# PengjieRen/CaSE_RG

Measured on AMD Instinct MI355X. Metric: train tokens/sec (query+passage) CaSE model, higher is better.
Workload: dtype bf16; 1 GPU; CaSE train step fwd+bwd+allreduce+clip+Adam+EMA, d_model=512, 6 encoder layers, 10 passages x 384 tok, query 64, answer 40, vocab 30522, per-GPU batch 32, dropout on; global_batch=32, parallelism=dp1

## Files before the change

### case_rg_amd/_abi.py

```python
import ctypes as C
import os

import torch

_HERE = os.path.dirname(os.path.abspath(__file__))
LIB_PATH = os.environ.get("CASE_HIP_LIB") or os.path.join(_HERE, "csrc", "libcase_hip.so")

ABI_VERSION = 600
F32, BF16 = 0, 1
WS_ATTENTION_SPLITKV, WS_ATTENTION_BWD, WS_OPTIM_SUMSQ, WS_ENCODER_CHAIN_PACK, WS_GEMM_DW_SLABS = 1, 2, 3, 4, 5
(FEAT_GEMM_256, FEAT_GEMM_SMALL, FEAT_ENCODER_CHAIN, FEAT_ATTN_SCORES, FEAT_ATTN_DECODE, FEAT_OPTIM, FEAT_ATTN_RESIDENT, FEAT_RESERVED_CUS,
 FEAT_GEMM_DW_SLABS, FEAT_DECODER_CHAIN, FEAT_ATTN_DECODE_MQA, FEAT_POINTER_DECODE, FEAT_POINTER_HEAD, FEAT_GEMM_LN, FEAT_STEP_STATE,
 FEAT_INTERACTION, FEAT_ATTN_DECODE_APPEND, FEAT_LINEAR_SKINNY) = (1 << i for i in range(18))
EPI_BIAS_COL, EPI_BIAS_ROW, EPI_GELU, EPI_RELU = 1, 2, 4, 8
EPI_RESIDUAL, EPI_MUL_DGELU, EPI_MUL_DRELU, EPI_ATOMIC, EPI_DROPOUT = 16, 32, 64, 128, 256

i32, i64, u64, f32, f64, ptr = C.c_int32, C.c_int64, C.c_uint64, C.c_float, C.c_double, C.c_void_p


class GemmDesc(C.Structure):
    _fields_ = [(n, i64) for n in ("M", "N", "K", "lda", "ldb", "ldc", "ld_aux", "batch1", "batch2",
                                   "sa1", "sa2", "sb1", "sb2", "sc1", "sc2", "saux1", "saux2")] + \
               [(n, i32) for n in ("a_kmajor", "b_kmajor", "in_dtype", "out_dtype", "epilogue", "split_k", "tile")] + \
               [("alpha", f32), ("drop_p", f32), ("seed", u64), ("offset", u64), ("state", ptr)]


class StepState(C.Structure):
    _fields_ = [("rng_base", u64), ("step_size", f32), ("bc2_sqrt", f32), ("lr", f32), ("step", i32), ("reserved", u64 * 5)]


class EncoderChainDesc(C.Structure):
    _fields_ = [("rows", i64), ("width", i32), ("variant", i32), ("eps_ln2", f32), ("eps_ln1_next", f32)]


class SoftmaxDesc(C.Structure):
    _fields_ = [("outer", i64), ("inner", i64), ("R", i64), ("C", i64), ("causal", i32), ("in_dtype", i32),
                ("out_dtype", i32), ("drop_p", f32), ("seed", u64), ("offset", u64), ("state", ptr)]


class AttnDesc(C.Structure):
    _fields_ = [(n, i64) for n in ("N", "heads", "Lq", "Lk", "head_dim", "ldq", "ldk", "ldv", "sq", "sk", "sv", "ldo", "so")] + \
               [("causal", i32), ("scale", f32), ("drop_p", f32), ("seed", u64), ("offset", u64), ("state", ptr)]


class InteractionDesc(C.Structure):
    _fields_ = [(n, i64) for n in ("n", "Lp", "Lq", "H", "eq_div")] + [("dtype", i32)]


class AttnProductDesc(C.Structure):
    _fields_ = [(n, i64) for n in ("N", "heads", "M", "Kc", "head_dim", "lda", "sa_seq", "sa_head", "ldb", "sb_seq", "sb_head",
                                   "ldc", "sc_seq", "sc_head")] + [("a_transposed", i32), ("alpha", f32)]


SIGNATURES = {
    "case_gemm": [C.POINTER(GemmDesc), ptr, ptr, ptr, ptr, ptr, ptr, ptr, ptr],
    "case_gemm_dw_bias": [C.POINTER(GemmDesc), ptr, ptr, ptr, ptr, ptr],
    "case_gemm_dw_slabs": [C.POINTER(GemmDesc), ptr, ptr, ptr, ptr, ptr, i64, ptr],
    "case_embed_pos_fwd": [ptr, ptr, ptr, ptr, i64, i64, i64, i64, f32, f32, u64, u64, ptr, i32, ptr],
    "case_embed_pos_bwd": [ptr, ptr, ptr, i64, i64, i64, f32, f32, u64, u64, ptr, i32, ptr],
    "case_scale_add_rows": [ptr, ptr, ptr, i64, i64, i64, f32, i32, ptr],
    "case_layernorm_fwd": [ptr, ptr, ptr, ptr, ptr, ptr, ptr, i64, i64, f32, i32, ptr],
    "case_layernorm_bwd": [ptr, ptr, ptr, ptr, ptr, ptr, ptr, ptr, ptr, ptr, i64, i64, i32, ptr],
    "case_layernorm_bwd_dropout": [ptr, ptr, ptr, ptr, ptr, ptr, ptr, ptr, ptr, i64, i64, f32, u64, u64, ptr, i32, ptr],
    "case_layernorm_bwd_concat5": [ptr] * 15 + [i64, i64, i32, ptr],
    "case_softmax_fwd": [C.POINTER(SoftmaxDesc), ptr, ptr, ptr, ptr, ptr, ptr],
    "case_softmax_bwd": [C.POINTER(SoftmaxDesc), ptr, ptr, ptr, ptr],
    "case_attention_supported": [i64],
    "case_attention_fwd": [C.POINTER(AttnDesc), ptr, ptr, ptr, ptr, ptr, ptr, ptr],
    "case_attention_splitkv_workspace": [C.POINTER(AttnDesc), i32, C.POINTER(i64)],
    "case_attention_fwd_splitkv": [C.POINTER(AttnDesc), ptr, ptr, ptr, ptr, ptr, ptr, ptr, i64, i32, ptr],
    "case_attention_bwd_supported": [i64],
    "case_attention_decode_supported": [i64],
    "case_attention_decode": [C.POINTER(AttnDesc), ptr, ptr, ptr, ptr, ptr, ptr],
    "case_attention_decode_append": [C.POINTER(AttnDesc), ptr, ptr, ptr, ptr, ptr, i64, i64, ptr, ptr, ptr],
    "case_attention_bwd": [C.POINTER(AttnDesc), ptr, ptr, ptr, ptr, ptr, ptr, ptr, ptr, ptr, ptr, ptr, ptr],
    "case_attention_scores_supported": [C.POINTER(AttnDesc)],
    "case_attention_scores_fwd": [C.POINTER(AttnDesc), ptr, ptr, ptr, ptr, ptr, ptr],
    "case_attention_scores_bwd": [C.POINTER(AttnDesc), ptr, ptr, ptr, ptr, ptr],
    "case_attention_product_supported": [C.POINTER(AttnProductDesc)],
    "case_attention_product": [C.POINTER(AttnProductDesc), ptr, ptr, ptr, ptr],
    "case_add": [ptr, ptr, ptr, i64, i32, ptr],
    "case_add_n": [C.POINTER(ptr), i32, ptr, i64, i32, ptr],
    "case_dropout": [ptr, ptr, i64, f32, u64, u64, ptr, i32, ptr],
    "case_mask_rows": [ptr, ptr, ptr, i64, i64, i32, ptr],
    "case_colsum": [ptr, ptr, i64, i64, i32, ptr],
    "case_cast": [ptr, ptr, i64, i32, i32, ptr],
    "case_scale_cols": [ptr, ptr, ptr, i64, i64, i32, ptr],
    "case_scale_cols_bwd": [ptr, ptr, ptr, ptr, ptr, i64, i64, i32, ptr],
    "case_rowdot_fwd": [ptr, ptr, ptr, ptr, i64, i64, i32, ptr],
    "case_linear_skinny": [ptr, ptr, i32, ptr, ptr, ptr, i64, i32, i32, ptr],
    "case_rowdot_bwd": [ptr, ptr, ptr, ptr, ptr, ptr, i64, i64, i32, ptr],
    "case_masked_mean_fwd": [ptr, ptr, ptr, i64, i64, i64, i32, ptr],
    "case_masked_mean_bwd": [ptr, ptr, ptr, i64, i64, i64, i32, ptr],
    "case_highway_gate_fwd": [ptr, ptr, i64, i64, i32, ptr],
    "case_highway_gate_bwd": [ptr, ptr, ptr, i64, i64, i32, ptr],
    "case_concat5_fwd": [ptr, ptr, ptr, ptr, ptr, i64, i64, i32, ptr],
    "case_concat5_bwd": [ptr, ptr, ptr, ptr, ptr, ptr, ptr, ptr, i64, i64, i32, ptr],
    "case_max_over_p_fwd": [ptr, ptr, ptr, i64, i64, i64, i32, ptr],
    "case_max_over_p_bwd": [ptr, ptr, ptr, i64, i64, i64, i32, ptr],
    "case_additive_scores_fwd": [ptr, ptr, ptr, ptr, i64, i64, i64, i64, i32, ptr],
    "case_additive_scores_bwd": [ptr, ptr, ptr, ptr, ptr, ptr, ptr, i64, i64, i64, i64, i32, ptr],
    "case_copy_scatter_fwd": [ptr, ptr, ptr, i64, i64, i64, i64, ptr],
    "case_copy_scatter_bwd": [ptr, ptr, ptr, i64, i64, i64, i64, ptr],
    "case_source_sort": [ptr, ptr, i64, i64, i64, ptr],
    "case_copy_scatter_sorted_fwd": [ptr, ptr, ptr, i64, i64, i64, i64, ptr],
    "case_nll_gather_fwd": [ptr, ptr, ptr, i64, i64, ptr],
    "case_nll_gather_bwd": [ptr, ptr, ptr, ptr, i64, i64, ptr],
    "case_row_argmax": [ptr, ptr, ptr, i64, i64, i64, ptr],
    "case_sentence_compact": [ptr, ptr, ptr, i64, i64, i64, i64, i64, ptr],
    "case_encoder_chain_pack": [ptr, ptr, ptr, ptr, ptr, ptr],
    "case_encoder_chain": [C.POINTER(EncoderChainDesc)] + [ptr] * 14,
    "case_set_reserved_cus": [i32],
    "case_attention_decode_mqa": [ptr, ptr, ptr, ptr, i64, i64, i64, i32, ptr, i64, ptr],
    "case_additive_key_exp": [ptr, ptr, i64, ptr],
    "case_pointer_attend_decode": [ptr] * 11 + [i64, i64, i64, ptr],
    "case_pointer_head_decode": [ptr] * 5 + [i32] + [ptr] * 4 + [i64, i64, i64, ptr],
    "case_gemm_ln": [C.POINTER(GemmDesc), ptr, ptr, ptr, f32, ptr, ptr, ptr, ptr, ptr, ptr],
    "case_optim_sumsq": [ptr, ptr, i64, ptr, ptr, ptr],
    "case_optim_adam_ema": [ptr, ptr, i64, ptr, f32, f64, f64, f64, f64, ptr, ptr],
    "case_step_advance": [ptr, u64, f64, f64, ptr],
    "case_interaction_supported": [C.POINTER(InteractionDesc)],
    "case_interaction_fwd": [C.POINTER(InteractionDesc), ptr, ptr, ptr, ptr, ptr, ptr, ptr, ptr, ptr, ptr],
}


def _load():
    if not os.path.exists(LIB_PATH):
        raise ImportError(
            "case_rg_amd: %s is missing. Build it with `python -c 'import __graft_entry__ as g; g.build()'` "
            "(or `make -C case_rg_amd/csrc`). There is no CPU or eager fallback." % LIB_PATH)
    lib = C.CDLL(LIB_PATH)
    lib.case_version.restype = C.c_int
    if lib.case_version() != ABI_VERSION:
        raise ImportError("case_rg_amd: %s is ABI generation %d, this package binds %d -- rebuild it (make -C case_rg_amd/csrc)"
                          % (LIB_PATH, lib.case_version(), ABI_VERSION))
    for name, args in SIGNATURES.items():
        fn = getattr(lib, name)
        fn.argtypes = args
        fn.restype = C.c_int
    lib.case_optim_chunk_elems.restype = C.c_int
    lib.case_optim_chunk_elems.argtypes = []
    lib.case_encoder_chain_packed_bytes.restype = C.c_int64
    lib.case_encoder_chain_packed_bytes.argtypes = []
    lib.case_attention_bwd_scratch_floats.restype = C.c_int64
    lib.case_attention_bwd_scratch_floats.argtypes = [C.POINTER(AttnDesc)]
# ... 35 lines not shown
```

### case_rg_amd/common/TransformerBlock.py

```python
import torch
import torch.nn as nn
import torch.nn.functional as F

from .. import config, ops
from .attention import MultiheadAttention


class TransformerBlock(nn.Module):
    def __init__(self, num_heads, input_hidden_size, output_hidden_size, activation=None):
        super().__init__()
        self.output_hidden_size = output_hidden_size
        self.self_attn = MultiheadAttention(input_hidden_size, num_heads, dropout=0.1)
        self.norm1 = nn.LayerNorm(input_hidden_size)
        self.norm2 = nn.LayerNorm(input_hidden_size)
        self.linear1 = nn.Linear(input_hidden_size, output_hidden_size)
        self.linear2 = nn.Linear(output_hidden_size, output_hidden_size)
        if activation is None or activation is F.relu:
            self.activation = "relu"
        elif activation is F.gelu:
            self.activation = "gelu"
        else:
            raise NotImplementedError("TransformerBlock on the HIP path supports relu (reference default) or gelu")

    def forward(self, input, input_mask):
        B, N, L, E = input.shape
        x = input.reshape(B * N, L, E)
        valid = input_mask.reshape(B * N, L)
        p = config.drop_p(0.1, self.training)
        if torch.is_grad_enabled() and x.requires_grad:
            fused = ops.concat5_layer_norm_carry(input, self.norm1.weight, self.norm1.bias, self.norm1.eps)
            if fused is not None:
                n1, xres = fused[0].reshape(B * N, L, E), fused[1].reshape(B * N, L, E)
            else:
                n1, xres = ops.layer_norm_carry(x, self.norm1.weight, self.norm1.bias, self.norm1.eps)
        else:
            n1, xres = ops.layer_norm(x, self.norm1.weight, self.norm1.bias, self.norm1.eps), x
        n2 = self.self_attn.self_attention(n1, valid, residual=xres, p_res=0.1, ln=(self.norm2.weight, self.norm2.bias, self.norm2.eps))
        y = ops.ffn(n2, self.linear1.weight, self.linear1.bias, self.linear2.weight, self.linear2.bias,
                    self.activation, p_inner=p, p_out=0.0)
        y = ops.mask_rows(y, valid, in_place=True)
        return y.reshape(B, N, L, self.output_hidden_size)
```

### case_rg_amd/common/heads.py

```python
import os

import torch
import torch.distributed as dist
import torch.nn as nn
import torch.nn.functional as F

from .. import ops
from .TransformerBlock import TransformerBlock


def block_stack(num_heads, hidden_size, extra):
    return nn.ModuleList([TransformerBlock(num_heads, 5 * hidden_size, hidden_size)] +
                         [TransformerBlock(num_heads, hidden_size, hidden_size) for _ in range(extra)])


def run_blocks(blocks, reps, mask):
    for block in blocks:
        reps = block(reps, mask)
    return reps


SIDE_STREAM = os.environ.get("CASE_SIDE_STREAM", "1") != "0"
SIDE_STREAM_INFERENCE = os.environ.get("CASE_SIDE_STREAM_INFERENCE", "0") == "1"
SIDE_STREAM_NOT_UNDER_DP = os.environ.get("CASE_SIDE_STREAM_UNDER_DP", "0") != "1"
SIDE_STREAM_MIN_ELEMS = 100_000_000
_side = {}


def run_block_pair(query_blocks, g_pq, query_mask, passage_blocks, g_qp, passage_mask):
    if not (SIDE_STREAM and g_pq.is_cuda and g_qp.numel() >= SIDE_STREAM_MIN_ELEMS and (torch.is_grad_enabled() or SIDE_STREAM_INFERENCE)
            and not torch.cuda.is_current_stream_capturing() and not (SIDE_STREAM_NOT_UNDER_DP and dist.is_available() and dist.is_initialized())):
        return run_blocks(query_blocks, g_pq, query_mask), run_blocks(passage_blocks, g_qp, passage_mask)
    cur = torch.cuda.current_stream()
    side = _side.get(g_pq.device)
    if side is None:
        side = _side[g_pq.device] = torch.cuda.Stream(device=g_pq.device)
    ops.AUX_STREAMS[side.cuda_stream] = side
    ops.AUX_STREAMS[cur.cuda_stream] = cur
    side.wait_stream(cur)
    with torch.cuda.stream(side):
        g_pq.record_stream(side)
        if torch.is_tensor(query_mask):
            query_mask.record_stream(side)
        query_reps = run_blocks(query_blocks, g_pq, query_mask)
    passage_reps = run_blocks(passage_blocks, g_qp, passage_mask)
    cur.wait_stream(side)
    query_reps.record_stream(cur)
    return query_reps, passage_reps


def passage_bce(passage_score, passage_label):
    target = torch.zeros_like(passage_score).scatter_(1, passage_label.unsqueeze(-1), 1.0)
    return F.binary_cross_entropy_with_logits(passage_score.float(), target.float()).unsqueeze(0)


def generation_nll(dist, response):
    V = dist.size(-1)
    rows = ops.nll_rows(dist.reshape(-1, V), response.reshape(-1))
    count = response.ne(0).sum().clamp(min=1)
    return (rows.sum() / count).unsqueeze(0)
```

### case_rg_amd/csrc/gemm.hip

```cpp
#include "common.h"

typedef __attribute__((ext_vector_type(8))) short bf16x8;
typedef __attribute__((ext_vector_type(4))) short s16x4;
typedef __attribute__((ext_vector_type(16))) float f32x16;
typedef __attribute__((ext_vector_type(4))) float f32x4;
typedef __attribute__((ext_vector_type(4))) unsigned int u32x4;

struct Args {
  const void* A; const void* B; void* C;
  const float* bias_col; const float* bias_row; const void* aux; void* aux_out;
  int64_t M, N, K, lda, ldb, ldc, ld_aux;
  int64_t batch2, sa1, sa2, sb1, sb2, sc1, sc2, saux1, saux2;
  int tiles_m, tiles_n, split_k, k_tiles_per_split;
  int nwg;
  float alpha, drop_p;
  uint64_t seed, offset;
  const CaseStepState* state;
  int vec_a, vec_b;
  int vec_c;
  float* rowsum;
  float* slabs;
  int64_t slab_stride;
  const float* ln_gamma; const float* ln_beta; void* ln_out; float ln_eps;
};

#define GEMM_NS gemm_w4
#define GEMM_NTHREADS 256
#include "gemm_impl.inc"
#undef GEMM_NS
#undef GEMM_NTHREADS

#include "gemm8w.inc"
#include "gemm_small.inc"

namespace {
constexpr int BM = 128, BN = 128, ROWB = 128;

int device_cus() { return case_device_cus(); }
}

namespace {
int prepare(const CaseGemmDesc* d, const void* A, const void* B, void* C, const float* bias_col, const float* bias_row,
            const void* aux, void* aux_out, Args& a, int* tile) {
  CASE_REQUIRE(d && A && B && C, "case_gemm: null argument");
  CASE_REQUIRE(d->M > 0 && d->N > 0 && d->K > 0, "case_gemm: empty problem M=%lld N=%lld K=%lld", (long long)d->M,
               (long long)d->N, (long long)d->K);
  CASE_REQUIRE(d->batch1 > 0 && d->batch2 > 0, "case_gemm: batch must be positive");
  CASE_REQUIRE(d->tile == 0 || d->tile == 64 || d->tile == 128 || d->tile == 256, "case_gemm: tile must be 0, 64, 128 or 256");
  const int epi = d->epilogue;
  CASE_REQUIRE(!(epi & CASE_EPI_BIAS_COL) || bias_col, "case_gemm: BIAS_COL without bias_col");
  CASE_REQUIRE(!(epi & CASE_EPI_BIAS_ROW) || bias_row, "case_gemm: BIAS_ROW without bias_row");
  CASE_REQUIRE(!(epi & (CASE_EPI_RESIDUAL | CASE_EPI_MUL_DGELU | CASE_EPI_MUL_DRELU)) || aux,
               "case_gemm: epilogue needs aux");
  const int split = d->split_k < 1 ? 1 : d->split_k;
  CASE_REQUIRE(split == 1 || ((epi & CASE_EPI_ATOMIC) && d->out_dtype == CASE_F32),
               "case_gemm: split_k > 1 needs CASE_EPI_ATOMIC and f32 output");
  CASE_REQUIRE(!((epi & CASE_EPI_RESIDUAL) && (epi & (CASE_EPI_MUL_DGELU | CASE_EPI_MUL_DRELU))),
               "case_gemm: RESIDUAL and MUL_D* share the aux operand and cannot be combined");
  CASE_REQUIRE(!(epi & CASE_EPI_DROPOUT) || (d->drop_p > 0.f && d->drop_p < 1.f), "case_gemm: drop_p out of range");
  CASE_REQUIRE(!(epi & CASE_EPI_ATOMIC) ||
                   !(epi & (CASE_EPI_GELU | CASE_EPI_RELU | CASE_EPI_RESIDUAL | CASE_EPI_MUL_DGELU | CASE_EPI_MUL_DRELU |
                            CASE_EPI_DROPOUT)),
               "case_gemm: non-linear epilogue cannot be combined with split-K accumulation");
  CASE_REQUIRE((d->in_dtype == CASE_BF16 || d->in_dtype == CASE_F32) && (d->out_dtype == CASE_F32 || (d->out_dtype == CASE_BF16 && d->in_dtype == CASE_BF16)),
               "case_gemm: dtype combination in=%d out=%d", d->in_dtype, d->out_dtype);
  const int esz = d->in_dtype == CASE_BF16 ? 2 : 4;
  const int ept = 16 / esz;
  a.A = A; a.B = B; a.C = C; a.bias_col = bias_col; a.bias_row = bias_row; a.aux = aux; a.aux_out = aux_out;
  a.M = d->M; a.N = d->N; a.K = d->K; a.lda = d->lda; a.ldb = d->ldb; a.ldc = d->ldc; a.ld_aux = d->ld_aux;
  a.batch2 = d->batch2; a.sa1 = d->sa1; a.sa2 = d->sa2; a.sb1 = d->sb1; a.sb2 = d->sb2; a.sc1 = d->sc1;
  a.sc2 = d->sc2; a.saux1 = d->saux1; a.saux2 = d->saux2;
  a.tiles_m = (int)((d->M + BM - 1) / BM);
  a.tiles_n = (int)((d->N + BN - 1) / BN);
  const int bke = ROWB / esz;
  const int kt = (int)((d->K + bke - 1) / bke);
  a.split_k = split > kt ? kt : split;
  a.k_tiles_per_split = (kt + a.split_k - 1) / a.split_k;
  a.split_k = (kt + a.k_tiles_per_split - 1) / a.k_tiles_per_split;
  const int64_t nwg = (int64_t)a.tiles_m * a.tiles_n * a.split_k * d->batch1 * d->batch2;
  CASE_REQUIRE(nwg < (1ll << 31), "case_gemm: grid too large");
  a.nwg = (int)nwg;
  a.alpha = d->alpha;
  a.rowsum = nullptr;
  a.slabs = nullptr;
  a.slab_stride = 0;
  a.ln_gamma = a.ln_beta = nullptr;
  a.ln_out = nullptr;
  a.ln_eps = 0.f;
  a.drop_p = d->drop_p; a.seed = d->seed; a.offset = d->offset; a.state = d->state;
  auto aligned = [&](const void* p, int64_t ld, int64_t s1, int64_t s2, int64_t extent) {
    return ((uintptr_t)p % 16 == 0) && (ld % ept == 0) && (s1 % ept == 0) && (s2 % ept == 0) && (extent % ept == 0);
  };
  a.vec_a = aligned(A, d->lda, d->sa1, d->sa2, d->a_kmajor ? d->M : d->K);
  a.vec_b = aligned(B, d->ldb, d->sb1, d->sb2, d->b_kmajor ? d->N : d->K);
  {
    const int eo = d->out_dtype == CASE_BF16 ? 8 : 4;
    auto ok = [&](const void* p, int64_t ld, int64_t s1, int64_t s2, int e) {
      return p == nullptr || (((uintptr_t)p % 16 == 0) && ld % e == 0 && s1 % e == 0 && s2 % e == 0);
    };
    a.vec_c = ok(C, d->ldc, d->sc1, d->sc2, eo) && ok(aux, d->ld_aux, d->saux1, d->saux2, ept) &&
              ok(aux_out, d->ld_aux, d->saux1, d->saux2, ept) && ok(bias_col, 4, 0, 0, 4);
  }
  *tile = 128;
  if (d->tile != 128 && d->in_dtype == CASE_BF16 && d->batch1 * d->batch2 == 1 && d->M % 256 == 0 && d->N % 256 == 0 && d->K % 64 == 0 &&
      a.vec_a && a.vec_b && a.vec_c && d->lda < (1 << 22) && d->ldb < (1 << 22) && d->ldc < (1 << 22) && d->ld_aux < (1 << 22) &&
      (!(epi & CASE_EPI_ATOMIC) || (epi == CASE_EPI_ATOMIC && d->out_dtype == CASE_F32))) {
    const int64_t t256 = (d->M / 256) * (d->N / 256) * a.split_k;
    const bool span_ok = (!d->a_kmajor || (d->K / a.split_k + 64) * d->lda < (1ll << 30)) &&
                         (!d->b_kmajor || (d->K / a.split_k + 64) * d->ldb < (1ll << 30));
    if (span_ok && d->tile != 64 && (d->tile == 256 || gemm_t8w::prefer(nwg, t256, device_cus()))) *tile = 256;
  }
  if (*tile == 128 && d->tile != 128 && d->tile != 256 && d->in_dtype == CASE_BF16 && d->batch1 * d->batch2 == 1 && d->M % 64 == 0 &&
      d->N % 64 == 0 && d->K % 64 == 0 && a.k_tiles_per_split <= gemm_sm::MAXKT && a.vec_a && a.vec_b && d->lda < (1 << 22) &&
      d->ldb < (1 << 22) && (!(epi & CASE_EPI_ATOMIC) || d->out_dtype == CASE_F32)) {
    const int64_t t64 = (d->M / 64) * (d->N / 64) * a.split_k;
    const bool span_ok = (!d->a_kmajor || (int64_t)a.k_tiles_per_split * 64 * d->lda < (1ll << 30)) &&
                         (!d->b_kmajor || (int64_t)a.k_tiles_per_split * 64 * d->ldb < (1ll << 30));
    if (span_ok && (d->tile == 64 || (nwg < device_cus() && t64 <= 2 * device_cus()))) *tile = 64;
  }
  return 0;
}
}

#ifdef G8_CLOCK_STAMPS
extern "C" int case_debug_gemm_clock(unsigned long long* out2) {
  unsigned long long h[4];
  if (hipMemcpyFromSymbol(h, HIP_SYMBOL(gemm_t8w::g_clock_stamps), sizeof(h)) != hipSuccess) return 1;
  out2[0] = h[2] - h[0];
  out2[1] = h[3] - h[1];
  return 0;
}
#endif
extern "C" int case_gemm_tile_for(const CaseGemmDesc* d, const void* A, const void* B, const void* C, const float* bias_col,
                                  const void* aux, const void* aux_out) {
  Args a;
  int tile = 0;
  const float one = 0.f;
  const int rc = prepare(d, A, B, const_cast<void*>(C), bias_col, (d && (d->epilogue & CASE_EPI_BIAS_ROW)) ? &one : nullptr, aux,
                         const_cast<void*>(aux_out), a, &tile);
  return rc ? rc : tile;
}

extern "C" int case_gemm_dw_bias(const CaseGemmDesc* d, const void* A, const void* B, void* C, float* d_bias, case_stream_t stream) {
  Args a;
  int tile = 0;
  const int rc = prepare(d, A, B, C, nullptr, nullptr, nullptr, nullptr, a, &tile);
  if (rc) return rc;
  CASE_REQUIRE(d_bias, "case_gemm_dw_bias: null d_bias");
  if (!(tile == 256 && d->a_kmajor && d->epilogue == CASE_EPI_ATOMIC && d->out_dtype == CASE_F32))
    return case_set_error(CASE_E_UNSUPPORTED, "case_gemm_dw_bias: needs the 256x256 tiling (see case_gemm_tile_for), a k-major A, "
                                              "the bare ATOMIC epilogue and f32 output");
  a.rowsum = d_bias;
  return gemm_t8w::launch<float, 1>(a, d->epilogue, d->a_kmajor, d->b_kmajor, case_persistent_cus(), (hipStream_t)stream);
}

namespace {
__global__ __launch_bounds__(256) void splitk_reduce_kernel(const float* __restrict__ slabs, float* __restrict__ C, const int64_t quads,
                                                            const int splits, const int64_t stride, const int accumulate) {
  const int64_t q = (int64_t)blockIdx.x * 256 + threadIdx.x;
  if (q >= quads) return;
  const f32x4* src = reinterpret_cast<const f32x4*>(slabs) + q;
  const int64_t sq = stride / 4;
  f32x4 acc = accumulate ? reinterpret_cast<const f32x4*>(C)[q] : f32x4{0.f, 0.f, 0.f, 0.f};
  int s = 0;
  for (; s + 8 <= splits; s += 8) {
    f32x4 v[8];
#pragma unroll
    for (int u = 0; u < 8; ++u) v[u] = __builtin_nontemporal_load(src + (int64_t)(s + u) * sq);
#pragma unroll
    for (int u = 0; u < 8; ++u) acc += v[u];
  }
  for (; s < splits; ++s) acc += __builtin_nontemporal_load(src + (int64_t)s * sq);
  reinterpret_cast<f32x4*>(C)[q] = acc;
}
}

extern "C" int64_t case_gemm_dw_slab_bytes(const CaseGemmDesc* d) {
  if (!d || d->M <= 0 || d->N <= 0 || d->K <= 0) return 0;
  const int kt = (int)((d->K + 63) / 64);
  int split = d->split_k < 1 ? 1 : d->split_k;
  split = split > kt ? kt : split;
  const int per = (kt + split - 1) / split;
  split = (kt + per - 1) / per;
  return split < 2 ? 0 : (int64_t)split * d->M * d->N * 4;
}

extern "C" int case_gemm_dw_slabs(const CaseGemmDesc* d, const void* A, const void* B, void* C, float* d_bias, void* slabs,
                                  int64_t slab_bytes, case_stream_t stream) {
  Args a;
// ... 69 lines not shown
```

### case_rg_amd/csrc/gemm8w.inc

```
namespace gemm_t8w {

using gemm_w4::Epilogue;

constexpr int TM = 256, TN = 256, BKE = 64, NTHR = 512;
constexpr int OPB = 32768, STAGE = 2 * OPB, EXTRA = 32768, LDS_BYTES = 2 * STAGE + EXTRA;
constexpr int STRIP = 8192;

#pragma clang diagnostic push
#pragma clang diagnostic ignored "-Winline-asm"
typedef __attribute__((ext_vector_type(4))) int i32x4;
__device__ __forceinline__ void dma16(i32x4 rsrc, unsigned voff, unsigned soff, unsigned lds_addr) {
  asm volatile("s_mov_b32 m0, %0\n\ts_nop 0\n\tbuffer_load_dwordx4 %1, %2, %3 offen lds" ::"s"(lds_addr), "v"(voff), "s"(rsrc),
               "s"(soff)
               : "memory", "m0");
}
#pragma clang diagnostic pop
__device__ __forceinline__ i32x4 make_rsrc(const void* p) {
  i32x4 r;
  r[0] = __builtin_amdgcn_readfirstlane((int)(size_t)p);
  r[1] = __builtin_amdgcn_readfirstlane((int)(((size_t)p) >> 32) & 0xffff);
  r[2] = -1;
  r[3] = 0x00020000;
  return r;
}
// ... 21 lines not shown
struct Op {
  static __device__ __forceinline__ void dma_voff(int wave, int l, int64_t ld, unsigned& v0, unsigned& v1) {
    if constexpr (!KMAJOR) {
      const int r0 = wave * 16 + (l >> 3), r1 = r0 + 8;
      v0 = (unsigned)(r0 * ld * 2 + (((l & 7) ^ ((r0 >> 1) & 7)) * 16));
      v1 = (unsigned)(r1 * ld * 2 + (((l & 7) ^ ((r1 >> 1) & 7)) * 16));
    } else {
      const int j = l >> 3, f = ((j >> 1) & 1) + 2 * (wave & 1);
      v0 = (unsigned)((wave * 8 + j) * ld * 2 + (((l & 7) ^ (2 * f)) * 16));
      v1 = v0 + 128;
    }
  }
  static __device__ __forceinline__ unsigned half_goff(int64_t ld) { return KMAJOR ? 256u : (unsigned)(128 * ld * 2); }
  static __device__ __forceinline__ unsigned kt_goff(int64_t ld) { return KMAJOR ? (unsigned)(64 * ld * 2) : 128u; }
  static __device__ __forceinline__ unsigned piece0(unsigned wv) { return KMAJOR ? wv * 1024 : wv * 2048; }
  static __device__ __forceinline__ unsigned piece1(unsigned wv) { return KMAJOR ? 8192 + wv * 1024 : wv * 2048 + 1024; }
  static __device__ __forceinline__ const char* origin(const bf16_t* op, int64_t ld, int64_t mn0, int64_t k0) {
    return reinterpret_cast<const char*>(KMAJOR ? op + k0 * ld + mn0 : op + mn0 * ld + k0);
  }

  int base[KMAJOR ? 4 : 2];
  __device__ __forceinline__ void init(int l) {
    if constexpr (!KMAJOR) {
      const int r = l & 15, s = r >> 1;
      base[0] = r * 128 + ((((l >> 4) + 0) ^ s) * 16);
      base[1] = r * 128 + ((((l >> 4) + 4) ^ s) * 16);
    } else {
      const int g = l >> 4, q = (l & 15) >> 2, t = l & 3, f = (q >> 1) + 2 * (g & 1);
#pragma unroll
      for (int x = 0; x < 4; ++x) base[x] = g * 1024 + q * 128 + (((x ^ f) * 2 + (t >> 1)) * 16) + (t & 1) * 8;
    }
  }
  __device__ __forceinline__ bf16x8 frag_at(const char* img, int lane_base, int c, int kh) const {
    if constexpr (!KMAJOR) {
      return *reinterpret_cast<const bf16x8*>(img + c * 2048 + base[kh]);
    } else {
      typedef __attribute__((address_space(3))) s16x4 lds_s16x4;
      const char* p = img + kh * 4096 + lane_base;
      const s16x4 lo = __builtin_amdgcn_ds_read_tr16_b64_v4i16((lds_s16x4*)(p));
      const s16x4 hi = __builtin_amdgcn_ds_read_tr16_b64_v4i16((lds_s16x4*)(p + 512));
      bf16x8 r;
      r[0] = lo[0]; r[1] = lo[1]; r[2] = lo[2]; r[3] = lo[3];
      r[4] = hi[0]; r[5] = hi[1]; r[6] = hi[2]; r[7] = hi[3];
      return r;
    }
  }
  __device__ __forceinline__ int lane_base_of(bool upper, int i) const {
    if constexpr (!KMAJOR) return 0;
    else return upper ? base[2 + i] : base[i];
  }
  __device__ __forceinline__ bf16x8 frag(const char* img, int c, int kh) const {
    if constexpr (!KMAJOR) {
      return *reinterpret_cast<const bf16x8*>(img + c * 2048 + base[kh]);
    } else {
      typedef __attribute__((address_space(3))) s16x4 lds_s16x4;
      const char* p = img + ((c >> 2) & 1) * 8192 + kh * 4096 + base[c & 3];
      const s16x4 lo = __builtin_amdgcn_ds_read_tr16_b64_v4i16((lds_s16x4*)(p));
      const s16x4 hi = __builtin_amdgcn_ds_read_tr16_b64_v4i16((lds_s16x4*)(p + 512));
      bf16x8 r;
      r[0] = lo[0]; r[1] = lo[1]; r[2] = lo[2]; r[3] = lo[3];
      r[4] = hi[0]; r[5] = hi[1]; r[6] = hi[2]; r[7] = hi[3];
      return r;
    }
  }
};


struct Tile {
  int64_t m0, n0;
  int kt_begin, kt_end, split;
};

#define G8_FENCE() { asm volatile("" ::: "memory"); __builtin_amdgcn_sched_barrier(0); }
#define G8_BARRIER() { G8_FENCE() __builtin_amdgcn_s_barrier(); G8_FENCE() }

#ifndef CASE_STREAM_DEFAULT_POLICY
#define G8_AUX_POLICY 2
#else
#define G8_AUX_POLICY 0
#endif
template <int ECT, typename OutT>
__device__ __forceinline__ void drain_pass(const Args& g, const int epi_rt, const float* strip, const int le, const int p,
                                           const int64_t row_w, const int64_t col_w, const float (&bc)[8], const u32x4 (&ax)[4],
                                           const __amdgpu_buffer_rsrc_t rc, const __amdgpu_buffer_rsrc_t ro) {
  const int E = ECT >= 0 ? ECT : epi_rt;
  const int cc = (le & 7) * 8;
  const bool need_aux = E & (CASE_EPI_RESIDUAL | CASE_EPI_MUL_DGELU | CASE_EPI_MUL_DRELU);
  const float drop_scale = (E & CASE_EPI_DROPOUT) ? 1.f / (1.f - g.drop_p) : 1.f;
  const int vc = (int)(((le >> 3) * g.ldc + cc) * (int64_t)sizeof(OutT));
  const int va = (int)(((le >> 3) * g.ld_aux + cc) * 2);
  float v[4][8];
#pragma unroll
  for (int s = 0; s < 4; ++s) {
    const int rr = s * 8 + (le >> 3);
    const int s0 = ((le & 7) * 2) ^ (rr & 15), s1 = ((le & 7) * 2 + 1) ^ (rr & 15);
    const f32x4 lo = *reinterpret_cast<const f32x4*>(strip + rr * 64 + s0 * 4);
    const f32x4 hi = *reinterpret_cast<const f32x4*>(strip + rr * 64 + s1 * 4);
    v[s][0] = lo[0]; v[s][1] = lo[1]; v[s][2] = lo[2]; v[s][3] = lo[3];
    v[s][4] = hi[0]; v[s][5] = hi[1]; v[s][6] = hi[2]; v[s][7] = hi[3];
  }
#pragma unroll
  for (int s = 0; s < 4; ++s) {
    const int rb = p * 32 + s * 8;
    const int64_t row = row_w + rb + (le >> 3);
    float* x = v[s];
    float a8[8];
    if (need_aux) {
#pragma unroll
      for (int i = 0; i < 4; ++i) {
        a8[2 * i] = __uint_as_float(ax[s][i] << 16);
        a8[2 * i + 1] = __uint_as_float(ax[s][i] & 0xffff0000u);
      }
    }
    const float br = (E & CASE_EPI_BIAS_ROW) ? g.bias_row[row] : 0.f;
#pragma unroll
    for (int e = 0; e < 8; ++e) x[e] = g.alpha * x[e] + ((E & CASE_EPI_BIAS_COL) ? bc[e] : 0.f) + br;
    if (E & CASE_EPI_GELU) {
      if (g.aux_out) {
        u32x4 w;
#pragma unroll
        for (int i = 0; i < 4; ++i) w[i] = f32x2_to_bf16x2(x[2 * i], x[2 * i + 1]);
        __builtin_amdgcn_raw_buffer_store_b128(w, ro, va + (int)(rb * g.ld_aux * 2), 0, G8_AUX_POLICY);
      }
#pragma unroll
      for (int e = 0; e < 8; ++e) x[e] = gelu_f(x[e]);
    }
    if (E & CASE_EPI_RELU) {
#pragma unroll
      for (int e = 0; e < 8; ++e) x[e] = fmaxf(x[e], 0.f);
    }
    if (E & CASE_EPI_MUL_DGELU) {
#pragma unroll
      for (int e = 0; e < 8; ++e) x[e] *= dgelu_f(a8[e]);
    }
    if (E & CASE_EPI_MUL_DRELU) {
#pragma unroll
      for (int e = 0; e < 8; ++e) x[e] = a8[e] > 0.f ? x[e] : 0.f;
    }
    if (E & CASE_EPI_DROPOUT) {
      const uint64_t idx0 = g.offset + rng_base_of(g.state) + (uint64_t)(row * g.N + col_w + cc);
      dropout8(v[s], g.seed, idx0, g.drop_p, drop_scale);
    }
    if (E & CASE_EPI_RESIDUAL) {
#pragma unroll
      for (int e = 0; e < 8; ++e) x[e] += a8[e];
    }
    const int sc = (int)(rb * g.ldc * (int64_t)sizeof(OutT));
    if constexpr (sizeof(OutT) == 2) {
      u32x4 w;
#pragma unroll
      for (int i = 0; i < 4; ++i) w[i] = f32x2_to_bf16x2(x[2 * i], x[2 * i + 1]);
      __builtin_amdgcn_raw_buffer_store_b128(w, rc, vc + sc, 0, 0);
    } else {
      u32x4 w0, w1;
#pragma unroll
      for (int i = 0; i < 4; ++i) { w0[i] = __float_as_uint(x[i]); w1[i] = __float_as_uint(x[4 + i]); }
      __builtin_amdgcn_raw_buffer_store_b128(w0, rc, vc + sc, 0, 0);
      __builtin_amdgcn_raw_buffer_store_b128(w1, rc, vc + sc + 16, 0, 0);
    }
  }
}

template <int ECT, typename OutT>
__device__ __forceinline__ void epilogue_tile(const Args& g, const int epi_rt, float* strip, const int le, const int64_t row_w,
                                              const int64_t col_w, const f32x4 (&acc)[8][4], void* const cbase) {
  const int E = ECT >= 0 ? ECT : epi_rt;
  const bool need_aux = E & (CASE_EPI_RESIDUAL | CASE_EPI_MUL_DGELU | CASE_EPI_MUL_DRELU);
  float bc[8] = {0.f, 0.f, 0.f, 0.f, 0.f, 0.f, 0.f, 0.f};
  if (E & CASE_EPI_BIAS_COL) Epilogue<bf16_t, OutT>::load8(g.bias_col + col_w + (le & 7) * 8, bc);
  const __amdgpu_buffer_rsrc_t rc =
      __builtin_amdgcn_make_buffer_rsrc(uniform_ptr(reinterpret_cast<OutT*>(cbase) + row_w * g.ldc + col_w), 0, -1, 0x00020000);
  const bf16_t* auxp = g.aux ? (const bf16_t*)uniform_ptr(reinterpret_cast<const bf16_t*>(g.aux) + row_w * g.ld_aux + col_w) : nullptr;
  bf16_t* auxo = g.aux_out ? (bf16_t*)uniform_ptr(reinterpret_cast<bf16_t*>(g.aux_out) + row_w * g.ld_aux + col_w) : nullptr;
  const __amdgpu_buffer_rsrc_t ra = __builtin_amdgcn_make_buffer_rsrc((void*)auxp, 0, auxp ? -1 : 0, 0x00020000);
  const __amdgpu_buffer_rsrc_t ro = __builtin_amdgcn_make_buffer_rsrc((void*)auxo, 0, auxo ? -1 : 0, 0x00020000);
  const int va = (int)(((le >> 3) * g.ld_aux + (le & 7) * 8) * 2);
  const int lr = le & 15, lg = le >> 4;
#pragma unroll
  for (int p = 0; p < 4; ++p) {
    u32x4 ax[4];
    if (need_aux) {
#pragma unroll
      for (int s = 0; s < 4; ++s) ax[s] = __builtin_amdgcn_raw_buffer_load_b128(ra, va + (int)((p * 32 + s * 8) * g.ld_aux * 2), 0, G8_AUX_POLICY);
    }
#pragma unroll
    for (int ii = 0; ii < 2; ++ii)
#pragma unroll
      for (int j = 0; j < 4; ++j)
        *reinterpret_cast<f32x4*>(strip + (ii * 16 + lr) * 64 + (((j * 4 + lg) ^ lr) * 4)) = acc[2 * p + ii][j];
    asm volatile("" ::: "memory");
    __builtin_amdgcn_sched_barrier(0);
    drain_pass<ECT, OutT>(g, epi_rt, strip, le, p, row_w, col_w, bc, ax, rc, ro);
    asm volatile("" ::: "memory");
    __builtin_amdgcn_sched_barrier(0);
  }
}

template <int ECT, typename OutT>
__device__ __forceinline__ void epilogue_regs(const Args& g, const int epi_rt, const int le, const int64_t row_w, const int64_t col_w,
                                              const f32x4 (&acc)[8][4], void* const cbase) {
  const int E = ECT >= 0 ? ECT : epi_rt;
  const bool need_aux = E & (CASE_EPI_RESIDUAL | CASE_EPI_MUL_DGELU | CASE_EPI_MUL_DRELU);
  const float drop_scale = (E & CASE_EPI_DROPOUT) ? 1.f / (1.f - g.drop_p) : 1.f;
  const int lr = le & 15, lg = le >> 4;
  const int c0 = ((lg & 1) << 4) | ((lg >> 1) << 3);
  float bc[2][8];
#pragma unroll
  for (int p = 0; p < 2; ++p) {
    if (E & CASE_EPI_BIAS_COL) Epilogue<bf16_t, OutT>::load8(g.bias_col + col_w + c0 + 32 * p, bc[p]);
    else {
#pragma unroll
      for (int e = 0; e < 8; ++e) bc[p][e] = 0.f;
    }
  }
  const __amdgpu_buffer_rsrc_t rc =
      __builtin_amdgcn_make_buffer_rsrc(uniform_ptr(reinterpret_cast<OutT*>(cbase) + row_w * g.ldc + col_w), 0, -1, 0x00020000);
  const bf16_t* auxp = g.aux ? (const bf16_t*)uniform_ptr(reinterpret_cast<const bf16_t*>(g.aux) + row_w * g.ld_aux + col_w) : nullptr;
  bf16_t* auxo = g.aux_out ? (bf16_t*)uniform_ptr(reinterpret_cast<bf16_t*>(g.aux_out) + row_w * g.ld_aux + col_w) : nullptr;
  const __amdgpu_buffer_rsrc_t ra = __builtin_amdgcn_make_buffer_rsrc((void*)auxp, 0, auxp ? -1 : 0, 0x00020000);
  const __amdgpu_buffer_rsrc_t ro = __builtin_amdgcn_make_buffer_rsrc((void*)auxo, 0, auxo ? -1 : 0, 0x00020000);
  const int vc = (int)((lr * g.ldc + c0) * (int64_t)sizeof(OutT));
  const int va = (int)((lr * g.ld_aux + c0) * 2);
  u32x4 ax[4];
#define G8_AUX_LOAD(DST, IB)                                                                                          \
  _Pragma("unroll") for (int q = 0; q < 4; ++q)                                                                       \
    DST[q] = __builtin_amdgcn_raw_buffer_load_b128(ra, va + (int)((((IB) + (q >> 1)) * 16 * g.ld_aux + 32 * (q & 1)) * 2), 0, 0);
#pragma unroll
  for (int ib = 0; ib < 8; ib += 2) {
    if (need_aux) { G8_AUX_LOAD(ax, ib) }
#pragma unroll
    for (int q = 0; q < 4; ++q) {
      const int i = ib + (q >> 1), p = q & 1;
      float x[8];
#pragma unroll
      for (int e = 0; e < 4; ++e) {
        const auto sw = __builtin_amdgcn_permlane16_swap(__float_as_uint(acc[i][2 * p][e]), __float_as_uint(acc[i][2 * p + 1][e]), false, false);
        x[e] = __uint_as_float(sw[0]);
        x[4 + e] = __uint_as_float(sw[1]);
      }
      const int64_t row = row_w + 16 * i + lr;
      const int cc = c0 + 32 * p;
      float a8[8];
      if (need_aux) {
#pragma unroll
        for (int t = 0; t < 4; ++t) {
          a8[2 * t] = __uint_as_float(ax[q][t] << 16);
          a8[2 * t + 1] = __uint_as_float(ax[q][t] & 0xffff0000u);
        }
      }
      const float br = (E & CASE_EPI_BIAS_ROW) ? g.bias_row[row] : 0.f;
#pragma unroll
      for (int e = 0; e < 8; ++e) x[e] = g.alpha * x[e] + ((E & CASE_EPI_BIAS_COL) ? bc[p][e] : 0.f) + br;
      const int so = (int)((16 * i * g.ld_aux + 32 * p) * 2);
      if (E & CASE_EPI_GELU) {
        if (g.aux_out) {
          u32x4 w;
#pragma unroll
          for (int t = 0; t < 4; ++t) w[t] = f32x2_to_bf16x2(x[2 * t], x[2 * t + 1]);
          __builtin_amdgcn_raw_buffer_store_b128(w, ro, va + so, 0, 0);
        }
#pragma unroll
        for (int e = 0; e < 8; ++e) x[e] = gelu_f(x[e]);
      }
      if (E & CASE_EPI_RELU) {
#pragma unroll
        for (int e = 0; e < 8; ++e) x[e] = fmaxf(x[e], 0.f);
      }
      if (E & CASE_EPI_MUL_DGELU) {
#pragma unroll
        for (int e = 0; e < 8; ++e) x[e] *= dgelu_f(a8[e]);
      }
      if (E & CASE_EPI_MUL_DRELU) {
#pragma unroll
        for (int e = 0; e < 8; ++e) x[e] = a8[e] > 0.f ? x[e] : 0.f;
      }
      if (E & CASE_EPI_DROPOUT) {
        const uint64_t idx0 = g.offset + rng_base_of(g.state) + (uint64_t)(row * g.N + col_w + cc);
        dropout8(x, g.seed, idx0, g.drop_p, drop_scale);
      }
      if (E & CASE_EPI_RESIDUAL) {
#pragma unroll
        for (int e = 0; e < 8; ++e) x[e] += a8[e];
      }
      const int sc = (int)((16 * i * g.ldc + 32 * p) * (int64_t)sizeof(OutT));
      if constexpr (sizeof(OutT) == 2) {
        u32x4 w;
#pragma unroll
        for (int t = 0; t < 4; ++t) w[t] = f32x2_to_bf16x2(x[2 * t], x[2 * t + 1]);
        __builtin_amdgcn_raw_buffer_store_b128(w, rc, vc + sc, 0, 0);
      } else {
        u32x4 w0, w1;
#pragma unroll
        for (int t = 0; t < 4; ++t) { w0[t] = __float_as_uint(x[t]); w1[t] = __float_as_uint(x[4 + t]); }
        __builtin_amdgcn_raw_buffer_store_b128(w0, rc, vc + sc, 0, 0);
        __builtin_amdgcn_raw_buffer_store_b128(w1, rc, vc + sc + 16, 0, 0);
      }
    }
  }
#undef G8_AUX_LOAD
}

#ifdef G8_CLOCK_STAMPS
__device__ unsigned long long g_clock_stamps[4];
#endif
template <typename OutT, bool AK, bool BK_, int ATOMIC>
__global__ __launch_bounds__(NTHR, 2) void gemm8w_kernel(const Args g, const int epi, const int tiles_m, const int tiles_n,
                                                         const int ntiles) {
  extern __shared__ __attribute__((aligned(16))) char smem[];
  const int tid = threadIdx.x, l = tid & 63, wave = tid >> 6, wr = wave >> 2, wc = wave & 3;
  const unsigned lds0 = (unsigned)(size_t)(__attribute__((address_space(3))) char*)smem;
  const unsigned wv = __builtin_amdgcn_readfirstlane(wave);

  const int xcd = blockIdx.x & 7, idx = blockIdx.x >> 3;
  const int nwx = ((int)gridDim.x - xcd + 7) >> 3;
  const int q = ntiles >> 3, r = ntiles & 7;
  const int first = xcd < r ? xcd * (q + 1) : r * (q + 1) + (xcd - r) * q, count = q + (xcd < r ? 1 : 0);
  if (idx >= count) return;
#ifdef G8_CLOCK_STAMPS
  if (blockIdx.x == 0 && tid == 0) {
    g_clock_stamps[0] = __builtin_amdgcn_s_memtime();
    g_clock_stamps[1] = __builtin_amdgcn_s_memrealtime();
  }
#endif

  const int kt_total = (int)(g.K / BKE);
  auto decode = [&](int pid) {
    Tile t;
    const int per_slab = tiles_m * tiles_n;
    const int in_slab = pid % per_slab, split = pid / per_slab;
    constexpr int GM = 4;
    const int group = in_slab / (GM * tiles_n), first_m = group * GM, gm = min(GM, tiles_m - first_m);
    const int tm = first_m + (in_slab - group * GM * tiles_n) % gm, tn = (in_slab - group * GM * tiles_n) / gm;
    t.m0 = (int64_t)tm * TM;
    t.n0 = (int64_t)tn * TN;
    t.split = split;
    t.kt_begin = split * g.k_tiles_per_split;
    t.kt_end = min(t.kt_begin + g.k_tiles_per_split, kt_total);
    return t;
  };

  unsigned va0, va1, vb0, vb1;
  Op<AK>::dma_voff(wave, l, g.lda, va0, va1);
  Op<BK_>::dma_voff(wave, l, g.ldb, vb0, vb1);
  const unsigned hga = Op<AK>::half_goff(g.lda), hgb = Op<BK_>::half_goff(g.ldb);
  const unsigned kga = Op<AK>::kt_goff(g.lda), kgb = Op<BK_>::kt_goff(g.ldb);
  const unsigned pa0 = Op<AK>::piece0(wv), pa1 = Op<AK>::piece1(wv), pb0 = Op<BK_>::piece0(wv), pb1 = Op<BK_>::piece1(wv);
  const bf16_t* Ag = reinterpret_cast<const bf16_t*>(g.A);
  const bf16_t* Bg = reinterpret_cast<const bf16_t*>(g.B);
  Op<AK> fa;
  Op<BK_> fb;
  fa.init(l);
  fb.init(l);

#ifdef G8_TIMING_ONLY_L2_RESIDENT
#define G8_KT(KT) ((KT) & 7)
#else
#define G8_KT(KT) (KT)
#endif
#define ISSUE_A(S, H, KT)                                                       \
  {                                                                             \
    const unsigned sb = lds0 + (S) * STAGE + (H) * 16384;                       \
    const unsigned so = (unsigned)G8_KT(KT) * kga + (H) * hga;                  \
    dma16(rsa, va0, so, sb + pa0);                                              \
    dma16(rsa, va1, so, sb + pa1);                                              \
  }
// ... 140 lines not shown
      MMA(0, 1, HI)                                                                                                    \
      G8_BARRIER()                                                                                                     \
       \
       \
      READ_A(st, 1)                                                                                                    \
      if (n2) { ISSUE_B(s, 0, (kt) + 2) __builtin_amdgcn_s_waitcnt(0x0076); }                         \
      else if (n1) __builtin_amdgcn_s_waitcnt(0x0074);                                                \
      else LGKM0();                                                                                                    \
      G8_BARRIER()                                                                                                     \
      MMA(1, 1, HI)                                                                                                    \
      G8_BARRIER()                                                                                                     \
       \
       \
      if (n1) READ_B(sn, 0, HI)                                                                                        \
      if (n2) ISSUE_B(s, 1, (kt) + 2)                                                                                  \
      ROWSUM(1)                                                                                                        \
      if (n2) __builtin_amdgcn_s_waitcnt(0x0f74);                                                       \
      else __builtin_amdgcn_s_waitcnt(0x0f70);                                                          \
      G8_BARRIER()                                                                                                     \
      MMA(1, 0, LO)                                                                                                    \
      G8_BARRIER()                                                                                                     \
    }
    READ_B(smem, 0, 0)
    for (int kt2 = 0; kt2 < nk; kt2 += 2) {
      KTILE(kt2, 0, 1)
      if (kt2 + 1 < nk) KTILE(kt2 + 1, 1, 0)
    }
#undef KTILE
#endif
    if (wr == 0) G8_BARRIER()
#undef ROWSUM
#undef READ_A
#undef READ_B
#undef MMA
#undef LGKM0

    const int nit = it + nwx;
    const bool more = nit < count;
    Tile nxt = cur;
    if (more) {
      nxt = decode(first + nit);
      rsa = make_rsrc(Op<AK>::origin(Ag, g.lda, nxt.m0, (int64_t)nxt.kt_begin * BKE));
      rsb = make_rsrc(Op<BK_>::origin(Bg, g.ldb, nxt.n0, (int64_t)nxt.kt_begin * BKE));
      PROLOGUE(nxt.kt_end - nxt.kt_begin)
    }

    int le = l;
    asm volatile("" : "+v"(le));
    const int64_t row_w = cur.m0 + wr * 128, col_w = cur.n0 + wc * 64;
    if constexpr (ATOMIC != 0) {
      if constexpr (ATOMIC == 2) {
        epilogue_regs<0, float>(g, 0, le, row_w, col_w, acc, g.slabs + (int64_t)cur.split * g.slab_stride);
      } else {
        float* Cf = reinterpret_cast<float*>(g.C) + (row_w + 4 * (le >> 4)) * g.ldc + col_w + (le & 15);
#ifdef G8_TIMING_ONLY_NO_ATOMICS
#pragma unroll
        for (int i = 0; i < 8; ++i)
#pragma unroll
          for (int j = 0; j < 4; ++j) asm volatile("" ::"v"(acc[i][j]));
        if (g.alpha == 12345.f) Cf[0] = acc[0][0][0];
#else
#pragma unroll
        for (int i = 0; i < 8; ++i)
#pragma unroll
          for (int j = 0; j < 4; ++j)
#pragma unroll
            for (int e = 0; e < 4; ++e) atomicAdd(Cf + (i * 16 + e) * g.ldc + j * 16, g.alpha * acc[i][j][e]);
#endif
      }
      if constexpr (AK) {
        if (do_rs) {
#pragma unroll
          for (int u = 0; u < 2; ++u) {
            float v = rs[u];
            v += __shfl_xor(v, 16);
            v += __shfl_xor(v, 32);
            if (le < 16) atomicAdd(g.rowsum + row_w + (2 * wc + u) * 16 + le, g.alpha * v);
          }
        }
      }
    } else {
      float* strip = reinterpret_cast<float*>(smem + (wave < 4 ? STAGE + wave * STRIP : 2 * STAGE + (wave - 4) * STRIP));
      constexpr int B = CASE_EPI_BIAS_COL, R = CASE_EPI_RESIDUAL, D = CASE_EPI_DROPOUT, G = CASE_EPI_GELU;
      constexpr int RL = CASE_EPI_RELU, DG = CASE_EPI_MUL_DGELU, DR = CASE_EPI_MUL_DRELU;
#define EPI(E)                                                                                  \
  {                                                                                             \
    if constexpr (sizeof(OutT) == 4) epilogue_regs<E, OutT>(g, epi, le, row_w, col_w, acc, g.C); \
    else epilogue_tile<E, OutT>(g, epi, strip, le, row_w, col_w, acc, g.C);                     \
  }
      switch (epi) {
        case 0: EPI(0); break;
        case B: EPI(B); break;
        case B | R: EPI(B | R); break;
        case B | R | D: EPI(B | R | D); break;
        case B | G: EPI(B | G); break;
        case B | G | D: EPI(B | G | D); break;
        case B | RL | D: EPI(B | RL | D); break;
        case DG | D: EPI(DG | D); break;
        case DR | D: EPI(DR | D); break;
        default: EPI(-1); break;
      }
#undef EPI
    }
    if (!more) break;
    younger = younger_per_tile;
    cur = nxt;
    it = nit;
  }
#ifdef G8_CLOCK_STAMPS
  if (blockIdx.x == 0 && tid == 0) {
    g_clock_stamps[2] = __builtin_amdgcn_s_memtime();
    g_clock_stamps[3] = __builtin_amdgcn_s_memrealtime();
  }
#endif
#undef ISSUE_A
#undef ISSUE_B
#undef PROLOGUE
}
#undef G8_FENCE
#undef G8_BARRIER

static inline bool prefer(int64_t tiles128, int64_t tiles256, int cus) {
  const double t128 = (double)((tiles128 + 2 * cus - 1) / (2 * cus)) * 2.0 / 830.0;
  const double t256 = (double)((tiles256 + cus - 1) / cus) * 4.0 / 1300.0;
  return t256 < t128;
}

template <typename OutT, int ATOMIC>
int launch(const Args& a, int epi, bool ak, bool bk, int cus, hipStream_t s) {
  const int tiles_m = (int)(a.M / TM), tiles_n = (int)(a.N / TN);
  const int ntiles = tiles_m * tiles_n * a.split_k;
  const dim3 grid(ntiles < cus ? ntiles : cus), block(NTHR);
#define GO(AKV, BKV)                                                                                       \
  do {                                                                                                     \
    if (hipFuncSetAttribute(reinterpret_cast<const void*>(&gemm8w_kernel<OutT, AKV, BKV, ATOMIC>),         \
                            hipFuncAttributeMaxDynamicSharedMemorySize, LDS_BYTES) != hipSuccess)          \
      return case_set_error(CASE_E_LAUNCH, "case_gemm: cannot reserve %d bytes of LDS", LDS_BYTES);        \
    hipLaunchKernelGGL((gemm8w_kernel<OutT, AKV, BKV, ATOMIC>), grid, block, LDS_BYTES, s, a, epi, tiles_m, tiles_n, ntiles); \
  } while (0)
  if (!ak && !bk) GO(false, false);
  else if (!ak && bk) GO(false, true);
  else if (ak && !bk) GO(true, false);
  else GO(true, true);
#undef GO
  return case_check_launch("case_gemm");
}

}
```

### case_rg_amd/csrc/gemm_impl.inc

```
namespace GEMM_NS {

constexpr int BM = 128, BN = 128, NTHREADS = GEMM_NTHREADS;
constexpr int CHUNKS = 1024 / NTHREADS;
constexpr int MI = 512 / NTHREADS;
constexpr int MIN_WAVES = NTHREADS / 128;
constexpr int ROWB = 128;
constexpr int RM_STRIDE = ROWB + 16;
constexpr int OP_BYTES = 20480;
constexpr int STAGE_BYTES = 2 * OP_BYTES;

template <typename T> struct KM;
template <> struct KM<bf16_t> { static constexpr int row_stride = 256 + 64; };
template <> struct KM<float> { static constexpr int row_stride = 512 + 16; };


template <typename T, bool VEC>
__device__ __forceinline__ u32x4 load_chunk(const T* __restrict__ base, int64_t ld, int64_t lead, int64_t lead_max,
                                            int64_t c0, int64_t c_max, bool& ok) {
  constexpr int EPT = 16 / sizeof(T);
  ok = lead < lead_max && c0 < c_max;
  if constexpr (VEC) {
    return *reinterpret_cast<const u32x4*>(base + (ok ? lead * ld + c0 : 0));
  } else {
    T tmp[EPT];
// ... 165 lines not shown
      for (int e = 0; e < 4; ++e)
#pragma unroll
        for (int i = 0; i < MI; ++i)
#pragma unroll
          for (int j = 0; j < 2; ++j)
            acc[i][j] = __builtin_amdgcn_mfma_f32_32x32x2f32(a[i][e], b[j][e], acc[i][j], 0, 0, 0);
    }
  }
}

template <typename T, bool AK, bool BK_, bool VEC, bool FULL>
__device__ __forceinline__ void k_loop(f32x16 (&acc)[MI][2], char* smem, const T* __restrict__ A, const T* __restrict__ B,
                                       const Args& g, int64_t m0, int64_t n0, int kt_begin, int kt_end, int wr, int wc) {
  constexpr int BKE = ROWB / sizeof(T);
  u32x4 ra0[CHUNKS], rb0[CHUNKS], ra1[CHUNKS], rb1[CHUNKS];
  unsigned oka0, okb0, oka1 = 0, okb1 = 0;
  Loader<T, AK> lda_;
  Loader<T, BK_> ldb_;
  if constexpr (VEC) {
    lda_.init(A, g.lda, m0, g.M, (int64_t)kt_begin * BKE);
    ldb_.init(B, g.ldb, n0, g.N, (int64_t)kt_begin * BKE);
  }
#define LOAD_A(R, KT) (VEC ? lda_.template load<FULL>(R, (int64_t)(KT) * BKE, g.K) : stage_load<T, AK, false>(R, A, g.lda, m0, g.M, (int64_t)(KT) * BKE, g.K))
#define LOAD_B(R, KT) (VEC ? ldb_.template load<FULL>(R, (int64_t)(KT) * BKE, g.K) : stage_load<T, BK_, false>(R, B, g.ldb, n0, g.N, (int64_t)(KT) * BKE, g.K))
  oka0 = LOAD_A(ra0, kt_begin);
  okb0 = LOAD_B(rb0, kt_begin);
  stage_store<T, AK, FULL>(ra0, oka0, smem);
  stage_store<T, BK_, FULL>(rb0, okb0, smem + OP_BYTES);
  if (kt_begin + 1 < kt_end) {
    oka0 = LOAD_A(ra0, kt_begin + 1);
    okb0 = LOAD_B(rb0, kt_begin + 1);
  }
  __syncthreads();
  int cur = 0;
#define GEMM_STEP(KT, FARC, NEXTC, WAITN, RA_NEXT, RB_NEXT, OKA_NEXT, OKB_NEXT, RA_FAR, RB_FAR, OKA_FAR, OKB_FAR)  \
  {                                                                                                                \
    if (FARC) {                                                                                                    \
      OKA_FAR = LOAD_A(RA_FAR, (KT) + 2);                                                                          \
      OKB_FAR = LOAD_B(RB_FAR, (KT) + 2);                                                                          \
    }                                                                                                              \
    const char* la = smem + cur * STAGE_BYTES;                                                                     \
    mma_tile<T, AK, BK_>(acc, la, la + OP_BYTES, wr, wc);                                                          \
    if (NEXTC) {                                                                                                   \
      char* nx = smem + (cur ^ 1) * STAGE_BYTES;                                                                   \
      stage_store<T, AK, FULL>(RA_NEXT, OKA_NEXT, nx);                                                             \
      stage_store<T, BK_, FULL>(RB_NEXT, OKB_NEXT, nx + OP_BYTES);                                                 \
    }                                                                                                              \
    __syncthreads();                                                                                               \
    cur ^= 1;                                                                                                      \
  }
  int kt = kt_begin;
  for (; kt + 3 < kt_end; kt += 2) {
    GEMM_STEP(kt, true, true, 8, ra0, rb0, oka0, okb0, ra1, rb1, oka1, okb1)
    GEMM_STEP(kt + 1, true, true, 8, ra1, rb1, oka1, okb1, ra0, rb0, oka0, okb0)
  }
  const int left = kt_end - kt;
  if (left == 3) {
    GEMM_STEP(kt, true, true, 8, ra0, rb0, oka0, okb0, ra1, rb1, oka1, okb1)
    GEMM_STEP(kt + 1, false, true, 0, ra1, rb1, oka1, okb1, ra0, rb0, oka0, okb0)
    GEMM_STEP(kt + 2, false, false, 0, ra0, rb0, oka0, okb0, ra1, rb1, oka1, okb1)
  } else if (left == 2) {
    GEMM_STEP(kt, false, true, 0, ra0, rb0, oka0, okb0, ra1, rb1, oka1, okb1)
    GEMM_STEP(kt + 1, false, false, 0, ra1, rb1, oka1, okb1, ra0, rb0, oka0, okb0)
  } else if (left == 1) {
    GEMM_STEP(kt, false, false, 0, ra0, rb0, oka0, okb0, ra1, rb1, oka1, okb1)
  }
#undef GEMM_STEP
#undef LOAD_A
#undef LOAD_B
}

constexpr int CT_STRIDE = 132;
static_assert(BM * CT_STRIDE * 4 <= 2 * STAGE_BYTES, "staged C tile must fit in the K-loop buffers");

__device__ __forceinline__ void stage_acc(float* ctile, const f32x16& a, int r0, int c0) {
  float* base = ctile + r0 * CT_STRIDE + c0;
#pragma unroll
  for (int e = 0; e < 16; ++e) base[((e & 3) + 8 * (e >> 2)) * CT_STRIDE] = a[e];
}

template <typename T, typename OutT>
struct Epilogue {
  OutT* C; const T* aux; T* aux_out; const float* bias_row; const float* bias_col;
  int64_t ldc, ld_aux, M, N;
  float alpha, drop_p, drop_scale;
  uint64_t seed, rng_base;
  int epi;
  __device__ __forceinline__ void emit(float accv, int64_t row, int64_t col, float bias_c) const {
    if (row >= M || col >= N) return;
    float v = alpha * accv + bias_c;
    if (epi & CASE_EPI_BIAS_ROW) v += bias_row[row];
    if (epi & CASE_EPI_GELU) {
      if (aux_out) Elem<T>::st(aux_out + row * ld_aux + col, v);
      v = gelu_f(v);
    }
    if (epi & CASE_EPI_RELU) v = fmaxf(v, 0.f);
    if (epi & CASE_EPI_MUL_DGELU) v *= dgelu_f(Elem<T>::ld(aux + row * ld_aux + col));
    if (epi & CASE_EPI_MUL_DRELU) v = Elem<T>::ld(aux + row * ld_aux + col) > 0.f ? v : 0.f;
    if (epi & CASE_EPI_DROPOUT) v = rng_uniform(seed, rng_base + (uint64_t)(row * N + col)) >= drop_p ? v * drop_scale : 0.f;
    if (epi & CASE_EPI_RESIDUAL) v += Elem<T>::ld(aux + row * ld_aux + col);
    OutT* dst = C + row * ldc + col;
    if constexpr (sizeof(OutT) == 4) {
      if (epi & CASE_EPI_ATOMIC) atomicAdd(reinterpret_cast<float*>(dst), v);
      else *reinterpret_cast<float*>(dst) = v;
    } else {
      Elem<OutT>::st(dst, v);
    }
  }
  __device__ __forceinline__ void tile(const f32x16& a, int64_t row0, int64_t col) const {
    const float bc = ((epi & CASE_EPI_BIAS_COL) && col < N) ? bias_col[col] : 0.f;
    emit(a[0], row0 + 0, col, bc);   emit(a[1], row0 + 1, col, bc);   emit(a[2], row0 + 2, col, bc);   emit(a[3], row0 + 3, col, bc);
    emit(a[4], row0 + 8, col, bc);   emit(a[5], row0 + 9, col, bc);   emit(a[6], row0 + 10, col, bc);  emit(a[7], row0 + 11, col, bc);
    emit(a[8], row0 + 16, col, bc);  emit(a[9], row0 + 17, col, bc);  emit(a[10], row0 + 18, col, bc); emit(a[11], row0 + 19, col, bc);
    emit(a[12], row0 + 24, col, bc); emit(a[13], row0 + 25, col, bc); emit(a[14], row0 + 26, col, bc); emit(a[15], row0 + 27, col, bc);
  }
  __device__ __forceinline__ void chunk8(float (&v)[8], int64_t row, int64_t col, bool vec) const {
    const bool full = vec && col + 8 <= N;
    if (full) {
      float ax[8];
      const bool need_aux = epi & (CASE_EPI_RESIDUAL | CASE_EPI_MUL_DGELU | CASE_EPI_MUL_DRELU);
      if (need_aux) load8(aux + row * ld_aux + col, ax);
      float bc[8];
      if (epi & CASE_EPI_BIAS_COL) {
        const f32x4 b0 = *reinterpret_cast<const f32x4*>(bias_col + col), b1 = *reinterpret_cast<const f32x4*>(bias_col + col + 4);
        bc[0] = b0[0]; bc[1] = b0[1]; bc[2] = b0[2]; bc[3] = b0[3]; bc[4] = b1[0]; bc[5] = b1[1]; bc[6] = b1[2]; bc[7] = b1[3];
      }
      const float br = (epi & CASE_EPI_BIAS_ROW) ? bias_row[row] : 0.f;
#pragma unroll
      for (int e = 0; e < 8; ++e) v[e] = alpha * v[e] + ((epi & CASE_EPI_BIAS_COL) ? bc[e] : 0.f) + br;
      if (epi & CASE_EPI_GELU) {
        if (aux_out) store8(aux_out + row * ld_aux + col, v);
#pragma unroll
        for (int e = 0; e < 8; ++e) v[e] = gelu_f(v[e]);
      }
      if (epi & CASE_EPI_RELU) {
#pragma unroll
        for (int e = 0; e < 8; ++e) v[e] = fmaxf(v[e], 0.f);
      }
      if (epi & CASE_EPI_MUL_DGELU) {
#pragma unroll
        for (int e = 0; e < 8; ++e) v[e] *= dgelu_f(ax[e]);
      }
      if (epi & CASE_EPI_MUL_DRELU) {
#pragma unroll
        for (int e = 0; e < 8; ++e) v[e] = ax[e] > 0.f ? v[e] : 0.f;
      }
      if (epi & CASE_EPI_DROPOUT) {
        dropout8(v, seed, rng_base + (uint64_t)(row * N + col), drop_p, drop_scale);
      }
      if (epi & CASE_EPI_RESIDUAL) {
#pragma unroll
        for (int e = 0; e < 8; ++e) v[e] += ax[e];
      }
      store8(C + row * ldc + col, v);
    } else {
#pragma unroll
      for (int e = 0; e < 8; ++e)
        emit(v[e], row, col + e, ((epi & CASE_EPI_BIAS_COL) && col + e < N) ? bias_col[col + e] : 0.f);
    }
  }
  __device__ __forceinline__ void store_tile(const float* ctile, int64_t m0, int64_t n0, bool vec) const {
#pragma unroll 2
    for (int i = 0; i < 2048 / NTHREADS; ++i) {
      const int c = threadIdx.x + i * NTHREADS;
      const int r = c >> 4, cc = (c & 15) * 8;
      const int64_t row = m0 + r, col = n0 + cc;
      if (row >= M || col >= N) continue;
      const f32x4 lo = *reinterpret_cast<const f32x4*>(ctile + r * CT_STRIDE + cc);
      const f32x4 hi = *reinterpret_cast<const f32x4*>(ctile + r * CT_STRIDE + cc + 4);
      float v[8] = {lo[0], lo[1], lo[2], lo[3], hi[0], hi[1], hi[2], hi[3]};
      chunk8(v, row, col, vec);
    }
  }
  static __device__ __forceinline__ void load8(const float* p, float (&o)[8]) {
    const f32x4 a = *reinterpret_cast<const f32x4*>(p), b = *reinterpret_cast<const f32x4*>(p + 4);
    o[0] = a[0]; o[1] = a[1]; o[2] = a[2]; o[3] = a[3]; o[4] = b[0]; o[5] = b[1]; o[6] = b[2]; o[7] = b[3];
  }
  static __device__ __forceinline__ void load8(const bf16_t* p, float (&o)[8]) {
    const u32x4 w = *reinterpret_cast<const u32x4*>(p);
#pragma unroll
    for (int i = 0; i < 4; ++i) {
      o[2 * i] = __uint_as_float(w[i] << 16);
      o[2 * i + 1] = __uint_as_float(w[i] & 0xffff0000u);
    }
  }
  static __device__ __forceinline__ void store8(float* p, const float (&v)[8]) {
    f32x4 a = {v[0], v[1], v[2], v[3]}, b = {v[4], v[5], v[6], v[7]};
    *reinterpret_cast<f32x4*>(p) = a;
    *reinterpret_cast<f32x4*>(p + 4) = b;
  }
  static __device__ __forceinline__ void store8(bf16_t* p, const float (&v)[8]) {
    u32x4 w;
#pragma unroll
    for (int i = 0; i < 4; ++i) w[i] = f32x2_to_bf16x2(v[2 * i], v[2 * i + 1]);
    *reinterpret_cast<u32x4*>(p) = w;
  }
};

template <typename T, typename OutT, bool AK, bool BK_, bool VEC>
__global__ __launch_bounds__(NTHREADS, MIN_WAVES) void gemm_kernel(const Args g, const int epi) {
  extern __shared__ __attribute__((aligned(16))) char smem[];
  constexpr int BKE = ROWB / sizeof(T);

  int pid = blockIdx.x;
  {
    const int nwg = g.nwg, q = nwg >> 3, r = nwg & 7, xcd = pid & 7, idx = pid >> 3;
    pid = (xcd < r ? xcd * (q + 1) : r * (q + 1) + (xcd - r) * q) + idx;
  }
  const int per_slab = g.tiles_m * g.tiles_n;
  const int in_slab = pid % per_slab;
  int rest = pid / per_slab;
  constexpr int GM = 8;
  const int group = in_slab / (GM * g.tiles_n);
  const int first_m = group * GM;
  const int gm = min(GM, g.tiles_m - first_m);
  const int tm = first_m + (in_slab - group * GM * g.tiles_n) % gm;
  const int tn = (in_slab - group * GM * g.tiles_n) / gm;
  const int split = rest % g.split_k;
  const int64_t batch = rest / g.split_k;
  const int64_t b1 = batch / g.batch2, b2 = batch % g.batch2;

  const T* A = reinterpret_cast<const T*>(g.A) + b1 * g.sa1 + b2 * g.sa2;
  const T* B = reinterpret_cast<const T*>(g.B) + b1 * g.sb1 + b2 * g.sb2;
  const int64_t m0 = (int64_t)tm * BM, n0 = (int64_t)tn * BN;
  const int kt_begin = split * g.k_tiles_per_split;
  const int kt_total = (int)((g.K + BKE - 1) / BKE);
  int kt_end = kt_begin + g.k_tiles_per_split;
  if (kt_end > kt_total) kt_end = kt_total;

  const int wave = threadIdx.x >> 6, wr = wave >> 1, wc = wave & 1;
  f32x16 acc[MI][2];
#pragma unroll
  for (int i = 0; i < MI; ++i)
#pragma unroll
    for (int j = 0; j < 2; ++j)
#pragma unroll
      for (int e = 0; e < 16; ++e) acc[i][j][e] = 0.f;

  if (kt_begin < kt_end) {
    const bool full = VEC && (m0 + BM <= g.M) && (n0 + BN <= g.N) && (g.K % BKE == 0) &&
                      (uint64_t)g.lda * (uint64_t)(AK ? BKE : BM) * sizeof(T) < (1ull << 32) &&
                      (uint64_t)g.ldb * (uint64_t)(BK_ ? BKE : BN) * sizeof(T) < (1ull << 32);
    if (full) k_loop<T, AK, BK_, VEC, true>(acc, smem, A, B, g, m0, n0, kt_begin, kt_end, wr, wc);
    else k_loop<T, AK, BK_, VEC, false>(acc, smem, A, B, g, m0, n0, kt_begin, kt_end, wr, wc);
  }

  const int lane = threadIdx.x & 63;
  Epilogue<T, OutT> ep;
  ep.C = reinterpret_cast<OutT*>(g.C) + b1 * g.sc1 + b2 * g.sc2;
  ep.aux = g.aux ? reinterpret_cast<const T*>(g.aux) + b1 * g.saux1 + b2 * g.saux2 : nullptr;
  ep.aux_out = g.aux_out ? reinterpret_cast<T*>(g.aux_out) + b1 * g.saux1 + b2 * g.saux2 : nullptr;
  ep.bias_row = g.bias_row ? g.bias_row + batch * g.M : nullptr;
  ep.bias_col = g.bias_col;
  ep.ldc = g.ldc; ep.ld_aux = g.ld_aux; ep.M = g.M; ep.N = g.N;
  ep.alpha = g.alpha; ep.drop_p = g.drop_p; ep.seed = g.seed;
  ep.rng_base = g.offset + rng_base_of(g.state) + (uint64_t)(batch * g.M * g.N);
  ep.drop_scale = (epi & CASE_EPI_DROPOUT) ? 1.f / (1.f - g.drop_p) : 1.f;
  ep.epi = (split == 0) ? epi : (epi & ~(CASE_EPI_BIAS_COL | CASE_EPI_BIAS_ROW));
  if (epi & CASE_EPI_ATOMIC) {
    const int64_t col_base = n0 + wc * 64 + (lane & 31), row_base = m0 + wr * (32 * MI) + 4 * (lane >> 5);
    ep.tile(acc[0][0], row_base, col_base);
    ep.tile(acc[0][1], row_base, col_base + 32);
    if constexpr (MI == 2) {
      ep.tile(acc[MI - 1][0], row_base + 32, col_base);
      ep.tile(acc[MI - 1][1], row_base + 32, col_base + 32);
    }
    return;
  }
  float* ctile = reinterpret_cast<float*>(smem);
  {
    const int c0 = wc * 64 + (lane & 31), r0 = wr * (32 * MI) + 4 * (lane >> 5);
    stage_acc(ctile, acc[0][0], r0, c0);
    stage_acc(ctile, acc[0][1], r0, c0 + 32);
    if constexpr (MI == 2) {
      stage_acc(ctile, acc[MI - 1][0], r0 + 32, c0);
      stage_acc(ctile, acc[MI - 1][1], r0 + 32, c0 + 32);
    }
  }
  __syncthreads();
  ep.store_tile(ctile, m0, n0, g.vec_c != 0);
}

template <typename T, typename OutT>
int launch(const Args& a, int epi, bool ak, bool bk, hipStream_t s) {
  const dim3 grid(a.nwg), block(NTHREADS);
  const size_t lds = 2 * STAGE_BYTES;
#define GO1(AKV, BKV, VV)                                                                                  \
  do {                                                                                                     \
    static bool attr_set = false;                                                                          \
    if (!attr_set) {                                                                                       \
      (void)hipFuncSetAttribute(reinterpret_cast<const void*>(&gemm_kernel<T, OutT, AKV, BKV, VV>),        \
                                hipFuncAttributeMaxDynamicSharedMemorySize, (int)lds);                     \
      attr_set = true;                                                                                     \
    }                                                                                                      \
    hipLaunchKernelGGL((gemm_kernel<T, OutT, AKV, BKV, VV>), grid, block, lds, s, a, epi);                 \
  } while (0)
#define GO(AKV, BKV)                                                                                       \
  do {                                                                                                     \
    if (a.vec_a && a.vec_b) GO1(AKV, BKV, true);                                                           \
    else GO1(AKV, BKV, false);                                                                             \
  } while (0)
  if (!ak && !bk) GO(false, false);
  else if (!ak && bk) GO(false, true);
  else if (ak && !bk) GO(true, false);
  else GO(true, true);
#undef GO1
#undef GO
  return case_check_launch("case_gemm");
}

}
```

### case_rg_amd/csrc/gemm_small.inc

```
namespace gemm_sm {

using gemm_t8w::dma16;
using gemm_t8w::i32x4;
using gemm_t8w::make_rsrc;
using gemm_t8w::Op;

constexpr int TM = 64, TN = 64, BKE = 64, NTHR = 256, MAXKT = 10;
constexpr int IMG = 8192, KT_BYTES = 2 * IMG;

template <bool KMAJOR>
__device__ __forceinline__ void piece_voff(int p, int l, int64_t ld, unsigned& v) {
  if constexpr (!KMAJOR) {
    const int r = p * 8 + (l >> 3);
    v = (unsigned)(r * ld * 2 + (((l & 7) ^ ((r >> 1) & 7)) * 16));
  } else {
    const int j = l >> 3, f = ((j >> 1) & 1) + 2 * (p & 1);
    v = (unsigned)((p * 8 + j) * ld * 2 + (((l & 7) ^ (2 * f)) * 16));
  }
}

template <typename OutT, bool AK, bool BK_, bool LN = false>
__global__ __launch_bounds__(NTHR) void gemm_small_kernel(const Args g, const int epi, const int tiles_m, const int tiles_n) {
  extern __shared__ __attribute__((aligned(16))) char smem[];
  const int tid = threadIdx.x, l = tid & 63, wave = tid >> 6, wr = wave >> 1, wc = wave & 1;
// ... 52 lines not shown
    float sum = 0.f;
#pragma unroll
    for (int u = 0; u < 16; ++u) {
      const int kt = 2 * qd + (u >> 3), c = u & 7;
      Vec16<bf16_t>::load(reinterpret_cast<const bf16_t*>(smem + kt * KT_BYTES + r * 128 + ((c ^ sw) << 4)), v[u]);
#pragma unroll
      for (int e = 0; e < 8; ++e) sum += v[u][e];
    }
    sum += __shfl_xor(sum, 1, 64);
    sum += __shfl_xor(sum, 2, 64);
    const float mu = sum * (1.f / 512.f);
    float sq = 0.f;
#pragma unroll
    for (int u = 0; u < 16; ++u)
#pragma unroll
      for (int e = 0; e < 8; ++e) sq += (v[u][e] - mu) * (v[u][e] - mu);
    sq += __shfl_xor(sq, 1, 64);
    sq += __shfl_xor(sq, 2, 64);
    const float rs = rsqrtf(sq * (1.f / 512.f) + g.ln_eps);
    bf16_t* lo = (tn == 0 && g.ln_out) ? reinterpret_cast<bf16_t*>(g.ln_out) + (m0 + r) * 512 : nullptr;
#pragma unroll
    for (int u = 0; u < 16; ++u) {
      const int kt = 2 * qd + (u >> 3), c = u & 7, f = kt * 64 + c * 8;
      float gm[8], bt[8], o[8];
      Vec16<float>::load(gb + f, *reinterpret_cast<float(*)[4]>(gm));
      Vec16<float>::load(gb + f + 4, *reinterpret_cast<float(*)[4]>(gm + 4));
      Vec16<float>::load(gb + 512 + f, *reinterpret_cast<float(*)[4]>(bt));
      Vec16<float>::load(gb + 512 + f + 4, *reinterpret_cast<float(*)[4]>(bt + 4));
#pragma unroll
      for (int e = 0; e < 8; ++e) o[e] = (v[u][e] - mu) * rs * gm[e] + bt[e];
      Vec16<bf16_t>::store(reinterpret_cast<bf16_t*>(smem + kt * KT_BYTES + r * 128 + ((c ^ sw) << 4)), o);
      if (lo) Vec16<bf16_t>::store(lo + f, o);
    }
    __builtin_amdgcn_s_waitcnt(0xc07f);
  }
  for (int kt = 0; kt < nk; ++kt) {
    if constexpr (LN) {
      if (kt == 0) {
        asm volatile("" ::: "memory");
        __builtin_amdgcn_sched_barrier(0);
        __builtin_amdgcn_s_barrier();
        asm volatile("" ::: "memory");
        __builtin_amdgcn_sched_barrier(0);
      }
    } else
    switch (nk - 1 - kt) {
      case 0: __builtin_amdgcn_s_waitcnt(0x0f70); break;
      case 1: __builtin_amdgcn_s_waitcnt(0x0f74); break;
      case 2: __builtin_amdgcn_s_waitcnt(0x0f78); break;
      case 3: __builtin_amdgcn_s_waitcnt(0x0f7c); break;
      case 4: __builtin_amdgcn_s_waitcnt(0x4f70); break;
      case 5: __builtin_amdgcn_s_waitcnt(0x4f74); break;
      case 6: __builtin_amdgcn_s_waitcnt(0x4f78); break;
      case 7: __builtin_amdgcn_s_waitcnt(0x4f7c); break;
      case 8: __builtin_amdgcn_s_waitcnt(0x8f70); break;
      default: __builtin_amdgcn_s_waitcnt(0x8f74); break;
    }
    if constexpr (!LN) {
      asm volatile("" ::: "memory");
      __builtin_amdgcn_sched_barrier(0);
      __builtin_amdgcn_s_barrier();
      asm volatile("" ::: "memory");
      __builtin_amdgcn_sched_barrier(0);
    }
    const char* st = smem + kt * KT_BYTES;
    bf16x8 a[2][2], b[2][2];
#pragma unroll
    for (int i = 0; i < 2; ++i)
#pragma unroll
      for (int kh = 0; kh < 2; ++kh) {
        a[i][kh] = fa.frag_at(st, la[i], wr * 2 + i, kh);
        b[i][kh] = fb.frag_at(st + IMG, lb[i], wc * 2 + i, kh);
      }
#pragma unroll
    for (int kh = 0; kh < 2; ++kh)
#pragma unroll
      for (int i = 0; i < 2; ++i)
#pragma unroll
        for (int j = 0; j < 2; ++j) acc[i][j] = __builtin_amdgcn_mfma_f32_16x16x32_bf16(a[i][kh], b[j][kh], acc[i][j], 0, 0, 0);
  }

  gemm_w4::Epilogue<bf16_t, OutT> E;
  E.C = reinterpret_cast<OutT*>(g.C); E.aux = reinterpret_cast<const bf16_t*>(g.aux); E.aux_out = reinterpret_cast<bf16_t*>(g.aux_out);
  E.bias_row = g.bias_row; E.bias_col = g.bias_col; E.ldc = g.ldc; E.ld_aux = g.ld_aux; E.M = g.M; E.N = g.N;
  E.alpha = g.alpha; E.drop_p = g.drop_p; E.drop_scale = (epi & CASE_EPI_DROPOUT) ? 1.f / (1.f - g.drop_p) : 1.f;
  E.seed = g.seed; E.rng_base = g.offset + rng_base_of(g.state); E.epi = epi;
#pragma unroll
  for (int i = 0; i < 2; ++i)
#pragma unroll
    for (int j = 0; j < 2; ++j) {
      const int64_t col = n0 + wc * 32 + j * 16 + (l & 15);
      const float bc = (epi & CASE_EPI_BIAS_COL) ? g.bias_col[col] : 0.f;
#pragma unroll
      for (int e = 0; e < 4; ++e) E.emit(acc[i][j][e], m0 + wr * 32 + i * 16 + 4 * (l >> 4) + e, col, bc);
    }
}

template <typename OutT, bool LN>
int launch(const Args& a, int epi, bool ak, bool bk, hipStream_t s) {
  const int tiles_m = (int)(a.M / TM), tiles_n = (int)(a.N / TN);
  const int64_t nwg = (int64_t)tiles_m * tiles_n * a.split_k;
  const int lds = a.k_tiles_per_split * KT_BYTES + (LN ? 4096 : 0);
  const dim3 grid((unsigned)nwg), block(NTHR);
#define GO(AKV, BKV)                                                                                       \
  do {                                                                                                     \
    if (lds > 65536 && hipFuncSetAttribute(reinterpret_cast<const void*>(&gemm_small_kernel<OutT, AKV, BKV, LN>), \
                                           hipFuncAttributeMaxDynamicSharedMemorySize, LN ? 8 * KT_BYTES + 4096 : MAXKT * KT_BYTES) != hipSuccess) \
      return case_set_error(CASE_E_LAUNCH, "case_gemm: cannot reserve %d bytes of LDS", LN ? 8 * KT_BYTES + 4096 : MAXKT * KT_BYTES); \
    hipLaunchKernelGGL((gemm_small_kernel<OutT, AKV, BKV, LN>), grid, block, lds, s, a, epi, tiles_m, tiles_n); \
  } while (0)
  if constexpr (LN) {
    if (!bk) GO(false, false);
    else GO(false, true);
  } else {
    if (!ak && !bk) GO(false, false);
    else if (!ak && bk) GO(false, true);
    else if (ak && !bk) GO(true, false);
    else GO(true, true);
  }
#undef GO
  return case_check_launch("case_gemm");
}

}
```

### case_rg_amd/csrc/rowops.hip

```cpp
#include <stdlib.h>

#ifndef CASE_STREAM_DEFAULT_POLICY
#define CASE_VEC16_NT
#endif
#include "common.h"

namespace {

constexpr int LN_THREADS = 256;
constexpr int LN_MAXPT = 16;

template <typename T>
__global__ __launch_bounds__(LN_THREADS) void ln_fwd_kernel(const T* __restrict__ x, const T* __restrict__ x2,
                                                            const float* __restrict__ gamma,
                                                            const float* __restrict__ beta, T* __restrict__ y,
                                                            float* __restrict__ mean, float* __restrict__ rstd,
                                                            int64_t rows, int64_t cols, float eps) {
  __shared__ float red[32];
  for (int64_t r = blockIdx.x; r < rows; r += gridDim.x) {
    const T* xr = x + r * cols;
    const T* x2r = x2 ? x2 + r * cols : nullptr;
    float s = 0.f;
    for (int64_t c = threadIdx.x; c < cols; c += LN_THREADS) s += Elem<T>::ld(xr + c) + (x2r ? Elem<T>::ld(x2r + c) : 0.f);
    const float mu = block_sum(s, red) / (float)cols;
    float q = 0.f;
    for (int64_t c = threadIdx.x; c < cols; c += LN_THREADS) {
      const float d = Elem<T>::ld(xr + c) + (x2r ? Elem<T>::ld(x2r + c) : 0.f) - mu;
      q += d * d;
    }
    const float rs = rsqrtf(block_sum(q, red) / (float)cols + eps);
    if (threadIdx.x == 0) {
      mean[r] = mu;
      rstd[r] = rs;
    }
    T* yr = y + r * cols;
    for (int64_t c = threadIdx.x; c < cols; c += LN_THREADS) {
      const float v = Elem<T>::ld(xr + c) + (x2r ? Elem<T>::ld(x2r + c) : 0.f);
      Elem<T>::st(yr + c, (v - mu) * rs * gamma[c] + beta[c]);
    }
  }
}

template <typename T>
__global__ __launch_bounds__(LN_THREADS) void ln_bwd_kernel(const T* __restrict__ dy, const T* __restrict__ x,
                                                            const T* __restrict__ x2, const float* __restrict__ gamma,
                                                            const float* __restrict__ mean,
                                                            const float* __restrict__ rstd, T* __restrict__ dx,
                                                            const T* __restrict__ dx_add, float* __restrict__ d_gamma,
                                                            float* __restrict__ d_beta, int64_t rows, int64_t cols) {
  __shared__ float red[32];
  float acc_g[LN_MAXPT], acc_b[LN_MAXPT];
#pragma unroll
  for (int i = 0; i < LN_MAXPT; ++i) acc_g[i] = acc_b[i] = 0.f;
  for (int64_t r = blockIdx.x; r < rows; r += gridDim.x) {
    const T* xr = x + r * cols;
    const T* x2r = x2 ? x2 + r * cols : nullptr;
    const T* dyr = dy + r * cols;
    const float mu = mean[r], rs = rstd[r];
    float s1 = 0.f, s2 = 0.f;
#pragma unroll
    for (int i = 0; i < LN_MAXPT; ++i) {
      const int64_t c = threadIdx.x + (int64_t)i * LN_THREADS;
      if (c < cols) {
        const float xh = (Elem<T>::ld(xr + c) + (x2r ? Elem<T>::ld(x2r + c) : 0.f) - mu) * rs;
        const float d = Elem<T>::ld(dyr + c);
        const float g = d * gamma[c];
        s1 += g;
        s2 += g * xh;
        acc_g[i] += d * xh;
        acc_b[i] += d;
      }
    }
    const float m1 = block_sum(s1, red) / (float)cols;
    const float m2 = block_sum(s2, red) / (float)cols;
    T* dxr = dx + r * cols;
#pragma unroll
    for (int i = 0; i < LN_MAXPT; ++i) {
      const int64_t c = threadIdx.x + (int64_t)i * LN_THREADS;
      if (c < cols) {
        const float xh = (Elem<T>::ld(xr + c) + (x2r ? Elem<T>::ld(x2r + c) : 0.f) - mu) * rs;
        const float g = Elem<T>::ld(dyr + c) * gamma[c];
        Elem<T>::st(dxr + c, rs * (g - m1 - xh * m2) + (dx_add ? Elem<T>::ld(dx_add + r * cols + c) : 0.f));
      }
    }
  }
#pragma unroll
  for (int i = 0; i < LN_MAXPT; ++i) {
    const int64_t c = threadIdx.x + (int64_t)i * LN_THREADS;
    if (c < cols) {
      atomicAdd(d_gamma + c, acc_g[i]);
      atomicAdd(d_beta + c, acc_b[i]);
    }
  }
}

constexpr int LNV_MAX = 8;

template <typename T, int NV>
__global__ __launch_bounds__(256) void ln_fwd_vec_kernel(const T* __restrict__ x, const T* __restrict__ x2,
                                                         const float* __restrict__ gamma, const float* __restrict__ beta,
                                                         T* __restrict__ y, float* __restrict__ mean,
                                                         float* __restrict__ rstd, int64_t rows, int64_t cols, float eps) {
  constexpr int E = Vec16<T>::N;
  const int lane = threadIdx.x & 63;
  const int64_t wave = (int64_t)blockIdx.x * 4 + (threadIdx.x >> 6), nwaves = (int64_t)gridDim.x * 4;
  for (int64_t r = wave; r < rows; r += nwaves) {
    float v[NV][E];
    float s = 0.f;
#pragma unroll
    for (int i = 0; i < NV; ++i) {
      const int64_t c = ((int64_t)i * 64 + lane) * E;
      if (c < cols) {
        Vec16<T>::load(x + r * cols + c, v[i]);
        if (x2) {
          float w[E];
          Vec16<T>::load(x2 + r * cols + c, w);
#pragma unroll
          for (int e = 0; e < E; ++e) v[i][e] += w[e];
        }
#pragma unroll
        for (int e = 0; e < E; ++e) s += v[i][e];
      }
    }
    const float mu = wave_sum(s) / (float)cols;
    float q = 0.f;
#pragma unroll
    for (int i = 0; i < NV; ++i)
      if (((int64_t)i * 64 + lane) * E < cols) {
#pragma unroll
        for (int e = 0; e < E; ++e) q += (v[i][e] - mu) * (v[i][e] - mu);
      }
    const float rs = rsqrtf(wave_sum(q) / (float)cols + eps);
    if (lane == 0) {
      mean[r] = mu;
      rstd[r] = rs;
    }
#pragma unroll
    for (int i = 0; i < NV; ++i) {
      const int64_t c = ((int64_t)i * 64 + lane) * E;
      if (c < cols) {
        float g[E], b[E], o[E];
#pragma unroll
        for (int e = 0; e < E; e += 4) {
          const float4 gg = *reinterpret_cast<const float4*>(gamma + c + e), bb = *reinterpret_cast<const float4*>(beta + c + e);
          g[e] = gg.x; g[e + 1] = gg.y; g[e + 2] = gg.z; g[e + 3] = gg.w;
          b[e] = bb.x; b[e + 1] = bb.y; b[e + 2] = bb.z; b[e + 3] = bb.w;
        }
#pragma unroll
        for (int e = 0; e < E; ++e) o[e] = (v[i][e] - mu) * rs * g[e] + b[e];
        Vec16<T>::store(y + r * cols + c, o);
      }
    }
  }
}

template <typename T, int NV>
__global__ __launch_bounds__(256) void ln_bwd_vec_guarded_kernel(const T* __restrict__ dy, const T* __restrict__ x,
                                                         const T* __restrict__ x2, const float* __restrict__ gamma,
                                                         const float* __restrict__ mean, const float* __restrict__ rstd,
                                                         T* __restrict__ dx, const T* __restrict__ dx_add,
                                                         float* __restrict__ d_gamma, float* __restrict__ d_beta, int64_t rows,
                                                         int64_t cols) {
  constexpr int E = Vec16<T>::N;
  extern __shared__ float part[];
  const int lane = threadIdx.x & 63, wid = threadIdx.x >> 6;
  const int64_t wave = (int64_t)blockIdx.x * 4 + wid, nwaves = (int64_t)gridDim.x * 4;
  float ag[NV][E], ab[NV][E], g[NV][E];
#pragma unroll
  for (int i = 0; i < NV; ++i) {
    const int64_t c = ((int64_t)i * 64 + lane) * E;
#pragma unroll
    for (int e = 0; e < E; ++e) {
      ag[i][e] = ab[i][e] = 0.f;
      g[i][e] = c < cols ? gamma[c + e] : 0.f;
    }
  }
  for (int64_t r = wave; r < rows; r += nwaves) {
    const float mu = mean[r], rs = rstd[r];
    float xh[NV][E], gy[NV][E];
    float s1 = 0.f, s2 = 0.f;
#pragma unroll
    for (int i = 0; i < NV; ++i) {
      const int64_t c = ((int64_t)i * 64 + lane) * E;
      if (c < cols) {
        float d[E];
        Vec16<T>::load(x + r * cols + c, xh[i]);
        if (x2) {
          float w[E];
          Vec16<T>::load(x2 + r * cols + c, w);
#pragma unroll
          for (int e = 0; e < E; ++e) xh[i][e] += w[e];
        }
        Vec16<T>::load(dy + r * cols + c, d);
#pragma unroll
        for (int e = 0; e < E; ++e) {
          xh[i][e] = (xh[i][e] - mu) * rs;
          gy[i][e] = d[e] * g[i][e];
          s1 += gy[i][e];
          s2 += gy[i][e] * xh[i][e];
          ag[i][e] += d[e] * xh[i][e];
          ab[i][e] += d[e];
        }
      }
    }
    const float m1 = wave_sum(s1) / (float)cols, m2 = wave_sum(s2) / (float)cols;
#pragma unroll
    for (int i = 0; i < NV; ++i) {
      const int64_t c = ((int64_t)i * 64 + lane) * E;
      if (c < cols) {
        float o[E];
#pragma unroll
        for (int e = 0; e < E; ++e) o[e] = rs * (gy[i][e] - m1 - xh[i][e] * m2);
        if (dx_add) {
          float w[E];
          Vec16<T>::load(dx_add + r * cols + c, w);
#pragma unroll
          for (int e = 0; e < E; ++e) o[e] += w[e];
        }
        Vec16<T>::store(dx + r * cols + c, o);
      }
    }
  }
  for (int w = 1; w < 4; ++w) {
    if (wid == w) {
#pragma unroll
      for (int i = 0; i < NV; ++i) {
        const int64_t c = ((int64_t)i * 64 + lane) * E;
        if (c < cols) {
#pragma unroll
          for (int e = 0; e < E; ++e) {
            part[c + e] = ag[i][e];
            part[cols + c + e] = ab[i][e];
          }
        }
      }
    }
    __syncthreads();
    if (wid == 0) {
#pragma unroll
      for (int i = 0; i < NV; ++i) {
        const int64_t c = ((int64_t)i * 64 + lane) * E;
        if (c < cols) {
#pragma unroll
          for (int e = 0; e < E; ++e) {
            ag[i][e] += part[c + e];
            ab[i][e] += part[cols + c + e];
          }
        }
      }
    }
    __syncthreads();
  }
  if (wid == 0) {
#pragma unroll
    for (int i = 0; i < NV; ++i) {
      const int64_t c = ((int64_t)i * 64 + lane) * E;
      if (c < cols) {
#pragma unroll
        for (int e = 0; e < E; ++e) {
          atomicAdd(d_gamma + c + e, ag[i][e]);
          atomicAdd(d_beta + c + e, ab[i][e]);
        }
      }
    }
  }
}

struct LnDrop {
  void* out;
  float p;
  uint64_t seed, offset;
  const CaseStepState* state;
};
template <typename T, typename V = Vec16<T>>
__device__ __forceinline__ void ln_store_dropped(const LnDrop& dr, int64_t idx, const float (&o)[V::N]) {
  constexpr int E = V::N;
  float q[E];
  if constexpr (sizeof(T) == 2) {
#pragma unroll
    for (int i = 0; i < E; i += 2) {
      const uint32_t w = f32x2_to_bf16x2(o[i], o[i + 1]);
      q[i] = __uint_as_float(w << 16);
      q[i + 1] = __uint_as_float(w & 0xffff0000u);
    }
  } else {
#pragma unroll
    for (int e = 0; e < E; ++e) q[e] = o[e];
  }
  const float scale = 1.f / (1.f - dr.p);
#pragma unroll
  for (int e = 0; e < E; e += 2) {
    float u0, u1;
    rng_uniform2(dr.seed, dr.offset + rng_base_of(dr.state) + (uint64_t)(idx + e), u0, u1);
    q[e] = u0 >= dr.p ? q[e] * scale : 0.f;
    q[e + 1] = u1 >= dr.p ? q[e + 1] * scale : 0.f;
  }
  V::store(reinterpret_cast<T*>(dr.out) + idx, q);
}

template <typename T, int NV, bool HAS_X2, bool HAS_ADD, bool DROP2 = false, typename V = Vec16<T>>
__global__ __launch_bounds__(256) void ln_bwd_vec_kernel(const T* __restrict__ dy, const T* __restrict__ x,
                                                         const T* __restrict__ x2, const float* __restrict__ gamma,
                                                         const float* __restrict__ mean, const float* __restrict__ rstd,
                                                         T* __restrict__ dx, const T* __restrict__ dx_add,
                                                         float* __restrict__ d_gamma, float* __restrict__ d_beta, int64_t rows,
                                                         int64_t cols, const LnDrop dr = LnDrop()) {
  constexpr int E = V::N;
  typedef typename V::raw raw_t;
  extern __shared__ float part[];
  const int lane = threadIdx.x & 63, wid = threadIdx.x >> 6;
  const int64_t wave = (int64_t)blockIdx.x * 4 + wid, nwaves = (int64_t)gridDim.x * 4;
  float ag[NV][E], ab[NV][E], g[NV][E];
#pragma unroll
  for (int i = 0; i < NV; ++i) {
    const int64_t c = ((int64_t)i * 64 + lane) * E;
#pragma unroll
    for (int e = 0; e < E; ++e) {
      ag[i][e] = ab[i][e] = 0.f;
      g[i][e] = gamma[c + e];
    }
  }
  struct Raw {
    raw_t x[NV], d[NV], x2[HAS_X2 ? NV : 1], add[HAS_ADD ? NV : 1];
    float mu, rs;
  };
  auto request = [&](Raw& w, int64_t r) {
    const int64_t base = r * cols + (int64_t)lane * E;
    w.mu = mean[r];
    w.rs = rstd[r];
#pragma unroll
    for (int i = 0; i < NV; ++i) {
      const int64_t o = base + (int64_t)i * 64 * E;
      w.x[i] = *reinterpret_cast<const raw_t*>(x + o);
      w.d[i] = *reinterpret_cast<const raw_t*>(dy + o);
      if constexpr (HAS_X2) w.x2[i] = *reinterpret_cast<const raw_t*>(x2 + o);
      if constexpr (HAS_ADD) w.add[i] = *reinterpret_cast<const raw_t*>(dx_add + o);
    }
  };
  auto normalised = [&](const Raw& w, int i, float (&xh)[E]) {
    V::unpack(w.x[i], xh);
    if constexpr (HAS_X2) {
      float t[E];
      V::unpack(w.x2[i], t);
#pragma unroll
      for (int e = 0; e < E; ++e) xh[e] += t[e];
    }
#pragma unroll
    for (int e = 0; e < E; ++e) xh[e] = (xh[e] - w.mu) * w.rs;
  };
  Raw cur, nxt;
  request(cur, wave < rows ? wave : rows - 1);
  for (int64_t r = wave; r < rows; r += nwaves) {
    request(nxt, r + nwaves < rows ? r + nwaves : rows - 1);
    float s1 = 0.f, s2 = 0.f;
#pragma unroll
    for (int i = 0; i < NV; ++i) {
      float xh[E], d[E];
      normalised(cur, i, xh);
      V::unpack(cur.d[i], d);
#pragma unroll
      for (int e = 0; e < E; ++e) {
        const float gy = d[e] * g[i][e];
        s1 += gy;
        s2 = fmaf(gy, xh[e], s2);
        ag[i][e] = fmaf(d[e], xh[e], ag[i][e]);
        ab[i][e] += d[e];
      }
    }
    const float m1 = wave_sum(s1) / (float)cols, m2 = wave_sum(s2) / (float)cols;
#pragma unroll
    for (int i = 0; i < NV; ++i) {
      float xh[E], d[E], o[E];
      normalised(cur, i, xh);
      V::unpack(cur.d[i], d);
#pragma unroll
      for (int e = 0; e < E; ++e) o[e] = cur.rs * fmaf(-xh[e], m2, fmaf(d[e], g[i][e], -m1));
      if constexpr (HAS_ADD) {
        float w[E];
        V::unpack(cur.add[i], w);
#pragma unroll
        for (int e = 0; e < E; ++e) o[e] += w[e];
      }
      V::store(dx + r * cols + ((int64_t)i * 64 + lane) * E, o);
      if constexpr (DROP2) ln_store_dropped<T, V>(dr, r * cols + ((int64_t)i * 64 + lane) * E, o);
    }
    cur = nxt;
  }
  float* mine = part + (int64_t)wid * 2 * cols;
#pragma unroll
  for (int i = 0; i < NV; ++i) {
    const int64_t c = ((int64_t)i * 64 + lane) * E;
#pragma unroll
    for (int e = 0; e < E; ++e) {
      mine[c + e] = ag[i][e];
      mine[cols + c + e] = ab[i][e];
    }
  }
  __syncthreads();
  for (int64_t c = threadIdx.x; c < 2 * cols; c += 256) {
    const float t = part[c] + part[2 * cols + c] + part[4 * cols + c] + part[6 * cols + c];
    atomicAdd(c < cols ? d_gamma + c : d_beta + (c - cols), t);
  }
}

template <typename T, int R, bool HAS_X2, bool HAS_ADD, bool DROP2 = false, typename V = Vec16<T>, int MAXW = 8>
__global__ __launch_bounds__(64 * MAXW) void ln_bwd_split_kernel(const T* __restrict__ dy, const T* __restrict__ x,
                                                           const T* __restrict__ x2, const float* __restrict__ gamma,
                                                           const float* __restrict__ mean, const float* __restrict__ rstd,
                                                           T* __restrict__ dx, const T* __restrict__ dx_add,
                                                           float* __restrict__ d_gamma, float* __restrict__ d_beta, int64_t rows,
                                                           int64_t cols, const LnDrop dr = LnDrop()) {
  constexpr int E = V::N;
  typedef typename V::raw raw_t;
  __shared__ float part[2][R][MAXW][2];
  const int lane = threadIdx.x & 63, wid = threadIdx.x >> 6, nw = blockDim.x >> 6;
  const int64_t col = ((int64_t)wid * 64 + lane) * E;
  float ag[E], ab[E], g[E];
#pragma unroll
  for (int e = 0; e < E; ++e) {
    ag[e] = ab[e] = 0.f;
    g[e] = gamma[col + e];
  }
  struct Raw {
    raw_t x[R], d[R], x2[HAS_X2 ? R : 1], add[HAS_ADD ? R : 1];
    float mu[R], rs[R];
  };
  auto request = [&](Raw& w, int64_t row0) {
#pragma unroll
    for (int j = 0; j < R; ++j) {
      const int64_t r = row0 + j < rows ? row0 + j : rows - 1;
      const int64_t o = r * cols + col;
      w.mu[j] = mean[r];
      w.rs[j] = rstd[r];
      w.x[j] = *reinterpret_cast<const raw_t*>(x + o);
      w.d[j] = *reinterpret_cast<const raw_t*>(dy + o);
      if constexpr (HAS_X2) w.x2[j] = *reinterpret_cast<const raw_t*>(x2 + o);
      if constexpr (HAS_ADD) w.add[j] = *reinterpret_cast<const raw_t*>(dx_add + o);
    }
  };
  auto normalised = [&](const Raw& w, int j, float (&xh)[E]) {
    V::unpack(w.x[j], xh);
    if constexpr (HAS_X2) {
      float t[E];
      V::unpack(w.x2[j], t);
#pragma unroll
      for (int e = 0; e < E; ++e) xh[e] += t[e];
    }
#pragma unroll
    for (int e = 0; e < E; ++e) xh[e] = (xh[e] - w.mu[j]) * w.rs[j];
  };
  const int64_t stride = (int64_t)gridDim.x * R;
  Raw cur, nxt;
  int buf = 0;
  if ((int64_t)blockIdx.x * R < rows) request(cur, (int64_t)blockIdx.x * R);
  for (int64_t row0 = (int64_t)blockIdx.x * R; row0 < rows; row0 += stride, buf ^= 1) {
#pragma unroll
    for (int j = 0; j < R; ++j) {
      float xh[E], d[E];
      normalised(cur, j, xh);
      V::unpack(cur.d[j], d);
      float s1 = 0.f, s2 = 0.f;
      const bool real = row0 + j < rows;
#pragma unroll
      for (int e = 0; e < E; ++e) {
        const float gy = d[e] * g[e];
        s1 += gy;
        s2 = fmaf(gy, xh[e], s2);
        if (real) {
          ag[e] = fmaf(d[e], xh[e], ag[e]);
          ab[e] += d[e];
        }
      }
      s1 = wave_sum(s1);
      s2 = wave_sum(s2);
      if (lane == 0) {
        part[buf][j][wid][0] = s1;
        part[buf][j][wid][1] = s2;
      }
    }
    if (row0 + stride < rows) request(nxt, row0 + stride);
    __syncthreads();
#pragma unroll
    for (int j = 0; j < R; ++j) {
      float m1 = 0.f, m2 = 0.f;
      for (int w = 0; w < nw; ++w) {
        m1 += part[buf][j][w][0];
        m2 += part[buf][j][w][1];
      }
      m1 /= (float)cols;
      m2 /= (float)cols;
      if (row0 + j < rows) {
        float xh[E], d[E], o[E];
        normalised(cur, j, xh);
        V::unpack(cur.d[j], d);
#pragma unroll
        for (int e = 0; e < E; ++e) o[e] = cur.rs[j] * fmaf(-xh[e], m2, fmaf(d[e], g[e], -m1));
        if constexpr (HAS_ADD) {
          float w[E];
          V::unpack(cur.add[j], w);
#pragma unroll
          for (int e = 0; e < E; ++e) o[e] += w[e];
        }
        V::store(dx + (row0 + j) * cols + col, o);
        if constexpr (DROP2) ln_store_dropped<T, V>(dr, (row0 + j) * cols + col, o);
      }
    }
    cur = nxt;
  }
  extern __shared__ float cpart[];
  __syncthreads();
#pragma unroll
  for (int e = 0; e < E; ++e) {
    cpart[col + e] = ag[e];
    cpart[cols + col + e] = ab[e];
  }
  __syncthreads();
  for (int64_t c = threadIdx.x; c < 2 * cols; c += blockDim.x) atomicAdd(c < cols ? d_gamma + c : d_beta + (c - cols), cpart[c]);
}

template <typename T>
bool ln_vec_ok(const void* a, const void* b, const void* c, int64_t cols) {
  constexpr int E = Vec16<T>::N;
  auto al = [](const void* p) { return p == nullptr || ((uintptr_t)p % 16 == 0); };
  return cols % E == 0 && cols <= (int64_t)LNV_MAX * 64 * E && al(a) && al(b) && al(c);
}

template <typename T>
void ln_fwd_vec_launch(const void* x, const void* x2, const float* gamma, const float* beta, void* y, float* mean,
                       float* rstd, int64_t rows, int64_t cols, float eps, hipStream_t s) {
  constexpr int E = Vec16<T>::N;
  const int nv = (int)((cols + 64 * E - 1) / (64 * E));
  const int grid = grid_for(rows, 4, 1, 256 * 16);
#define LNF(NVV) hipLaunchKernelGGL((ln_fwd_vec_kernel<T, NVV>), dim3(grid), dim3(256), 0, s, (const T*)x, (const T*)x2, gamma, beta, (T*)y, mean, rstd, rows, cols, eps)
  switch (nv) { case 1: LNF(1); break; case 2: LNF(2); break; case 3: LNF(3); break; case 4: LNF(4); break;
                case 5: LNF(5); break; case 6: LNF(6); break; case 7: LNF(7); break; default: LNF(8); break; }
#undef LNF
}

template <typename T>
void ln_bwd_vec_launch(const void* dy, const void* x, const void* x2, const float* gamma, const float* mean,
                       const float* rstd, void* dx, const void* dx_add, float* dg, float* db, int64_t rows, int64_t cols,
                       hipStream_t s) {
  constexpr int E = Vec16<T>::N;
  const int nv = (int)((cols + 64 * E - 1) / (64 * E));
  if constexpr (sizeof(T) == 2) {
    if (cols % 256 == 0 && cols % 512 != 0 && cols <= 1280) {
      const int grid = grid_for(rows, 4, 8, 256 * 8);
      const size_t lds = 8 * cols * sizeof(float);
#define LN8(NVV, X2, ADD) hipLaunchKernelGGL((ln_bwd_vec_kernel<T, NVV, X2, ADD, false, Vec8<T>>), dim3(grid), dim3(256), lds, s, (const T*)dy, (const T*)x, (const T*)x2, gamma, mean, rstd, (T*)dx, (const T*)dx_add, dg, db, rows, cols)
#define LN8B(NVV) do { if (x2 && dx_add) LN8(NVV, true, true); else if (x2) LN8(NVV, true, false); else if (dx_add) LN8(NVV, false, true); else LN8(NVV, false, false); } while (0)
      if (cols == 256) LN8B(1);
      else if (cols == 768) LN8B(3);
      else LN8B(5);
#undef LN8B
#undef LN8
      return;
    }
    if (cols % 256 == 0 && cols % 512 != 0 && cols <= 15 * 256) {
      constexpr int R = 2;
      const int nw = (int)(cols / 256);
      const int grid = grid_for(rows, 1, R * 16, 256 * 4);
#define LNS8(X2, ADD) hipLaunchKernelGGL((ln_bwd_split_kernel<T, R, X2, ADD, false, Vec8<T>, 16>), dim3(grid), dim3(64 * nw), 2 * cols * sizeof(float), s, (const T*)dy, (const T*)x, (const T*)x2, gamma, mean, rstd, (T*)dx, (const T*)dx_add, dg, db, rows, cols)
      if (x2 && dx_add) LNS8(true, true);
      else if (x2) LNS8(true, false);
      else if (dx_add) LNS8(false, true);
      else LNS8(false, false);
#undef LNS8
      return;
    }
  }
  if (cols != (int64_t)nv * 64 * E || nv > 8) {
    const int grid = grid_for(rows, 4, 16, 256 * 4);
    const size_t lds = 2 * cols * sizeof(float);
#define LNG(NVV) hipLaunchKernelGGL((ln_bwd_vec_guarded_kernel<T, NVV>), dim3(grid), dim3(256), lds, s, (const T*)dy, (const T*)x, (const T*)x2, gamma, mean, rstd, (T*)dx, (const T*)dx_add, dg, db, rows, cols)
    switch (nv) { case 1: LNG(1); break; case 2: LNG(2); break; case 3: LNG(3); break; case 4: LNG(4); break;
                  case 5: LNG(5); break; case 6: LNG(6); break; case 7: LNG(7); break; default: LNG(8); break; }
#undef LNG
    return;
  }
  if (nv >= 3) {
    constexpr int R = 2;
    const int grid = grid_for(rows, 1, R * 16, 256 * 4);
#define LNS(X2, ADD) hipLaunchKernelGGL((ln_bwd_split_kernel<T, R, X2, ADD>), dim3(grid), dim3(64 * nv), 2 * cols * sizeof(float), s, (const T*)dy, (const T*)x, (const T*)x2, gamma, mean, rstd, (T*)dx, (const T*)dx_add, dg, db, rows, cols)
    if (x2 && dx_add) LNS(true, true);
    else if (x2) LNS(true, false);
    else if (dx_add) LNS(false, true);
    else LNS(false, false);
#undef LNS
    return;
  }
  const int grid = grid_for(rows, 4, 8, 256 * 8);
  const size_t lds = 8 * cols * sizeof(float);
#define LNB(NVV, X2, ADD) hipLaunchKernelGGL((ln_bwd_vec_kernel<T, NVV, X2, ADD>), dim3(grid), dim3(256), lds, s, (const T*)dy, (const T*)x, (const T*)x2, gamma, mean, rstd, (T*)dx, (const T*)dx_add, dg, db, rows, cols)
#define LNB2(NVV) do { if (x2 && dx_add) LNB(NVV, true, true); else if (x2) LNB(NVV, true, false); else if (dx_add) LNB(NVV, false, true); else LNB(NVV, false, false); } while (0)
  if (nv == 1) LNB2(1);
  else LNB2(2);
#undef LNB2
#undef LNB
}

template <int TPR>
__device__ __forceinline__ float row_max(float v, float* red) {
  if constexpr (TPR == 64) return wave_max(v);
  else return block_max(v, red);
}
template <int TPR>
__device__ __forceinline__ float row_sum(float v, float* red) {
  if constexpr (TPR == 64) return wave_sum(v);
  else return block_sum(v, red);
}

template <typename TI, typename TO, int TPR>
__global__ __launch_bounds__(256) void softmax_fwd_kernel(const CaseSoftmaxDesc d, const TI* __restrict__ x,
                                                          const uint8_t* __restrict__ col_valid,
                                                          const uint8_t* __restrict__ row_valid, TO* __restrict__ p_out,
                                                          TO* __restrict__ y_out) {
  __shared__ float red[32];
  const int rows_per_block = 256 / TPR;
  const int sub = threadIdx.x / TPR, t = threadIdx.x % TPR;
  const int64_t total = d.outer * d.inner * d.R;
  const float keep_scale = d.drop_p > 0.f ? 1.f / (1.f - d.drop_p) : 1.f;
  const uint32_t thr = rng_threshold(d.drop_p);
  for (int64_t base = (int64_t)blockIdx.x * rows_per_block; base < total; base += (int64_t)gridDim.x * rows_per_block) {
    const int64_t row = base + sub;
    const bool live = row < total;
    const int64_t rr = live ? row : 0;
    const int64_t r = rr % d.R, o = rr / (d.R * d.inner);
    const TI* xr = x + rr * d.C;
    const uint8_t* cv = col_valid ? col_valid + o * d.C : nullptr;
    const bool row_ok = live && (!row_valid || row_valid[o * d.R + r]);
    const int64_t cmax = d.causal ? (r + 1 < d.C ? r + 1 : d.C) : d.C;
    float m = -INFINITY;
    if (row_ok)
      for (int64_t c = t; c < cmax; c += TPR)
        if (!cv || cv[c]) m = fmaxf(m, Elem<TI>::ld(xr + c));
    m = row_max<TPR>(m, red);
    float s = 0.f;
    if (row_ok && m > -INFINITY)
      for (int64_t c = t; c < cmax; c += TPR)
        if (!cv || cv[c]) s += expf(Elem<TI>::ld(xr + c) - m);
    s = row_sum<TPR>(s, red);
    if (!live) continue;
    const float inv = s > 0.f ? 1.f / s : 0.f;
    const uint32_t rkey = d.drop_p > 0.f ? rng_row_key(d.seed, d.offset + rng_base_of(d.state) + (uint64_t)rr) : 0u;
    for (int64_t c = t; c < d.C; c += TPR) {
      float p = 0.f;
      if (row_ok && c < cmax && (!cv || cv[c]) && inv > 0.f) p = expf(Elem<TI>::ld(xr + c) - m) * inv;
      Elem<TO>::st(p_out + rr * d.C + c, p);
      if (d.drop_p > 0.f) Elem<TO>::st(y_out + rr * d.C + c, attn_keep(rkey, (uint32_t)c, thr) ? p * keep_scale : 0.f);
    }
  }
}

template <typename TI, typename TO, int TPR>
__global__ __launch_bounds__(256) void softmax_bwd_kernel(const CaseSoftmaxDesc d, const TO* __restrict__ dy,
                                                          const TO* __restrict__ p, TI* __restrict__ dx) {
  __shared__ float red[32];
  const int rows_per_block = 256 / TPR;
  const int sub = threadIdx.x / TPR, t = threadIdx.x % TPR;
  const int64_t total = d.outer * d.inner * d.R;
  const float keep_scale = d.drop_p > 0.f ? 1.f / (1.f - d.drop_p) : 1.f;
  const uint32_t thr = rng_threshold(d.drop_p);
  for (int64_t base = (int64_t)blockIdx.x * rows_per_block; base < total; base += (int64_t)gridDim.x * rows_per_block) {
    const int64_t row = base + sub;
    const bool live = row < total;
    const int64_t rr = live ? row : 0;
    const uint32_t rkey = d.drop_p > 0.f ? rng_row_key(d.seed, d.offset + rng_base_of(d.state) + (uint64_t)rr) : 0u;
    float dot = 0.f;
    if (live)
      for (int64_t c = t; c < d.C; c += TPR) {
        float g = Elem<TO>::ld(dy + rr * d.C + c);
        if (d.drop_p > 0.f) g = attn_keep(rkey, (uint32_t)c, thr) ? g * keep_scale : 0.f;
        dot += g * Elem<TO>::ld(p + rr * d.C + c);
      }
    dot = row_sum<TPR>(dot, red);
    if (!live) continue;
    for (int64_t c = t; c < d.C; c += TPR) {
      float g = Elem<TO>::ld(dy + rr * d.C + c);
      if (d.drop_p > 0.f) g = attn_keep(rkey, (uint32_t)c, thr) ? g * keep_scale : 0.f;
      const float pv = Elem<TO>::ld(p + rr * d.C + c);
      Elem<TI>::st(dx + rr * d.C + c, pv * (g - dot));
// ... 351 lines not shown
        float w[E];
        Vec16<T>::unpack(av[p], w);
#pragma unroll
        for (int e = 0; e < E; ++e) o[e] += w[e];
      }
      Vec16<T>::unpack(make_uint4(f32x2_to_bf16x2(o[0], o[1]), f32x2_to_bf16x2(o[2], o[3]), f32x2_to_bf16x2(o[4], o[5]), f32x2_to_bf16x2(o[6], o[7])),
                       og[p]);
    }
    float ev[E], x1[E], x2[E], oe[E], o1[E], o2[E];
    Vec16<T>::unpack(xv[0], ev);
    Vec16<T>::unpack(xv[1], x1);
    Vec16<T>::unpack(xv[2], x2);
#pragma unroll
    for (int e = 0; e < E; ++e) {
      oe[e] = ok ? og[0][e] + og[3][e] * x1[e] + og[4][e] * x2[e] : 0.f;
      o1[e] = ok ? og[1][e] + og[3][e] * ev[e] : 0.f;
      o2[e] = ok ? og[2][e] + og[4][e] * ev[e] : 0.f;
    }
    Vec16<T>::store(de + r * H + pc, oe);
    Vec16<T>::store(da1 + r * H + pc, o1);
    Vec16<T>::store(da2 + r * H + pc, o2);
  }
  for (int w = 0; w < 4; ++w) {
    __syncthreads();
    if (wid == w) {
#pragma unroll
      for (int p = 0; p < 5; ++p)
#pragma unroll
        for (int e = 0; e < E; ++e) {
          const int c = p * H + pc + e;
          sh[c] = (w == 0 ? 0.f : sh[c]) + ag[p][e];
          sh[COLS + c] = (w == 0 ? 0.f : sh[COLS + c]) + ab[p][e];
        }
    }
  }
  __syncthreads();
  for (int c = threadIdx.x; c < 2 * COLS; c += 256) atomicAdd(c < COLS ? d_gamma + c : d_beta + (c - COLS), sh[c]);
}

extern "C" int case_layernorm_bwd_concat5(const void* dy, const void* x, const float* gamma, const float* mean, const float* rstd,
                                          const void* dx_add, const void* e, const void* a1, const void* a2, const uint8_t* row_valid, void* de,
                                          void* da1, void* da2, float* d_gamma, float* d_beta, int64_t rows, int64_t H, int32_t dtype,
                                          case_stream_t stream) {
  CASE_REQUIRE(dy && x && gamma && mean && rstd && e && a1 && a2 && row_valid && de && da1 && da2 && d_gamma && d_beta && rows > 0,
               "case_layernorm_bwd_concat5: bad argument");
  if (dtype != CASE_BF16 || H != 512)
    return case_set_error(CASE_E_UNSUPPORTED, "case_layernorm_bwd_concat5: built for bf16 rows of 5 x 512 (run case_layernorm_bwd + case_concat5_bwd)");
  for (const void* p : {dy, x, dx_add, (const void*)de, (const void*)da1, (const void*)da2})
    CASE_REQUIRE((reinterpret_cast<uintptr_t>(p) & 15) == 0, "case_layernorm_bwd_concat5: tensors must be 16-byte aligned");
  (void)e; (void)a1; (void)a2;
  hipStream_t s = (hipStream_t)stream;
  const int grid_r = grid_for(rows, 4, 8, 256 * 8);
  if (dx_add)
    hipLaunchKernelGGL(ln_bwd_concat5_rows_kernel<true>, dim3(grid_r), dim3(256), 0, s, (const bf16_t*)dy, (const bf16_t*)x, gamma, mean, rstd,
                       (const bf16_t*)dx_add, row_valid, (bf16_t*)de, (bf16_t*)da1, (bf16_t*)da2, d_gamma, d_beta, rows);
  else
    hipLaunchKernelGGL(ln_bwd_concat5_rows_kernel<false>, dim3(grid_r), dim3(256), 0, s, (const bf16_t*)dy, (const bf16_t*)x, gamma, mean, rstd,
                       (const bf16_t*)nullptr, row_valid, (bf16_t*)de, (bf16_t*)da1, (bf16_t*)da2, d_gamma, d_beta, rows);
  return case_check_launch("case_layernorm_bwd_concat5");
}

extern "C" int case_layernorm_bwd_dropout(const void* dy, const void* x, const float* gamma, const float* mean, const float* rstd, void* dx,
                                          void* dx_dropped, float* d_gamma, float* d_beta, int64_t rows, int64_t cols, float p, uint64_t seed,
                                          uint64_t offset, const CaseStepState* state, int32_t dtype, case_stream_t stream) {
  CASE_REQUIRE(dy && x && gamma && mean && rstd && dx && dx_dropped && d_gamma && d_beta && rows > 0 && cols > 0 && p > 0.f && p < 1.f,
               "case_layernorm_bwd_dropout: bad argument");
  CASE_REQUIRE((offset & 1) == 0, "case_layernorm_bwd_dropout: the RNG offset must be even (the mask is drawn per element pair)");
  const LnDrop dr = {dx_dropped, p, seed, offset, state};
  hipStream_t s = (hipStream_t)stream;
  bool ok = false;
  if (dtype == CASE_F32 && ln_vec_ok<float>(dy, x, dx, cols) && ln_vec_ok<float>(dx_dropped, nullptr, nullptr, cols))
    ok = ln_bwd_drop_launch<float>(dy, x, gamma, mean, rstd, dx, d_gamma, d_beta, rows, cols, dr, s);
  else if (dtype == CASE_BF16 && ln_vec_ok<bf16_t>(dy, x, dx, cols) && ln_vec_ok<bf16_t>(dx_dropped, nullptr, nullptr, cols))
    ok = ln_bwd_drop_launch<bf16_t>(dy, x, gamma, mean, rstd, dx, d_gamma, d_beta, rows, cols, dr, s);
  if (!ok)
    return case_set_error(CASE_E_UNSUPPORTED, "case_layernorm_bwd_dropout: needs 16-byte aligned rows of a whole number of 64-lane chunks "
                                              "(cols = %d x k, k <= 8); run case_layernorm_bwd + case_dropout", dtype == CASE_BF16 ? 512 : 256);
  return case_check_launch("case_layernorm_bwd_dropout");
}

extern "C" int case_layernorm_bwd(const void* dy, const void* x, const void* x2, const float* gamma, const float* mean,
                                  const float* rstd, void* dx, const void* dx_add, float* d_gamma, float* d_beta,
                                  int64_t rows, int64_t cols, int32_t dtype, case_stream_t stream) {
  CASE_REQUIRE(dy && x && gamma && mean && rstd && dx && d_gamma && d_beta && rows > 0 && cols > 0,
               "case_layernorm_bwd: bad argument");
  CASE_REQUIRE(cols <= (int64_t)LN_THREADS * LN_MAXPT, "case_layernorm_bwd: cols %lld > %d", (long long)cols,
               LN_THREADS * LN_MAXPT);
  const int grid = grid_for(rows, 1, 8, 256 * 2);
  hipStream_t s = (hipStream_t)stream;
  if (dtype == CASE_F32 && ln_vec_ok<float>(dy, x, dx, cols) && ln_vec_ok<float>(x2, dx_add, nullptr, cols)) {
    ln_bwd_vec_launch<float>(dy, x, x2, gamma, mean, rstd, dx, dx_add, d_gamma, d_beta, rows, cols, s);
    return case_check_launch("case_layernorm_bwd");
  }
  if (dtype == CASE_BF16 && ln_vec_ok<bf16_t>(dy, x, dx, cols) && ln_vec_ok<bf16_t>(x2, dx_add, nullptr, cols)) {
    ln_bwd_vec_launch<bf16_t>(dy, x, x2, gamma, mean, rstd, dx, dx_add, d_gamma, d_beta, rows, cols, s);
    return case_check_launch("case_layernorm_bwd");
  }
  if (dtype == CASE_F32)
    hipLaunchKernelGGL(ln_bwd_kernel<float>, dim3(grid), dim3(LN_THREADS), 0, s, (const float*)dy, (const float*)x,
                       (const float*)x2, gamma, mean, rstd, (float*)dx, (const float*)dx_add, d_gamma, d_beta, rows, cols);
  else
    hipLaunchKernelGGL(ln_bwd_kernel<bf16_t>, dim3(grid), dim3(LN_THREADS), 0, s, (const bf16_t*)dy, (const bf16_t*)x,
                       (const bf16_t*)x2, gamma, mean, rstd, (bf16_t*)dx, (const bf16_t*)dx_add, d_gamma, d_beta, rows, cols);
  return case_check_launch("case_layernorm_bwd");
}

extern "C" int case_softmax_fwd(const CaseSoftmaxDesc* d, const void* x, const uint8_t* col_valid,
                                const uint8_t* row_valid, void* p_out, void* y_out, case_stream_t stream) {
  CASE_REQUIRE(d && x && p_out && d->outer > 0 && d->inner > 0 && d->R > 0 && d->C > 0, "case_softmax_fwd: bad argument");
  CASE_REQUIRE(d->drop_p == 0.f || y_out, "case_softmax_fwd: dropout needs y_out");
  CASE_REQUIRE(d->drop_p >= 0.f && d->drop_p < 1.f, "case_softmax_fwd: drop_p out of range");
  return softmax_dispatch<true>(d, x, col_valid, row_valid, p_out, y_out, (hipStream_t)stream);
}

extern "C" int case_softmax_bwd(const CaseSoftmaxDesc* d, const void* dy, const void* p, void* dx, case_stream_t stream) {
  CASE_REQUIRE(d && dy && p && dx && d->outer > 0 && d->inner > 0 && d->R > 0 && d->C > 0, "case_softmax_bwd: bad argument");
  return softmax_dispatch<false>(d, dy, nullptr, nullptr, (void*)p, dx, (hipStream_t)stream);
}
```

### case_rg_amd/ops.py

```python
import math
import ctypes as C
import os

import torch
from torch.autograd import Function

from . import _abi as A
from . import config, paramcache

_DT = {torch.float32: A.F32, torch.bfloat16: A.BF16}


def _code(t):
    try:
        return _DT[t.dtype]
    except KeyError:
        raise TypeError("case_rg_amd: unsupported activation dtype %s" % t.dtype)


_raw_stream, _cur_device = getattr(torch._C, "_cuda_getCurrentRawStream", None), getattr(torch._C, "_cuda_getDevice", None)


def _stream():
    if _raw_stream is not None and _cur_device is not None:
# ... 28 lines not shown

def cast_param(p, dtype):
    if p.dtype == dtype:
        return p.detach().contiguous()
    base = getattr(p, "_base", None)
    owner = p if isinstance(p, torch.nn.Parameter) else (base if isinstance(base, torch.nn.Parameter) else None)
    if owner is None:
        return cast(p.detach(), dtype)
    owners, tag = (owner,), paramcache.cast_tag(p, dtype)
    hit = paramcache.peek(owners, tag)
    if hit is not None:
        return hit
    if owner is not p and p.is_contiguous() and owner.is_contiguous():
        whole = paramcache.peek(owners, paramcache.cast_tag(owner, dtype))
        if whole is not None:
            return whole.as_strided(p.shape, p.stride(), p.storage_offset() - owner.storage_offset())
    return paramcache.derived(owners, tag, lambda: cast(p.detach(), dtype))


def cast(x, dtype):
    if x.dtype == dtype:
        return x
    x = x.contiguous()
    out = torch.empty(x.shape, dtype=dtype, device=x.device)
    A.call("case_cast", _ptr(x), _ptr(out), x.numel(), _code(x), _DT[dtype], _stream())
    return out


ENCODER_CHAIN = "auto"


def encoder_chain_supported(x, width, ffn_width, needs_grad):
    return (ENCODER_CHAIN == "auto" and x.is_cuda and x.dtype == torch.bfloat16 and width == 512 and ffn_width == 512
            and not needs_grad)


def _chain_pack(mats):
    def build():
        low = [None if m is None else cast_param(m, torch.bfloat16) for m in mats]
        packed = torch.empty(A.lib.case_encoder_chain_packed_bytes() // 2, dtype=torch.bfloat16, device=next(m for m in mats if m is not None).device)
        A.call("case_encoder_chain_pack", _ptr(low[0]), _ptr(low[1]), _ptr(low[2]), _ptr(low[3]), _ptr(packed), _stream())
        return packed

    return paramcache.derived(mats, "chain", build)


def encoder_chain(variant, x_in, resid, layer, next_layer):
    M = x_in.shape[0] * x_in.shape[1]
    dev = x_in.device
    f32 = lambda p: None if p is None else p.detach()
    lay = None if variant == "head" else layer
    nxt = None if variant == "tail" else next_layer
    packed = _chain_pack((None if lay is None else lay.self_attn.out_proj.weight, None if lay is None else lay.linear1.weight,
                          None if lay is None else lay.linear2.weight, None if nxt is None else nxt.self_attn.in_proj_weight))
    d = A.EncoderChainDesc()
    d.rows, d.width, d.variant = M, 512, {"full": 0, "tail": 1, "head": 2}[variant]
    d.eps_ln2 = 0.0 if lay is None else lay.norm2.eps
    d.eps_ln1_next = 0.0 if nxt is None else nxt.norm1.eps
    s_out = torch.empty(x_in.shape, dtype=torch.bfloat16, device=dev)
    qkv = None if nxt is None else torch.empty(x_in.shape[0], x_in.shape[1], 1536, dtype=torch.bfloat16, device=dev)
    x_in = x_in if x_in.is_contiguous() else x_in.contiguous()
    if resid is not None and not resid.is_contiguous():
        resid = resid.contiguous()
    A.call("case_encoder_chain", d, _ptr(x_in), _ptr(resid), _ptr(packed),
           _ptr(None if lay is None else f32(lay.self_attn.out_proj.bias)), _ptr(None if lay is None else f32(lay.linear1.bias)),
           _ptr(None if lay is None else f32(lay.linear2.bias)), _ptr(None if nxt is None else f32(nxt.self_attn.in_proj_bias)),
           _ptr(None if lay is None else f32(lay.norm2.weight)), _ptr(None if lay is None else f32(lay.norm2.bias)),
           _ptr(None if nxt is None else f32(nxt.norm1.weight)), _ptr(None if nxt is None else f32(nxt.norm1.bias)),
           _ptr(s_out), _ptr(qkv), _stream())
    return s_out, qkv


GEMM_TILE = 0
AUX_STREAMS = {}


TILE_TRACE = None
DECODE_MIN_PAIRS = 192
FUSE_BIAS_GRAD = True


def gemm(a, b, c, M, N, K, lda, ldb, ldc, *, a_off=0, b_off=0, c_off=0, a_kmajor=False, b_kmajor=False,
         batch1=1, batch2=1, sa=(0, 0), sb=(0, 0), sc=(0, 0), alpha=1.0, epilogue=0, bias_col=None, bias_row=None,
         aux=None, aux_out=None, ld_aux=0, saux=(0, 0), split_k=1, drop=None, rowsum_out=None):
    d = A.GemmDesc()
    d.M, d.N, d.K, d.lda, d.ldb, d.ldc, d.ld_aux = M, N, K, lda, ldb, ldc, ld_aux
    d.batch1, d.batch2 = batch1, batch2
    d.sa1, d.sa2 = sa
    d.sb1, d.sb2 = sb
    d.sc1, d.sc2 = sc
    d.saux1, d.saux2 = saux
    d.a_kmajor, d.b_kmajor = int(a_kmajor), int(b_kmajor)
    d.in_dtype, d.out_dtype = _code(a), _code(c)
    d.tile = GEMM_TILE
    if b.dtype != a.dtype:
        raise TypeError("gemm operands differ in dtype: %s vs %s" % (a.dtype, b.dtype))
    for name, t in (("aux", aux), ("aux_out", aux_out)):
        if t is not None and t.dtype != a.dtype:
            raise TypeError("gemm %s must have the operand dtype %s, got %s" % (name, a.dtype, t.dtype))
    for name, t in (("bias_col", bias_col), ("bias_row", bias_row)):
        if t is not None and t.dtype != torch.float32:
            raise TypeError("gemm %s must be float32, got %s" % (name, t.dtype))
    if drop is not None and drop[0] > 0.0:
        epilogue |= A.EPI_DROPOUT
        d.drop_p, d.seed, d.offset, d.state = _drop4(drop)
    d.epilogue, d.split_k, d.alpha = epilogue, split_k, alpha
    if TILE_TRACE is not None:
        TILE_TRACE.append(A.lib.case_gemm_tile_for(d, _ptr(a, a_off), _ptr(b, b_off), _ptr(c, c_off), _ptr(bias_col), _ptr(aux),
                                                   _ptr(aux_out)))
    if rowsum_out is not None:
        if not (a_kmajor and epilogue == A.EPI_ATOMIC and lda == M and batch1 * batch2 == 1 and a_off == 0):
            raise ValueError("rowsum_out needs an unbatched k-major contiguous A and the bare ATOMIC epilogue")
        if FUSE_BIAS_GRAD and a.dtype == torch.bfloat16 and A.lib.case_gemm_tile_for(d, _ptr(a), _ptr(b, b_off), _ptr(c, c_off), None, None, None) == 256:
            if not _dw_slabs(d, a, b, b_off, c, c_off, rowsum_out):
                A.call("case_gemm_dw_bias", d, _ptr(a), _ptr(b, b_off), _ptr(c, c_off), _ptr(rowsum_out), _stream())
            return c
        A.call("case_colsum", _ptr(a), _ptr(rowsum_out), K, M, _code(a), _stream())
    elif (epilogue == A.EPI_ATOMIC and split_k >= DW_SLAB_MIN_SPLIT and a.dtype == torch.bfloat16 and batch1 * batch2 == 1 and a_off == 0
          and A.lib.case_gemm_tile_for(d, _ptr(a), _ptr(b, b_off), _ptr(c, c_off), None, None, None) == 256 and _dw_slabs(d, a, b, b_off, c, c_off, None)):
        return c
    A.call("case_gemm", d, _ptr(a, a_off), _ptr(b, b_off), _ptr(c, c_off), _ptr(bias_col), _ptr(bias_row), _ptr(aux),
           _ptr(aux_out), _stream())
    return c


DW_SLAB_MIN_SPLIT = int(os.environ.get("CASE_DW_SLAB_MIN_SPLIT", "8"))
DW_SLAB_MAX_BYTES = 256 << 20


def _dw_slabs(d, a, b, b_off, c, c_off, rowsum_out):
    if DW_SLAB_MIN_SPLIT <= 0 or d.split_k < DW_SLAB_MIN_SPLIT or d.ldc != d.N:
        return False
    need = A.lib.case_gemm_dw_slab_bytes(d)
    if need <= 0 or need > DW_SLAB_MAX_BYTES:
        return False
    ws = torch.empty(need, dtype=torch.uint8, device=c.device)
    A.call("case_gemm_dw_slabs", d, _ptr(a), _ptr(b, b_off), _ptr(c, c_off), _ptr(rowsum_out), _ptr(ws), need, _stream())
    return True


def _split_for(out_rows, out_cols, k_len, elem_bytes):
    k_tiles = max(1, (k_len * elem_bytes + 127) // 128)
    tiles256 = (out_rows // 256) * (out_cols // 256)
    if (elem_bytes == 2 and out_rows % 256 == 0 and out_cols % 256 == 0 and k_len % 64 == 0 and k_tiles >= 64
            and tiles256 * min(64, k_tiles // 8) >= 230):
        tiles = tiles256
        cus = max(8, (256 - int(A.lib.case_get_reserved_cus())) // 8 * 8)
        best, best_score = 1, -1.0
        for split in range(1, 65):
            if split > 1 and k_tiles // split < 8:
                break
            wgs = tiles * split
            eff = wgs / float(((wgs + cus - 1) // cus) * cus)
            score = eff - (0.012 if tiles >= 64 else 0.004) * split - (0.5 if wgs < 0.9 * cus else 0.0)
            if score > best_score:
                best, best_score = split, score
        return best
    tiles = ((out_rows + 127) // 128) * ((out_cols + 127) // 128)
    if elem_bytes == 2 and out_rows % 64 == 0 and out_cols % 64 == 0 and k_len % 64 == 0 and tiles < 128:
        t64 = (out_rows // 64) * (out_cols // 64)
        need = (k_tiles + 9) // 10
        want = max(need, (256 + t64 - 1) // t64)
        split = min(want, k_tiles, max(need, 512 // t64))
        if (k_tiles + split - 1) // split <= 10 and t64 * split <= 512:
            return max(1, split)
    min_k_tiles = 8 if tiles >= 128 else 2
    best, best_eff = 1, 0.0
    for split in range(1, 65):
        if split > 1 and k_tiles // split < min_k_tiles:
            break
        wgs = tiles * split
        eff = wgs / (((wgs + 511) // 512) * 512.0)
        if wgs >= 1024 and eff >= 0.92:
            return split
        if eff > best_eff + 1e-9:
            best, best_eff = split, eff
    return best


class _ZeroArena:
    ENABLED = os.environ.get("CASE_ZERO_ARENA", "1") != "0"
    ALIGN = 64

    def __init__(self):
        self.epoch, self.buf, self.pos, self.served, self.want, self.device = -1, None, 0, 0, 0, None

    def take(self, n, device):
        if not self.ENABLED or not torch.device(device).type == "cuda":
# ... 177 lines not shown
        wv = w.detach().reshape(-1).float().contiguous()
        bv = None if b is None else b.detach().reshape(-1).float().contiguous()
        y = torch.empty(x2.shape[0], dtype=torch.float32, device=x2.device)
        A.call("case_rowdot_fwd", _ptr(x2), _ptr(wv), _ptr(bv), _ptr(y), x2.shape[0], C, _code(x2), _stream())
        ctx.save_for_backward(x2, wv)
        ctx.meta = (x.shape, w.shape, b is not None)
        return y.view(*x.shape[:-1], 1)

    @staticmethod
    def backward(ctx, g):
        x2, wv = ctx.saved_tensors
        xshape, wshape, has_b = ctx.meta
        R, C = x2.shape
        g = g.reshape(-1).float().contiguous()
        dx = torch.empty_like(x2) if ctx.needs_input_grad[0] else None
        dw, db = _zeros_like_shapes(x2.device, (C,), (1,))
        db = db if has_b else None
        A.call("case_rowdot_bwd", _ptr(g), _ptr(x2), _ptr(wv), _ptr(dx), _ptr(dw), _ptr(db), R, C, _code(x2), _stream())
        return (None if dx is None else dx.view(xshape)), dw.view(wshape), db


def linear_carry(x, w, b=None):
    return LinearFn.apply(x, w, b, None, 0.0, None, True)


def linear(x, w, b=None, residual=None, p_drop=0.0, out_dtype=None, ln=None):
    if ln is not None:
        if LN_TAIL and out_dtype is None:
            return LinearFn.apply(x, w, b, residual, p_drop, None, False, ln[0], ln[1], ln[2])
        return layer_norm(linear(x, w, b, residual, p_drop, out_dtype), ln[0], ln[1], ln[2])
    if w.shape[0] == 1 and residual is None and p_drop == 0.0 and out_dtype in (None, torch.float32) and (
            out_dtype is torch.float32 or x.dtype == torch.float32):
        return RowDotFn.apply(x, w, b)
    return LinearFn.apply(x, w, b, residual, p_drop, out_dtype)


LN_GEMM = os.environ.get("CASE_LN_GEMM", "off")


def ln_gemm_supported(x, out_features):
    return (LN_GEMM == "on" and x.is_cuda and x.dtype == torch.bfloat16 and x.shape[-1] == 512 and (x.numel() // 512) % 64 == 0
            and out_features % 64 == 0 and not torch.is_grad_enabled() and bool(A.lib.case_abi_features() & A.FEAT_GEMM_LN))


def ln_linear(x, ln, w, b=None, act=None, residual=None):
    gamma, beta, eps = ln
    N = w.shape[0]
    if not ln_gemm_supported(x, N):
        xn = layer_norm(x, gamma, beta, eps)
        if act is not None:
            raise RuntimeError("ln_linear: an activation needs case_gemm_ln (check ln_gemm_supported; ops.ffn is the general path)")
        return linear(xn, w, b, residual=residual), xn
    x2 = x.reshape(-1, 512)
    x2 = x2 if x2.is_contiguous() else x2.contiguous()
    M = x2.shape[0]
    wc = cast_param(w, torch.bfloat16)
    y = torch.empty(M, N, dtype=torch.bfloat16, device=x.device)
    xn = torch.empty_like(x2)
    d = A.GemmDesc()
    d.M, d.N, d.K, d.lda, d.ldb, d.ldc, d.ld_aux = M, N, 512, 512, 512, N, N
    d.batch1 = d.batch2 = 1
    d.in_dtype, d.out_dtype, d.split_k, d.alpha, d.tile = A.BF16, A.BF16, 1, 1.0, 64
    epi = 0
    if b is not None:
        epi |= A.EPI_BIAS_COL
    if act == "gelu":
        epi |= A.EPI_GELU
    elif act == "relu":
        epi |= A.EPI_RELU
    elif act is not None:
        raise ValueError("ln_linear: activation %r" % (act,))
    res2 = None
    if residual is not None:
        res2 = residual.reshape(M, N)
        res2 = res2 if res2.is_contiguous() else res2.contiguous()
        epi |= A.EPI_RESIDUAL
    d.epilogue = epi
    g32, b32 = gamma.detach().float().contiguous(), beta.detach().float().contiguous()
    A.call("case_gemm_ln", d, _ptr(x2), _ptr(g32), _ptr(b32), float(eps), _ptr(xn), _ptr(wc), _ptr(y), _ptr(None if b is None else b.detach()),
           _ptr(res2), _stream())
    return y.view(*x.shape[:-1], N), xn.view(x.shape)


class FFNFn(Function):
    @staticmethod
    def forward(ctx, x, w1, b1, w2, b2, act, p_inner, p_out, residual, ln_g=None, ln_b=None, ln_eps=0.0):
        K, F_, N = x.shape[-1], w1.shape[0], w2.shape[0]
        x2 = x.reshape(-1, K)
        if not x2.is_contiguous():
            x2 = x2.contiguous()
        M = x2.shape[0]
        w1c, w2c = cast_param(w1, x2.dtype), cast_param(w2, x2.dtype)
        a = torch.empty(M, F_, dtype=x2.dtype, device=x2.device)
        z = torch.empty_like(a) if act == "gelu" else None
        drop_i = drop_o = None
        if p_inner > 0.0:
            drop_i = (p_inner,) + config.next_rng(M * F_)
        if p_out > 0.0:
            drop_o = (p_out,) + config.next_rng(M * N)
        gemm(x2, w1c, a, M, F_, K, K, K, F_, epilogue=A.EPI_BIAS_COL | (A.EPI_GELU if act == "gelu" else A.EPI_RELU),
             bias_col=b1, aux_out=z, ld_aux=F_, drop=drop_i)
        y = torch.empty(M, N, dtype=x2.dtype, device=x2.device)
        res2, epi = None, A.EPI_BIAS_COL
        if residual is not None:
            res2 = residual.reshape(M, N).contiguous()
            epi |= A.EPI_RESIDUAL
        gemm(a, w2c, y, M, N, F_, F_, F_, N, epilogue=epi, bias_col=b2, aux=res2, ld_aux=N, drop=drop_o)
        ctx.meta = (x.shape, act, drop_i, drop_o, residual is not None, residual is x and N == K)
        if ln_g is not None:
            n, g_, mean, rstd = _ln_tail_forward(y, (ln_g, ln_b, ln_eps))
            ctx.save_for_backward(x2, w1c, w2c, a, z, y, g_, mean, rstd)
            return n.view(*x.shape[:-1], N)
        ctx.save_for_backward(x2, w1c, w2c, a, z)
        return y.view(*x.shape[:-1], N)

    @staticmethod
    def backward(ctx, dy):
        xshape, act, drop_i, drop_o, has_res, res_is_x = ctx.meta
        d_lng = d_lnb = None
        if len(ctx.saved_tensors) == 9:
            x2, w1c, w2c, a, z, y, g_, mean, rstd = ctx.saved_tensors
            M, K = x2.shape
            F_, N = w1c.shape[0], w2c.shape[0]
            g_res, g, d_lng, d_lnb = _ln_tail_backward(dy, y, g_, mean, rstd, drop_o)
            dy = g_res.view(*xshape[:-1], N)
            fuse_res = res_is_x and ctx.needs_input_grad[0]
            d_res = dy if (has_res and not fuse_res) else None
        else:
            x2, w1c, w2c, a, z = ctx.saved_tensors
            M, K = x2.shape
            F_, N = w1c.shape[0], w2c.shape[0]
            g = dy.reshape(M, N)
            if not g.is_contiguous():
                g = g.contiguous()
            fuse_res = res_is_x and ctx.needs_input_grad[0] and g.dtype == x2.dtype
            d_res = dy if (has_res and not fuse_res) else None
            g_res = g
            if drop_o is not None:
                g = _dropout_raw(g, *drop_o)
        dw1, db1, dw2, db2 = _zeros_like_shapes(g.device, (F_, K), (F_,), (N, F_), (N,))
        _weight_grad(g, a, N, F_, out=dw2, bias_out=db2)
        dz = torch.empty(M, F_, dtype=x2.dtype, device=x2.device)
        if act == "gelu":
            gemm(g, w2c, dz, M, F_, N, N, F_, F_, b_kmajor=True, epilogue=A.EPI_MUL_DGELU, aux=z, ld_aux=F_, drop=drop_i)
        else:
            gemm(g, w2c, dz, M, F_, N, N, F_, F_, b_kmajor=True, epilogue=A.EPI_MUL_DRELU, aux=a, ld_aux=F_, drop=drop_i)
        _weight_grad(dz, x2, F_, K, out=dw1, bias_out=db1)
        dx = None
        if ctx.needs_input_grad[0]:
            dx = torch.empty(M, K, dtype=x2.dtype, device=x2.device)
            if fuse_res:
                gemm(dz, w1c, dx, M, K, F_, F_, K, K, b_kmajor=True, epilogue=A.EPI_RESIDUAL, aux=g_res, ld_aux=N)
            else:
                gemm(dz, w1c, dx, M, K, F_, F_, K, K, b_kmajor=True)
            dx = dx.view(xshape)
        return dx, dw1, db1, dw2, db2, None, None, None, d_res, d_lng, d_lnb, None


def ffn(x, w1, b1, w2, b2, act, p_inner=0.0, p_out=0.0, residual=None, ln=None):
    if ln is not None:
        if LN_TAIL:
            return FFNFn.apply(x, w1, b1, w2, b2, act, p_inner, p_out, residual, ln[0], ln[1], ln[2])
        return layer_norm(FFNFn.apply(x, w1, b1, w2, b2, act, p_inner, p_out, residual), ln[0], ln[1], ln[2])
    return FFNFn.apply(x, w1, b1, w2, b2, act, p_inner, p_out, residual)


class LayerNormFn(Function):

    @staticmethod
    def forward(ctx, x, x2, gamma, beta, eps, carry=False):
        C = x.shape[-1]
        xa = x.reshape(-1, C)
        xa = xa if xa.is_contiguous() else xa.contiguous()
        xb = None
        if x2 is not None:
            xb = x2.reshape(-1, C)
            xb = xb if xb.is_contiguous() else xb.contiguous()
        R = xa.shape[0]
        y = torch.empty_like(xa)
        mean = torch.empty(R, dtype=torch.float32, device=xa.device)
        rstd = torch.empty_like(mean)
        g, b = gamma.detach().contiguous(), beta.detach().contiguous()
        A.call("case_layernorm_fwd", _ptr(xa), _ptr(xb), _ptr(g), _ptr(b), _ptr(y), _ptr(mean), _ptr(rstd), R, C, eps,
               _code(xa), _stream())
        ctx.save_for_backward(xa, xb, g, mean, rstd)
        ctx.shape = x.shape
        if carry:
            return y.view(x.shape), x.view_as(x)
        return y.view(x.shape)

    @staticmethod
    def backward(ctx, dy, d_carry=None):
        xa, xb, g, mean, rstd = ctx.saved_tensors
        R, C = xa.shape
        dy2 = dy.reshape(R, C)
        dy2 = dy2 if dy2.is_contiguous() else dy2.contiguous()
        extra = None
        if d_carry is not None:
            extra = d_carry.reshape(R, C).to(xa.dtype)
            extra = extra if extra.is_contiguous() else extra.contiguous()
        dx = torch.empty_like(xa)
        dg, db = _zeros_like_shapes(xa.device, (C,), (C,))
        A.call("case_layernorm_bwd", _ptr(dy2), _ptr(xa), _ptr(xb), _ptr(g), _ptr(mean), _ptr(rstd), _ptr(dx), _ptr(extra),
               _ptr(dg), _ptr(db), R, C, _code(xa), _stream())
        dx = dx.view(ctx.shape)
        return dx, (dx if xb is not None else None), dg, db, None, None


def layer_norm(x, gamma, beta, eps=1e-5, add=None):
    return LayerNormFn.apply(x, add, gamma, beta, eps)


def layer_norm_carry(x, gamma, beta, eps=1e-5):
    return LayerNormFn.apply(x, None, gamma, beta, eps, True)


def _softmax_desc(outer, inner, R, C, causal, in_dt, out_dt, drop):
    d = A.SoftmaxDesc()
    d.outer, d.inner, d.R, d.C = outer, inner, R, C
    d.causal, d.in_dtype, d.out_dtype = int(causal), in_dt, out_dt
    d.drop_p, d.seed, d.offset, d.state = _drop4(drop)
    return d


class SoftmaxFn(Function):
    @staticmethod
    def forward(ctx, x, col_valid, row_valid, outer, causal, p_drop, out_dtype):
        R, C = x.shape[-2], x.shape[-1]
        xc = x if x.is_contiguous() else x.contiguous()
        inner = xc.numel() // (outer * R * C)
        odt = out_dtype or xc.dtype
        p = torch.empty(xc.shape, dtype=odt, device=xc.device)
        drop, y = None, p
        if p_drop > 0.0:
            drop = (p_drop,) + config.next_rng(xc.numel())
            y = torch.empty_like(p)
        d = _softmax_desc(outer, inner, R, C, causal, _code(xc), _DT[odt], drop)
        A.call("case_softmax_fwd", d, _ptr(xc), _ptr(col_valid), _ptr(row_valid), _ptr(p), _ptr(y), _stream())
        ctx.save_for_backward(p)
        ctx.meta = (outer, inner, R, C, causal, xc.dtype, odt, drop)
        return y

    @staticmethod
    def backward(ctx, dy):
        (p,) = ctx.saved_tensors
        outer, inner, R, C, causal, idt, odt, drop = ctx.meta
        dyc = cast(dy, odt)
        dyc = dyc if dyc.is_contiguous() else dyc.contiguous()
        dx = torch.empty(p.shape, dtype=idt, device=p.device)
        d = _softmax_desc(outer, inner, R, C, causal, _DT[idt], _DT[odt], drop)
        A.call("case_softmax_bwd", d, _ptr(dyc), _ptr(p), _ptr(dx), _stream())
        return dx, None, None, None, None, None, None


def masked_softmax(x, col_valid=None, row_valid=None, outer=1, causal=False, p_drop=0.0, out_dtype=None):
    return SoftmaxFn.apply(x, _u8(col_valid), _u8(row_valid), outer, causal, p_drop, out_dtype)


def _src_key(t):
    return (t.data_ptr(), tuple(t.shape), tuple(t.stride()))


ATTENTION_MODE = "auto"
SCORES_FUSED = os.environ.get("CASE_SCORES_FUSED", "1") != "0"
_FUSED_TRAINING = (32, 64, 96, 160)
_FUSED_INFERENCE = (32, 64, 96, 160, 320)
INFER_320 = os.environ.get("CASE_INFER_320", "slab")


def _fused_ok(q_src, k_src, v_src, q_off, k_off, v_off, d, needs_grad=True):
    if ATTENTION_MODE == "unfused" or q_src.dtype != torch.bfloat16 or not A.lib.case_attention_supported(d):
        return False
    if ATTENTION_MODE == "auto":
        if d not in (_FUSED_TRAINING if needs_grad else _FUSED_INFERENCE):
            return False
        if not needs_grad and d == 320 and INFER_320 == "scores" and SCORES_FUSED and k_src.shape[1] <= 384 and k_src.shape[1] % 8 == 0:
            return False
    for t, off in ((q_src, q_off), (k_src, k_off), (v_src, v_off)):
        if t.shape[2] % 8 or off % 8 or t.data_ptr() % 16:
            return False
    return True


def _kv_splits(N, heads, Lq, Lk, causal):
    wgs = N * heads * ((Lq + 127) // 128)
    if causal or wgs >= 512 or Lk < 2048:
        return 1
    return max(1, min(Lk // 960, (512 + wgs - 1) // wgs * (2 if wgs >= 128 else 1), 64))


def _attn_desc(N, heads, Lq, Lk, d, q_src, k_src, v_src, causal, alpha, drop):
    ad = A.AttnDesc()
    ad.N, ad.heads, ad.Lq, ad.Lk, ad.head_dim = N, heads, Lq, Lk, d
    ad.ldq, ad.ldk, ad.ldv = q_src.shape[2], k_src.shape[2], v_src.shape[2]
    ad.sq, ad.sk, ad.sv = Lq * q_src.shape[2], Lk * k_src.shape[2], Lk * v_src.shape[2]
    ad.ldo, ad.so = heads * d, Lq * heads * d
    ad.causal, ad.scale = int(causal), alpha
# ... 1079 lines not shown
```

### include/case_hip.h

```cpp
#ifndef CASE_HIP_H
#define CASE_HIP_H

#include <stddef.h>
#include <stdint.h>

#ifdef __cplusplus
extern "C" {
#endif

typedef void* case_stream_t;

typedef enum { CASE_F32 = 0, CASE_BF16 = 1 } case_dtype_t;

enum {
  CASE_OK = 0,
  CASE_E_ARG = -1,
  CASE_E_UNSUPPORTED = -2,
  CASE_E_LAUNCH = -3
};

#define CASE_ABI_VERSION 600
int case_version(void);
enum {
  CASE_FEAT_GEMM_256 = 1u << 0,
  CASE_FEAT_GEMM_SMALL = 1u << 1,
  CASE_FEAT_ENCODER_CHAIN = 1u << 2,
  CASE_FEAT_ATTN_SCORES = 1u << 3,
  CASE_FEAT_ATTN_DECODE = 1u << 4,
  CASE_FEAT_OPTIM = 1u << 5,
  CASE_FEAT_ATTN_RESIDENT = 1u << 6,
  CASE_FEAT_RESERVED_CUS = 1u << 7,
  CASE_FEAT_GEMM_DW_SLABS = 1u << 8,
  CASE_FEAT_DECODER_CHAIN = 1u << 9,
  CASE_FEAT_ATTN_DECODE_MQA = 1u << 10,
  CASE_FEAT_POINTER_DECODE = 1u << 11,
  CASE_FEAT_POINTER_HEAD = 1u << 12,
  CASE_FEAT_GEMM_LN = 1u << 13,
  CASE_FEAT_STEP_STATE = 1u << 14,
  CASE_FEAT_INTERACTION = 1u << 15,
  CASE_FEAT_ATTN_DECODE_APPEND = 1u << 16,
  CASE_FEAT_LINEAR_SKINNY = 1u << 17
};
uint32_t case_abi_features(void);
const char* case_last_error(void);

typedef struct {
  uint64_t rng_base;
  float step_size;
  float bc2_sqrt;
  float lr;
  int32_t step;
  uint64_t reserved[5];
} CaseStepState;
int case_sizeof_step_state(void);
int case_step_advance(CaseStepState* state, uint64_t rng_stride, double beta1, double beta2, case_stream_t stream);

int case_set_reserved_cus(int n);
int case_get_reserved_cus(void);

typedef enum { CASE_WS_ATTENTION_SPLITKV = 1, CASE_WS_ATTENTION_BWD = 2, CASE_WS_OPTIM_SUMSQ = 3, CASE_WS_ENCODER_CHAIN_PACK = 4, CASE_WS_GEMM_DW_SLABS = 5 } case_workspace_kind_t;
int64_t case_workspace_bytes(int32_t kind, const void* desc, int64_t arg);

enum {
  CASE_EPI_BIAS_COL = 1,
  CASE_EPI_BIAS_ROW = 2,
  CASE_EPI_GELU = 4,
  CASE_EPI_RELU = 8,
  CASE_EPI_RESIDUAL = 16,
  CASE_EPI_MUL_DGELU = 32,
  CASE_EPI_MUL_DRELU = 64,
  CASE_EPI_ATOMIC = 128,
  CASE_EPI_DROPOUT = 256
};

typedef struct {
  int64_t M, N, K;
  int64_t lda, ldb, ldc, ld_aux;
  int64_t batch1, batch2;
  int64_t sa1, sa2, sb1, sb2, sc1, sc2, saux1, saux2;
  int32_t a_kmajor, b_kmajor;
  int32_t in_dtype;
  int32_t out_dtype;
  int32_t epilogue;
  int32_t split_k;
  int32_t tile;
  float alpha;
  float drop_p;
  uint64_t seed, offset;
  const CaseStepState* state;
} CaseGemmDesc;

int case_gemm(const CaseGemmDesc* d, const void* A, const void* B, void* C, const float* bias_col,
              const float* bias_row, const void* aux, void* aux_out, case_stream_t stream);
int case_gemm_ln(const CaseGemmDesc* d, const void* A, const float* gamma, const float* beta, float eps, void* ln_out, const void* B, void* C,
                 const float* bias_col, const void* aux, case_stream_t stream);

int case_gemm_dw_bias(const CaseGemmDesc* d, const void* A, const void* B, void* C, float* d_bias, case_stream_t stream);
int case_gemm_dw_slabs(const CaseGemmDesc* d, const void* A, const void* B, void* C, float* d_bias, void* slabs, int64_t slab_bytes,
                       case_stream_t stream);
int64_t case_gemm_dw_slab_bytes(const CaseGemmDesc* d);

int case_gemm_tile_for(const CaseGemmDesc* d, const void* A, const void* B, const void* C, const float* bias_col,
                       const void* aux, const void* aux_out);

int case_embed_pos_fwd(const int64_t* ids, const float* table, const float* pe, void* out, int64_t rows,
                       int64_t seq_len, int64_t H, int64_t vocab, float scale, float drop_p, uint64_t seed,
                       uint64_t offset, const CaseStepState* state, int32_t dtype, case_stream_t stream);
int case_embed_pos_bwd(const int64_t* ids, const void* d_out, float* d_table, int64_t rows, int64_t H,
                       int64_t vocab, float scale, float drop_p, uint64_t seed, uint64_t offset, const CaseStepState* state,
                       int32_t dtype, case_stream_t stream);

int case_scale_add_rows(const void* x, const float* pe, void* y, int64_t rows, int64_t seq_len, int64_t H, float scale,
                        int32_t dtype, case_stream_t stream);

int case_layernorm_fwd(const void* x, const void* x2, const float* gamma, const float* beta, void* y, float* mean,
                       float* rstd, int64_t rows, int64_t cols, float eps, int32_t dtype, case_stream_t stream);
int case_layernorm_bwd(const void* dy, const void* x, const void* x2, const float* gamma, const float* mean,
                       const float* rstd, void* dx, const void* dx_add, float* d_gamma, float* d_beta, int64_t rows,
                       int64_t cols, int32_t dtype, case_stream_t stream);
int case_layernorm_bwd_dropout(const void* dy, const void* x, const float* gamma, const float* mean, const float* rstd, void* dx,
                               void* dx_dropped, float* d_gamma, float* d_beta, int64_t rows, int64_t cols, float p, uint64_t seed,
                               uint64_t offset, const CaseStepState* state, int32_t dtype, case_stream_t stream);
int case_layernorm_bwd_concat5(const void* dy, const void* x, const float* gamma, const float* mean, const float* rstd, const void* dx_add,
                               const void* e, const void* a1, const void* a2, const uint8_t* row_valid, void* de, void* da1, void* da2,
                               float* d_gamma, float* d_beta, int64_t rows, int64_t H, int32_t dtype, case_stream_t stream);

typedef struct {
  int64_t outer, inner, R, C;
  int32_t causal;
  int32_t in_dtype, out_dtype;
  float drop_p;
  uint64_t seed, offset;
  const CaseStepState* state;
} CaseSoftmaxDesc;

int case_softmax_fwd(const CaseSoftmaxDesc* d, const void* x, const uint8_t* col_valid, const uint8_t* row_valid,
                     void* p_out, void* y_out, case_stream_t stream);
int case_softmax_bwd(const CaseSoftmaxDesc* d, const void* dy, const void* p, void* dx, case_stream_t stream);

typedef struct {
  int64_t N, heads, Lq, Lk, head_dim;
  int64_t ldq, ldk, ldv, sq, sk, sv;
  int64_t ldo, so;
  int32_t causal;
  float scale, drop_p;
  uint64_t seed, offset;
  const CaseStepState* state;
} CaseAttnDesc;

int case_attention_supported(int64_t head_dim);
int case_attention_fwd(const CaseAttnDesc* d, const void* q, const void* k, const void* v, const uint8_t* key_valid,
                       void* out, float* lse, case_stream_t stream);
int case_attention_splitkv_workspace(const CaseAttnDesc* d, int32_t ksplit, int64_t* bytes);
int case_attention_fwd_splitkv(const CaseAttnDesc* d, const void* q, const void* k, const void* v, const uint8_t* key_valid,
                               void* out, float* lse, void* workspace, int64_t workspace_bytes, int32_t ksplit,
                               case_stream_t stream);
int case_attention_decode_supported(int64_t head_dim);
int case_attention_decode(const CaseAttnDesc* d, const void* q, const void* k, const void* v, const uint8_t* key_valid,
                          void* out, case_stream_t stream);
int case_attention_decode_append(const CaseAttnDesc* d, const void* q, void* k_cache, void* v_cache, const void* new_k, const void* new_v,
                                 int64_t new_stride, int64_t pos, const uint8_t* key_valid, void* out, case_stream_t stream);
int64_t case_attention_decode_mqa_workspace(int64_t B, int64_t S, int32_t nsplit);
int case_attention_decode_mqa_splits(int64_t B, int64_t S);
int case_attention_decode_mqa(const void* qp, const void* mem, const uint8_t* key_valid, void* out, int64_t B, int64_t S, int64_t ldo,
                              int32_t nsplit, void* workspace, int64_t workspace_bytes, case_stream_t stream);
int case_attention_bwd_supported(int64_t head_dim);
int64_t case_attention_bwd_scratch_floats(const CaseAttnDesc* d);
int case_attention_bwd(const CaseAttnDesc* d, const void* q, const void* k, const void* v, const uint8_t* key_valid,
                       const void* out, const float* lse, const void* dout, float* delta, void* dq, void* dk, void* dv,
                       case_stream_t stream);

int case_attention_scores_supported(const CaseAttnDesc* d);
int case_attention_scores_fwd(const CaseAttnDesc* d, const void* q, const void* k, const uint8_t* key_valid, void* p,
                              void* p_dropped, case_stream_t stream);
int case_attention_scores_bwd(const CaseAttnDesc* d, const void* dout, const void* v, const void* p, void* ds,
                              case_stream_t stream);
typedef struct {
  int64_t N, heads, M, Kc, head_dim;
  int64_t lda, sa_seq, sa_head;
  int64_t ldb, sb_seq, sb_head;
  int64_t ldc, sc_seq, sc_head;
  int32_t a_transposed;
  float alpha;
} CaseAttnProductDesc;
int case_attention_product_supported(const CaseAttnProductDesc* d);
int case_attention_product(const CaseAttnProductDesc* d, const void* a, const void* b, void* c, case_stream_t stream);

int case_add(const void* a, const void* b, void* out, int64_t n, int32_t dtype, case_stream_t stream);
int case_add_n(const void* const* srcs, int32_t count, void* out, int64_t n, int32_t dtype, case_stream_t stream);
int case_dropout(const void* x, void* y, int64_t n, float p, uint64_t seed, uint64_t offset, const CaseStepState* state,
                 int32_t dtype, case_stream_t stream);
int case_mask_rows(const void* x, const uint8_t* row_valid, void* y, int64_t rows, int64_t cols, int32_t dtype,
                   case_stream_t stream);
int case_colsum(const void* x, float* out, int64_t rows, int64_t cols, int32_t dtype, case_stream_t stream);
int case_cast(const void* x, void* y, int64_t n, int32_t src_dtype, int32_t dst_dtype, case_stream_t stream);
int case_scale_cols(const void* x, const float* w, void* y, int64_t rows, int64_t cols, int32_t dtype,
                    case_stream_t stream);
int case_scale_cols_bwd(const void* dy, const void* x, const float* w, void* dx, float* dw, int64_t rows,
                        int64_t cols, int32_t dtype, case_stream_t stream);
int case_rowdot_fwd(const void* x, const float* w, const float* b, float* y, int64_t rows, int64_t cols, int32_t dtype,
                    case_stream_t stream);
int case_rowdot_bwd(const float* g, const void* x, const float* w, void* dx, float* dw, float* db, int64_t rows,
// ... 94 lines not shown
```

Baseline: 1.342 million tokens/s.

## Fuse FFN output row masking into GEMM epilogue and next-layer LayerNorm backward

Adds a ROW_MASK epilogue to the GEMM kernels so the FFN output is zeroed for padded rows inside the second FFN GEMM, instead of a separate mask_rows pass. The backward mask on the gradient is pushed into the next block's LayerNorm backward through a promise object, with a fallback mask kernel when no consumer takes it. This removes an elementwise read and write pass per encoder layer in forward and backward. It adds a new epilogue template variant and a cross-module promise mechanism that assumes the LayerNorm is the only consumer of the block output.

```diff
diff --git a/case_rg_amd/_abi.py b/case_rg_amd/_abi.py
--- a/case_rg_amd/_abi.py
+++ b/case_rg_amd/_abi.py
@@ -6,14 +6,14 @@
 _HERE = os.path.dirname(os.path.abspath(__file__))
 LIB_PATH = os.environ.get("CASE_HIP_LIB") or os.path.join(_HERE, "csrc", "libcase_hip.so")
 
-ABI_VERSION = 600
+ABI_VERSION = 610
 F32, BF16 = 0, 1
 WS_ATTENTION_SPLITKV, WS_ATTENTION_BWD, WS_OPTIM_SUMSQ, WS_ENCODER_CHAIN_PACK, WS_GEMM_DW_SLABS = 1, 2, 3, 4, 5
 (FEAT_GEMM_256, FEAT_GEMM_SMALL, FEAT_ENCODER_CHAIN, FEAT_ATTN_SCORES, FEAT_ATTN_DECODE, FEAT_OPTIM, FEAT_ATTN_RESIDENT, FEAT_RESERVED_CUS,
  FEAT_GEMM_DW_SLABS, FEAT_DECODER_CHAIN, FEAT_ATTN_DECODE_MQA, FEAT_POINTER_DECODE, FEAT_POINTER_HEAD, FEAT_GEMM_LN, FEAT_STEP_STATE,
  FEAT_INTERACTION, FEAT_ATTN_DECODE_APPEND, FEAT_LINEAR_SKINNY) = (1 << i for i in range(18))
 EPI_BIAS_COL, EPI_BIAS_ROW, EPI_GELU, EPI_RELU = 1, 2, 4, 8
-EPI_RESIDUAL, EPI_MUL_DGELU, EPI_MUL_DRELU, EPI_ATOMIC, EPI_DROPOUT = 16, 32, 64, 128, 256
+EPI_RESIDUAL, EPI_MUL_DGELU, EPI_MUL_DRELU, EPI_ATOMIC, EPI_DROPOUT, EPI_ROW_MASK = 16, 32, 64, 128, 256, 512
 
 i32, i64, u64, f32, f64, ptr = C.c_int32, C.c_int64, C.c_uint64, C.c_float, C.c_double, C.c_void_p
 
@@ -22,7 +22,7 @@
     _fields_ = [(n, i64) for n in ("M", "N", "K", "lda", "ldb", "ldc", "ld_aux", "batch1", "batch2",
                                    "sa1", "sa2", "sb1", "sb2", "sc1", "sc2", "saux1", "saux2")] + \
                [(n, i32) for n in ("a_kmajor", "b_kmajor", "in_dtype", "out_dtype", "epilogue", "split_k", "tile")] + \
-               [("alpha", f32), ("drop_p", f32), ("seed", u64), ("offset", u64), ("state", ptr)]
+               [("alpha", f32), ("drop_p", f32), ("seed", u64), ("offset", u64), ("state", ptr), ("row_mask", ptr)]
 
 
 class StepState(C.Structure):
@@ -61,6 +61,7 @@
     "case_scale_add_rows": [ptr, ptr, ptr, i64, i64, i64, f32, i32, ptr],
     "case_layernorm_fwd": [ptr, ptr, ptr, ptr, ptr, ptr, ptr, i64, i64, f32, i32, ptr],
     "case_layernorm_bwd": [ptr, ptr, ptr, ptr, ptr, ptr, ptr, ptr, ptr, ptr, i64, i64, i32, ptr],
+    "case_layernorm_bwd_masked": [ptr] * 11 + [i64, i64, i32, ptr],
     "case_layernorm_bwd_dropout": [ptr, ptr, ptr, ptr, ptr, ptr, ptr, ptr, ptr, i64, i64, f32, u64, u64, ptr, i32, ptr],
     "case_layernorm_bwd_concat5": [ptr] * 15 + [i64, i64, i32, ptr],
     "case_softmax_fwd": [C.POINTER(SoftmaxDesc), ptr, ptr, ptr, ptr, ptr, ptr],
diff --git a/case_rg_amd/common/TransformerBlock.py b/case_rg_amd/common/TransformerBlock.py
--- a/case_rg_amd/common/TransformerBlock.py
+++ b/case_rg_amd/common/TransformerBlock.py
@@ -22,8 +22,9 @@
         else:
             raise NotImplementedError("TransformerBlock on the HIP path supports relu (reference default) or gelu")
 
-    def forward(self, input, input_mask):
+    def forward(self, input, input_mask, sole_consumer=False):
         B, N, L, E = input.shape
+        promise = ops.row_mask_promise(input) if sole_consumer else None
         x = input.reshape(B * N, L, E)
         valid = input_mask.reshape(B * N, L)
         p = config.drop_p(0.1, self.training)
@@ -32,10 +33,14 @@
             if fused is not None:
                 n1, xres = fused[0].reshape(B * N, L, E), fused[1].reshape(B * N, L, E)
             else:
-                n1, xres = ops.layer_norm_carry(x, self.norm1.weight, self.norm1.bias, self.norm1.eps)
+                n1, xres = ops.layer_norm_carry(x, self.norm1.weight, self.norm1.bias, self.norm1.eps, promise=promise)
         else:
             n1, xres = ops.layer_norm(x, self.norm1.weight, self.norm1.bias, self.norm1.eps), x
         n2 = self.self_attn.self_attention(n1, valid, residual=xres, p_res=0.1, ln=(self.norm2.weight, self.norm2.bias, self.norm2.eps))
+        if ops.ROW_MASK_FUSED and torch.is_grad_enabled() and n2.requires_grad:
+            y = ops.ffn(n2, self.linear1.weight, self.linear1.bias, self.linear2.weight, self.linear2.bias,
+                        self.activation, p_inner=p, p_out=0.0, row_valid=valid)
+            return ops.carry_row_mask_promise(y, y.reshape(B, N, L, self.output_hidden_size))
         y = ops.ffn(n2, self.linear1.weight, self.linear1.bias, self.linear2.weight, self.linear2.bias,
                     self.activation, p_inner=p, p_out=0.0)
         y = ops.mask_rows(y, valid, in_place=True)
diff --git a/case_rg_amd/common/heads.py b/case_rg_amd/common/heads.py
--- a/case_rg_amd/common/heads.py
+++ b/case_rg_amd/common/heads.py
@@ -15,8 +15,8 @@
 
 
 def run_blocks(blocks, reps, mask):
-    for block in blocks:
-        reps = block(reps, mask)
+    for i, block in enumerate(blocks):
+        reps = block(reps, mask, sole_consumer=i > 0)
     return reps
 
 
diff --git a/case_rg_amd/csrc/gemm.hip b/case_rg_amd/csrc/gemm.hip
--- a/case_rg_amd/csrc/gemm.hip
+++ b/case_rg_amd/csrc/gemm.hip
@@ -22,6 +22,7 @@
   float* slabs;
   int64_t slab_stride;
   const float* ln_gamma; const float* ln_beta; void* ln_out; float ln_eps;
+  const uint8_t* row_mask;
 };
 
 #define GEMM_NS gemm_w4
@@ -57,6 +58,8 @@
                "case_gemm: split_k > 1 needs CASE_EPI_ATOMIC and f32 output");
   CASE_REQUIRE(!((epi & CASE_EPI_RESIDUAL) && (epi & (CASE_EPI_MUL_DGELU | CASE_EPI_MUL_DRELU))),
                "case_gemm: RESIDUAL and MUL_D* share the aux operand and cannot be combined");
+  CASE_REQUIRE(!(epi & CASE_EPI_ROW_MASK) || (d->row_mask && !(epi & CASE_EPI_ATOMIC)),
+               "case_gemm: ROW_MASK needs row_mask and cannot be combined with split-K accumulation");
   CASE_REQUIRE(!(epi & CASE_EPI_DROPOUT) || (d->drop_p > 0.f && d->drop_p < 1.f), "case_gemm: drop_p out of range");
   CASE_REQUIRE(!(epi & CASE_EPI_ATOMIC) ||
                    !(epi & (CASE_EPI_GELU | CASE_EPI_RELU | CASE_EPI_RESIDUAL | CASE_EPI_MUL_DGELU | CASE_EPI_MUL_DRELU |
@@ -87,6 +90,7 @@
   a.ln_gamma = a.ln_beta = nullptr;
   a.ln_out = nullptr;
   a.ln_eps = 0.f;
+  a.row_mask = (epi & CASE_EPI_ROW_MASK) ? d->row_mask : nullptr;
   a.drop_p = d->drop_p; a.seed = d->seed; a.offset = d->offset; a.state = d->state;
   auto aligned = [&](const void* p, int64_t ld, int64_t s1, int64_t s2, int64_t extent) {
     return ((uintptr_t)p % 16 == 0) && (ld % ept == 0) && (s1 % ept == 0) && (s2 % ept == 0) && (extent % ept == 0);
@@ -104,7 +108,8 @@
   *tile = 128;
   if (d->tile != 128 && d->in_dtype == CASE_BF16 && d->batch1 * d->batch2 == 1 && d->M % 256 == 0 && d->N % 256 == 0 && d->K % 64 == 0 &&
       a.vec_a && a.vec_b && a.vec_c && d->lda < (1 << 22) && d->ldb < (1 << 22) && d->ldc < (1 << 22) && d->ld_aux < (1 << 22) &&
-      (!(epi & CASE_EPI_ATOMIC) || (epi == CASE_EPI_ATOMIC && d->out_dtype == CASE_F32))) {
+      (!(epi & CASE_EPI_ATOMIC) || (epi == CASE_EPI_ATOMIC && d->out_dtype == CASE_F32)) &&
+      (!(epi & CASE_EPI_ROW_MASK) || (epi == (CASE_EPI_BIAS_COL | CASE_EPI_ROW_MASK) && (uintptr_t)a.row_mask % 8 == 0))) {
     const int64_t t256 = (d->M / 256) * (d->N / 256) * a.split_k;
     const bool span_ok = (!d->a_kmajor || (d->K / a.split_k + 64) * d->lda < (1ll << 30)) &&
                          (!d->b_kmajor || (d->K / a.split_k + 64) * d->ldb < (1ll << 30));
diff --git a/case_rg_amd/csrc/gemm8w.inc b/case_rg_amd/csrc/gemm8w.inc
--- a/case_rg_amd/csrc/gemm8w.inc
+++ b/case_rg_amd/csrc/gemm8w.inc
@@ -127,8 +127,9 @@
 template <int ECT, typename OutT>
 __device__ __forceinline__ void drain_pass(const Args& g, const int epi_rt, const float* strip, const int le, const int p,
                                            const int64_t row_w, const int64_t col_w, const float (&bc)[8], const u32x4 (&ax)[4],
-                                           const __amdgpu_buffer_rsrc_t rc, const __amdgpu_buffer_rsrc_t ro) {
+                                           const uint64_t (&mw)[4], const __amdgpu_buffer_rsrc_t rc, const __amdgpu_buffer_rsrc_t ro) {
   const int E = ECT >= 0 ? ECT : epi_rt;
+  constexpr bool RMASK = ECT >= 0 && (ECT & CASE_EPI_ROW_MASK);
   const int cc = (le & 7) * 8;
   const bool need_aux = E & (CASE_EPI_RESIDUAL | CASE_EPI_MUL_DGELU | CASE_EPI_MUL_DRELU);
   const float drop_scale = (E & CASE_EPI_DROPOUT) ? 1.f / (1.f - g.drop_p) : 1.f;
@@ -191,15 +192,25 @@
       for (int e = 0; e < 8; ++e) x[e] += a8[e];
     }
     const int sc = (int)(rb * g.ldc * (int64_t)sizeof(OutT));
+    bool keep = true;
+    if constexpr (RMASK) keep = ((mw[s] >> (le & 56)) & 0xffull) != 0ull;
     if constexpr (sizeof(OutT) == 2) {
       u32x4 w;
 #pragma unroll
       for (int i = 0; i < 4; ++i) w[i] = f32x2_to_bf16x2(x[2 * i], x[2 * i + 1]);
+      if constexpr (RMASK) {
+#pragma unroll
+        for (int i = 0; i < 4; ++i) w[i] = keep ? w[i] : 0u;
+      }
       __builtin_amdgcn_raw_buffer_store_b128(w, rc, vc + sc, 0, 0);
     } else {
       u32x4 w0, w1;
 #pragma unroll
       for (int i = 0; i < 4; ++i) { w0[i] = __float_as_uint(x[i]); w1[i] = __float_as_uint(x[4 + i]); }
+      if constexpr (RMASK) {
+#pragma unroll
+        for (int i = 0; i < 4; ++i) { w0[i] = keep ? w0[i] : 0u; w1[i] = keep ? w1[i] : 0u; }
+      }
       __builtin_amdgcn_raw_buffer_store_b128(w0, rc, vc + sc, 0, 0);
       __builtin_amdgcn_raw_buffer_store_b128(w1, rc, vc + sc + 16, 0, 0);
     }
@@ -210,6 +221,7 @@
 __device__ __forceinline__ void epilogue_tile(const Args& g, const int epi_rt, float* strip, const int le, const int64_t row_w,
                                               const int64_t col_w, const f32x4 (&acc)[8][4], void* const cbase) {
   const int E = ECT >= 0 ? ECT : epi_rt;
+  constexpr bool RMASK = ECT >= 0 && (ECT & CASE_EPI_ROW_MASK);
   const bool need_aux = E & (CASE_EPI_RESIDUAL | CASE_EPI_MUL_DGELU | CASE_EPI_MUL_DRELU);
   float bc[8] = {0.f, 0.f, 0.f, 0.f, 0.f, 0.f, 0.f, 0.f};
   if (E & CASE_EPI_BIAS_COL) Epilogue<bf16_t, OutT>::load8(g.bias_col + col_w + (le & 7) * 8, bc);
@@ -221,12 +233,19 @@
   const __amdgpu_buffer_rsrc_t ro = __builtin_amdgcn_make_buffer_rsrc((void*)auxo, 0, auxo ? -1 : 0, 0x00020000);
   const int va = (int)(((le >> 3) * g.ld_aux + (le & 7) * 8) * 2);
   const int lr = le & 15, lg = le >> 4;
+  typedef const __attribute__((address_space(4))) uint64_t* mask_words_t;
+  const mask_words_t maskw = RMASK ? (mask_words_t)(uintptr_t)uniform_ptr(g.row_mask + row_w) : (mask_words_t)0;
 #pragma unroll
   for (int p = 0; p < 4; ++p) {
     u32x4 ax[4];
     if (need_aux) {
 #pragma unroll
       for (int s = 0; s < 4; ++s) ax[s] = __builtin_amdgcn_raw_buffer_load_b128(ra, va + (int)((p * 32 + s * 8) * g.ld_aux * 2), 0, G8_AUX_POLICY);
+    }
+    uint64_t mw[4] = {0ull, 0ull, 0ull, 0ull};
+    if constexpr (RMASK) {
+#pragma unroll
+      for (int k = 0; k < 4; ++k) mw[k] = maskw[p * 4 + k];
     }
 #pragma unroll
     for (int ii = 0; ii < 2; ++ii)
@@ -235,7 +254,7 @@
         *reinterpret_cast<f32x4*>(strip + (ii * 16 + lr) * 64 + (((j * 4 + lg) ^ lr) * 4)) = acc[2 * p + ii][j];
     asm volatile("" ::: "memory");
     __builtin_amdgcn_sched_barrier(0);
-    drain_pass<ECT, OutT>(g, epi_rt, strip, le, p, row_w, col_w, bc, ax, rc, ro);
+    drain_pass<ECT, OutT>(g, epi_rt, strip, le, p, row_w, col_w, bc, ax, mw, rc, ro);
     asm volatile("" ::: "memory");
     __builtin_amdgcn_sched_barrier(0);
   }
@@ -326,6 +345,11 @@
       if (E & CASE_EPI_RESIDUAL) {
 #pragma unroll
         for (int e = 0; e < 8; ++e) x[e] += a8[e];
+      }
+      if constexpr (ECT >= 0 && (ECT & CASE_EPI_ROW_MASK)) {
+        const bool keep = g.row_mask[row] != 0;
+#pragma unroll
+        for (int e = 0; e < 8; ++e) x[e] = keep ? x[e] : 0.f;
       }
       const int sc = (int)((16 * i * g.ldc + 32 * p) * (int64_t)sizeof(OutT));
       if constexpr (sizeof(OutT) == 2) {
@@ -632,7 +656,7 @@
     } else {
       float* strip = reinterpret_cast<float*>(smem + (wave < 4 ? STAGE + wave * STRIP : 2 * STAGE + (wave - 4) * STRIP));
       constexpr int B = CASE_EPI_BIAS_COL, R = CASE_EPI_RESIDUAL, D = CASE_EPI_DROPOUT, G = CASE_EPI_GELU;
-      constexpr int RL = CASE_EPI_RELU, DG = CASE_EPI_MUL_DGELU, DR = CASE_EPI_MUL_DRELU;
+      constexpr int RL = CASE_EPI_RELU, DG = CASE_EPI_MUL_DGELU, DR = CASE_EPI_MUL_DRELU, RM = CASE_EPI_ROW_MASK;
 #define EPI(E)                                                                                  \
   {                                                                                             \
     if constexpr (sizeof(OutT) == 4) epilogue_regs<E, OutT>(g, epi, le, row_w, col_w, acc, g.C); \
@@ -641,6 +665,7 @@
       switch (epi) {
         case 0: EPI(0); break;
         case B: EPI(B); break;
+        case B | RM: EPI(B | RM); break;
         case B | R: EPI(B | R); break;
         case B | R | D: EPI(B | R | D); break;
         case B | G: EPI(B | G); break;
diff --git a/case_rg_amd/csrc/gemm_impl.inc b/case_rg_amd/csrc/gemm_impl.inc
--- a/case_rg_amd/csrc/gemm_impl.inc
+++ b/case_rg_amd/csrc/gemm_impl.inc
@@ -271,6 +271,7 @@
 template <typename T, typename OutT>
 struct Epilogue {
   OutT* C; const T* aux; T* aux_out; const float* bias_row; const float* bias_col;
+  const uint8_t* row_mask;
   int64_t ldc, ld_aux, M, N;
   float alpha, drop_p, drop_scale;
   uint64_t seed, rng_base;
@@ -288,6 +289,7 @@
     if (epi & CASE_EPI_MUL_DRELU) v = Elem<T>::ld(aux + row * ld_aux + col) > 0.f ? v : 0.f;
     if (epi & CASE_EPI_DROPOUT) v = rng_uniform(seed, rng_base + (uint64_t)(row * N + col)) >= drop_p ? v * drop_scale : 0.f;
     if (epi & CASE_EPI_RESIDUAL) v += Elem<T>::ld(aux + row * ld_aux + col);
+    if (epi & CASE_EPI_ROW_MASK) v = row_mask[row] ? v : 0.f;
     OutT* dst = C + row * ldc + col;
     if constexpr (sizeof(OutT) == 4) {
       if (epi & CASE_EPI_ATOMIC) atomicAdd(reinterpret_cast<float*>(dst), v);
@@ -340,6 +342,11 @@
       if (epi & CASE_EPI_RESIDUAL) {
 #pragma unroll
         for (int e = 0; e < 8; ++e) v[e] += ax[e];
+      }
+      if (epi & CASE_EPI_ROW_MASK) {
+        const bool keep = row_mask[row] != 0;
+#pragma unroll
+        for (int e = 0; e < 8; ++e) v[e] = keep ? v[e] : 0.f;
       }
       store8(C + row * ldc + col, v);
     } else {
@@ -441,6 +448,7 @@
   ep.aux_out = g.aux_out ? reinterpret_cast<T*>(g.aux_out) + b1 * g.saux1 + b2 * g.saux2 : nullptr;
   ep.bias_row = g.bias_row ? g.bias_row + batch * g.M : nullptr;
   ep.bias_col = g.bias_col;
+  ep.row_mask = g.row_mask ? g.row_mask + batch * g.M : nullptr;
   ep.ldc = g.ldc; ep.ld_aux = g.ld_aux; ep.M = g.M; ep.N = g.N;
   ep.alpha = g.alpha; ep.drop_p = g.drop_p; ep.seed = g.seed;
   ep.rng_base = g.offset + rng_base_of(g.state) + (uint64_t)(batch * g.M * g.N);
diff --git a/case_rg_amd/csrc/gemm_small.inc b/case_rg_amd/csrc/gemm_small.inc
--- a/case_rg_amd/csrc/gemm_small.inc
+++ b/case_rg_amd/csrc/gemm_small.inc
@@ -158,7 +158,7 @@
 
   gemm_w4::Epilogue<bf16_t, OutT> E;
   E.C = reinterpret_cast<OutT*>(g.C); E.aux = reinterpret_cast<const bf16_t*>(g.aux); E.aux_out = reinterpret_cast<bf16_t*>(g.aux_out);
-  E.bias_row = g.bias_row; E.bias_col = g.bias_col; E.ldc = g.ldc; E.ld_aux = g.ld_aux; E.M = g.M; E.N = g.N;
+  E.bias_row = g.bias_row; E.bias_col = g.bias_col; E.row_mask = g.row_mask; E.ldc = g.ldc; E.ld_aux = g.ld_aux; E.M = g.M; E.N = g.N;
   E.alpha = g.alpha; E.drop_p = g.drop_p; E.drop_scale = (epi & CASE_EPI_DROPOUT) ? 1.f / (1.f - g.drop_p) : 1.f;
   E.seed = g.seed; E.rng_base = g.offset + rng_base_of(g.state); E.epi = epi;
 #pragma unroll
diff --git a/case_rg_amd/csrc/rowops.hip b/case_rg_amd/csrc/rowops.hip
--- a/case_rg_amd/csrc/rowops.hip
+++ b/case_rg_amd/csrc/rowops.hip
@@ -47,7 +47,8 @@
                                                             const float* __restrict__ mean,
                                                             const float* __restrict__ rstd, T* __restrict__ dx,
                                                             const T* __restrict__ dx_add, float* __restrict__ d_gamma,
-                                                            float* __restrict__ d_beta, int64_t rows, int64_t cols) {
+                                                            float* __restrict__ d_beta, int64_t rows, int64_t cols,
+                                                            const uint8_t* __restrict__ out_valid = nullptr) {
   __shared__ float red[32];
   float acc_g[LN_MAXPT], acc_b[LN_MAXPT];
 #pragma unroll
@@ -74,13 +75,15 @@
     const float m1 = block_sum(s1, red) / (float)cols;
     const float m2 = block_sum(s2, red) / (float)cols;
     T* dxr = dx + r * cols;
+    const bool keep = !out_valid || out_valid[r];
 #pragma unroll
     for (int i = 0; i < LN_MAXPT; ++i) {
       const int64_t c = threadIdx.x + (int64_t)i * LN_THREADS;
       if (c < cols) {
         const float xh = (Elem<T>::ld(xr + c) + (x2r ? Elem<T>::ld(x2r + c) : 0.f) - mu) * rs;
         const float g = Elem<T>::ld(dyr + c) * gamma[c];
-        Elem<T>::st(dxr + c, rs * (g - m1 - xh * m2) + (dx_add ? Elem<T>::ld(dx_add + r * cols + c) : 0.f));
+        const float o = rs * (g - m1 - xh * m2) + (dx_add ? Elem<T>::ld(dx_add + r * cols + c) : 0.f);
+        Elem<T>::st(dxr + c, keep ? o : 0.f);
       }
     }
   }
@@ -160,7 +163,7 @@
                                                          const float* __restrict__ mean, const float* __restrict__ rstd,
                                                          T* __restrict__ dx, const T* __restrict__ dx_add,
                                                          float* __restrict__ d_gamma, float* __restrict__ d_beta, int64_t rows,
-                                                         int64_t cols) {
+                                                         int64_t cols, const uint8_t* __restrict__ out_valid = nullptr) {
   constexpr int E = Vec16<T>::N;
   extern __shared__ float part[];
   const int lane = threadIdx.x & 63, wid = threadIdx.x >> 6;
@@ -204,6 +207,7 @@
       }
     }
     const float m1 = wave_sum(s1) / (float)cols, m2 = wave_sum(s2) / (float)cols;
+    const bool keep = !out_valid || out_valid[r];
 #pragma unroll
     for (int i = 0; i < NV; ++i) {
       const int64_t c = ((int64_t)i * 64 + lane) * E;
@@ -217,6 +221,8 @@
 #pragma unroll
           for (int e = 0; e < E; ++e) o[e] += w[e];
         }
+#pragma unroll
+        for (int e = 0; e < E; ++e) o[e] = keep ? o[e] : 0.f;
         Vec16<T>::store(dx + r * cols + c, o);
       }
     }
@@ -298,13 +304,14 @@
   V::store(reinterpret_cast<T*>(dr.out) + idx, q);
 }
 
-template <typename T, int NV, bool HAS_X2, bool HAS_ADD, bool DROP2 = false, typename V = Vec16<T>>
+template <typename T, int NV, bool HAS_X2, bool HAS_ADD, bool DROP2 = false, typename V = Vec16<T>, bool MASK = false>
 __global__ __launch_bounds__(256) void ln_bwd_vec_kernel(const T* __restrict__ dy, const T* __restrict__ x,
                                                          const T* __restrict__ x2, const float* __restrict__ gamma,
                                                          const float* __restrict__ mean, const float* __restrict__ rstd,
                                                          T* __restrict__ dx, const T* __restrict__ dx_add,
                                                          float* __restrict__ d_gamma, float* __restrict__ d_beta, int64_t rows,
-                                                         int64_t cols, const LnDrop dr = LnDrop()) {
+                                                         int64_t cols, const LnDrop dr = LnDrop(),
+                                                         const uint8_t* __restrict__ out_valid = nullptr) {
   constexpr int E = V::N;
   typedef typename V::raw raw_t;
   extern __shared__ float part[];
@@ -323,11 +330,13 @@
   struct Raw {
     raw_t x[NV], d[NV], x2[HAS_X2 ? NV : 1], add[HAS_ADD ? NV : 1];
     float mu, rs;
+    uint8_t keep;
   };
   auto request = [&](Raw& w, int64_t r) {
     const int64_t base = r * cols + (int64_t)lane * E;
     w.mu = mean[r];
     w.rs = rstd[r];
+    if constexpr (MASK) w.keep = out_valid[r];
 #pragma unroll
     for (int i = 0; i < NV; ++i) {
       const int64_t o = base + (int64_t)i * 64 * E;
@@ -380,6 +389,10 @@
         V::unpack(cur.add[i], w);
 #pragma unroll
         for (int e = 0; e < E; ++e) o[e] += w[e];
+      }
+      if constexpr (MASK) {
+#pragma unroll
+        for (int e = 0; e < E; ++e) o[e] = cur.keep ? o[e] : 0.f;
       }
       V::store(dx + r * cols + ((int64_t)i * 64 + lane) * E, o);
       if constexpr (DROP2) ln_store_dropped<T, V>(dr, r * cols + ((int64_t)i * 64 + lane) * E, o);
@@ -538,9 +551,9 @@
 }
 
 template <typename T>
-void ln_bwd_vec_launch(const void* dy, const void* x, const void* x2, const float* gamma, const float* mean,
+bool ln_bwd_vec_launch(const void* dy, const void* x, const void* x2, const float* gamma, const float* mean,
                        const float* rstd, void* dx, const void* dx_add, float* dg, float* db, int64_t rows, int64_t cols,
-                       hipStream_t s) {
+                       hipStream_t s, const uint8_t* ov = nullptr) {
   constexpr int E = Vec16<T>::N;
   const int nv = (int)((cols + 64 * E - 1) / (64 * E));
   if constexpr (sizeof(T) == 2) {
@@ -554,7 +567,7 @@
       else LN8B(5);
 #undef LN8B
 #undef LN8
-      return;
+      return false;
     }
     if (cols % 256 == 0 && cols % 512 != 0 && cols <= 15 * 256) {
       constexpr int R = 2;
@@ -566,17 +579,17 @@
       else if (dx_add) LNS8(false, true);
       else LNS8(false, false);
 #undef LNS8
-      return;
+      return false;
     }
   }
   if (cols != (int64_t)nv * 64 * E || nv > 8) {
     const int grid = grid_for(rows, 4, 16, 256 * 4);
     const size_t lds = 2 * cols * sizeof(float);
-#define LNG(NVV) hipLaunchKernelGGL((ln_bwd_vec_guarded_kernel<T, NVV>), dim3(grid), dim3(256), lds, s, (const T*)dy, (const T*)x, (const T*)x2, gamma, mean, rstd, (T*)dx, (const T*)dx_add, dg, db, rows, cols)
+#define LNG(NVV) hipLaunchKernelGGL((ln_bwd_vec_guarded_kernel<T, NVV>), dim3(grid), dim3(256), lds, s, (const T*)dy, (const T*)x, (const T*)x2, gamma, mean, rstd, (T*)dx, (const T*)dx_add, dg, db, rows, cols, ov)
     switch (nv) { case 1: LNG(1); break; case 2: LNG(2); break; case 3: LNG(3); break; case 4: LNG(4); break;
                   case 5: LNG(5); break; case 6: LNG(6); break; case 7: LNG(7); break; default: LNG(8); break; }
 #undef LNG
-    return;
+    return true;
   }
   if (nv >= 3) {
     constexpr int R = 2;
@@ -587,16 +600,26 @@
     else if (dx_add) LNS(false, true);
     else LNS(false, false);
 #undef LNS
-    return;
+    return false;
   }
   const int grid = grid_for(rows, 4, 8, 256 * 8);
   const size_t lds = 8 * cols * sizeof(float);
 #define LNB(NVV, X2, ADD) hipLaunchKernelGGL((ln_bwd_vec_kernel<T, NVV, X2, ADD>), dim3(grid), dim3(256), lds, s, (const T*)dy, (const T*)x, (const T*)x2, gamma, mean, rstd, (T*)dx, (const T*)dx_add, dg, db, rows, cols)
 #define LNB2(NVV) do { if (x2 && dx_add) LNB(NVV, true, true); else if (x2) LNB(NVV, true, false); else if (dx_add) LNB(NVV, false, true); else LNB(NVV, false, false); } while (0)
-  if (nv == 1) LNB2(1);
-  else LNB2(2);
+#define LNM(NVV, X2, ADD) hipLaunchKernelGGL((ln_bwd_vec_kernel<T, NVV, X2, ADD, false, Vec16<T>, true>), dim3(grid), dim3(256), lds, s, (const T*)dy, (const T*)x, (const T*)x2, gamma, mean, rstd, (T*)dx, (const T*)dx_add, dg, db, rows, cols, LnDrop(), ov)
+#define LNM2(NVV) do { if (x2 && dx_add) LNM(NVV, true, true); else if (x2) LNM(NVV, true, false); else if (dx_add) LNM(NVV, false, true); else LNM(NVV, false, false); } while (0)
+  if (ov) {
+    if (nv == 1) LNM2(1);
+    else LNM2(2);
+  } else {
+    if (nv == 1) LNB2(1);
+    else LNB2(2);
+  }
+#undef LNM2
+#undef LNM
 #undef LNB2
 #undef LNB
+  return true;
 }
 
 template <int TPR>
@@ -1114,6 +1137,13 @@
 extern "C" int case_layernorm_bwd(const void* dy, const void* x, const void* x2, const float* gamma, const float* mean,
                                   const float* rstd, void* dx, const void* dx_add, float* d_gamma, float* d_beta,
                                   int64_t rows, int64_t cols, int32_t dtype, case_stream_t stream) {
+  return case_layernorm_bwd_masked(dy, x, x2, gamma, mean, rstd, dx, dx_add, nullptr, d_gamma, d_beta, rows, cols, dtype, stream);
+}
+
+extern "C" int case_layernorm_bwd_masked(const void* dy, const void* x, const void* x2, const float* gamma, const float* mean,
+                                         const float* rstd, void* dx, const void* dx_add, const uint8_t* out_row_valid, float* d_gamma,
+                                         float* d_beta, int64_t rows, int64_t cols, int32_t dtype, case_stream_t stream) {
+  const uint8_t* ov = out_row_valid;
   CASE_REQUIRE(dy && x && gamma && mean && rstd && dx && d_gamma && d_beta && rows > 0 && cols > 0,
                "case_layernorm_bwd: bad argument");
   CASE_REQUIRE(cols <= (int64_t)LN_THREADS * LN_MAXPT, "case_layernorm_bwd: cols %lld > %d", (long long)cols,
@@ -1121,19 +1151,21 @@
   const int grid = grid_for(rows, 1, 8, 256 * 2);
   hipStream_t s = (hipStream_t)stream;
   if (dtype == CASE_F32 && ln_vec_ok<float>(dy, x, dx, cols) && ln_vec_ok<float>(x2, dx_add, nullptr, cols)) {
-    ln_bwd_vec_launch<float>(dy, x, x2, gamma, mean, rstd, dx, dx_add, d_gamma, d_beta, rows, cols, s);
-    return case_check_launch("case_layernorm_bwd");
+    const bool masked = ln_bwd_vec_launch<float>(dy, x, x2, gamma, mean, rstd, dx, dx_add, d_gamma, d_beta, rows, cols, s, ov);
+    const int rc = case_check_launch("case_layernorm_bwd");
+    return (rc || !ov || masked) ? rc : case_mask_rows(dx, ov, dx, rows, cols, dtype, stream);
   }
   if (dtype == CASE_BF16 && ln_vec_ok<bf16_t>(dy, x, dx, cols) && ln_vec_ok<bf16_t>(x2, dx_add, nullptr, cols)) {
-    ln_bwd_vec_launch<bf16_t>(dy, x, x2, gamma, mean, rstd, dx, dx_add, d_gamma, d_beta, rows, cols, s);
-    return case_check_launch("case_layernorm_bwd");
+    const bool masked = ln_bwd_vec_launch<bf16_t>(dy, x, x2, gamma, mean, rstd, dx, dx_add, d_gamma, d_beta, rows, cols, s, ov);
+    const int rc = case_check_launch("case_layernorm_bwd");
+    return (rc || !ov || masked) ? rc : case_mask_rows(dx, ov, dx, rows, cols, dtype, stream);
   }
   if (dtype == CASE_F32)
     hipLaunchKernelGGL(ln_bwd_kernel<float>, dim3(grid), dim3(LN_THREADS), 0, s, (const float*)dy, (const float*)x,
-                       (const float*)x2, gamma, mean, rstd, (float*)dx, (const float*)dx_add, d_gamma, d_beta, rows, cols);
+                       (const float*)x2, gamma, mean, rstd, (float*)dx, (const float*)dx_add, d_gamma, d_beta, rows, cols, ov);
   else
     hipLaunchKernelGGL(ln_bwd_kernel<bf16_t>, dim3(grid), dim3(LN_THREADS), 0, s, (const bf16_t*)dy, (const bf16_t*)x,
-                       (const bf16_t*)x2, gamma, mean, rstd, (bf16_t*)dx, (const bf16_t*)dx_add, d_gamma, d_beta, rows, cols);
+                       (const bf16_t*)x2, gamma, mean, rstd, (bf16_t*)dx, (const bf16_t*)dx_add, d_gamma, d_beta, rows, cols, ov);
   return case_check_launch("case_layernorm_bwd");
 }
 
diff --git a/case_rg_amd/ops.py b/case_rg_amd/ops.py
--- a/case_rg_amd/ops.py
+++ b/case_rg_amd/ops.py
@@ -134,7 +134,7 @@
 
 def gemm(a, b, c, M, N, K, lda, ldb, ldc, *, a_off=0, b_off=0, c_off=0, a_kmajor=False, b_kmajor=False,
          batch1=1, batch2=1, sa=(0, 0), sb=(0, 0), sc=(0, 0), alpha=1.0, epilogue=0, bias_col=None, bias_row=None,
-         aux=None, aux_out=None, ld_aux=0, saux=(0, 0), split_k=1, drop=None, rowsum_out=None):
+         aux=None, aux_out=None, ld_aux=0, saux=(0, 0), split_k=1, drop=None, rowsum_out=None, row_mask=None):
     d = A.GemmDesc()
     d.M, d.N, d.K, d.lda, d.ldb, d.ldc, d.ld_aux = M, N, K, lda, ldb, ldc, ld_aux
     d.batch1, d.batch2 = batch1, batch2
@@ -156,6 +156,11 @@
     if drop is not None and drop[0] > 0.0:
         epilogue |= A.EPI_DROPOUT
         d.drop_p, d.seed, d.offset, d.state = _drop4(drop)
+    if row_mask is not None:
+        if row_mask.dtype != torch.uint8 or not row_mask.is_contiguous() or row_mask.numel() != batch1 * batch2 * M:
+            raise TypeError("gemm row_mask must be a contiguous uint8 tensor of batch * M elements")
+        epilogue |= A.EPI_ROW_MASK
+        d.row_mask = _ptr(row_mask)
     d.epilogue, d.split_k, d.alpha = epilogue, split_k, alpha
     if TILE_TRACE is not None:
         TILE_TRACE.append(A.lib.case_gemm_tile_for(d, _ptr(a, a_off), _ptr(b, b_off), _ptr(c, c_off), _ptr(bias_col), _ptr(aux),
@@ -499,9 +504,36 @@
     return y.view(*x.shape[:-1], N), xn.view(x.shape)
 
 
+ROW_MASK_FUSED = os.environ.get("CASE_ROW_MASK_FUSED", "1") != "0"
+
+
+class RowMaskPromise(object):
+    __slots__ = ("valid", "rows", "taken")
+
+    def __init__(self, valid_u8):
+        self.valid, self.rows, self.taken = valid_u8, valid_u8.numel(), False
+
+    def take(self, x):
+        if self.taken or x.numel() // x.shape[-1] != self.rows:
+            return None
+        self.taken = True
+        return self.valid
+
+
+def row_mask_promise(t):
+    return getattr(t, "_case_row_mask_promise", None)
+
+
+def carry_row_mask_promise(src, dst):
+    p = row_mask_promise(src)
+    if p is not None:
+        dst._case_row_mask_promise = p
+    return dst
+
+
 class FFNFn(Function):
     @staticmethod
-    def forward(ctx, x, w1, b1, w2, b2, act, p_inner, p_out, residual, ln_g=None, ln_b=None, ln_eps=0.0):
+    def forward(ctx, x, w1, b1, w2, b2, act, p_inner, p_out, residual, ln_g=None, ln_b=None, ln_eps=0.0, promise=None):
         K, F_, N = x.shape[-1], w1.shape[0], w2.shape[0]
         x2 = x.reshape(-1, K)
         if not x2.is_contiguous():
@@ -522,7 +554,11 @@
         if residual is not None:
             res2 = residual.reshape(M, N).contiguous()
             epi |= A.EPI_RESIDUAL
-        gemm(a, w2c, y, M, N, F_, F_, F_, N, epilogue=epi, bias_col=b2, aux=res2, ld_aux=N, drop=drop_o)
+        gemm(a, w2c, y, M, N, F_, F_, F_, N, epilogue=epi, bias_col=b2, aux=res2, ld_aux=N, drop=drop_o,
+             row_mask=None if promise is None else promise.valid)
+        ctx.promise = promise
+        if promise is not None and (ln_g is not None or promise.rows != M):
+            raise ValueError("ffn row_valid: one flag per output row, and no LayerNorm tail behind a masked output")
         ctx.meta = (x.shape, act, drop_i, drop_o, residual is not None, residual is x and N == K)
         if ln_g is not None:
             n, g_, mean, rstd = _ln_tail_forward(y, (ln_g, ln_b, ln_eps))
@@ -550,6 +586,11 @@
             g = dy.reshape(M, N)
             if not g.is_contiguous():
                 g = g.contiguous()
+            if ctx.promise is not None and not ctx.promise.taken:
+                masked = torch.empty_like(g)
+                A.call("case_mask_rows", _ptr(g), _ptr(ctx.promise.valid), _ptr(masked), M, N, _code(g), _stream())
+                g = masked
+                dy = g.view(dy.shape)
             fuse_res = res_is_x and ctx.needs_input_grad[0] and g.dtype == x2.dtype
             d_res = dy if (has_res and not fuse_res) else None
             g_res = g
@@ -571,10 +612,18 @@
             else:
                 gemm(dz, w1c, dx, M, K, F_, F_, K, K, b_kmajor=True)
             dx = dx.view(xshape)
-        return dx, dw1, db1, dw2, db2, None, None, None, d_res, d_lng, d_lnb, None
-
-
-def ffn(x, w1, b1, w2, b2, act, p_inner=0.0, p_out=0.0, residual=None, ln=None):
+        return dx, dw1, db1, dw2, db2, None, None, None, d_res, d_lng, d_lnb, None, None
+
+
+def ffn(x, w1, b1, w2, b2, act, p_inner=0.0, p_out=0.0, residual=None, ln=None, row_valid=None):
+    if row_valid is not None:
+        if ln is not None:
+            raise ValueError("ffn: row_valid and ln cannot be combined")
+        promise = RowMaskPromise(_u8(row_valid).reshape(-1))
+        y = FFNFn.apply(x, w1, b1, w2, b2, act, p_inner, p_out, residual, None, None, 0.0, promise)
+        if y.requires_grad:
+            y._case_row_mask_promise = promise
+        return y
     if ln is not None:
         if LN_TAIL:
             return FFNFn.apply(x, w1, b1, w2, b2, act, p_inner, p_out, residual, ln[0], ln[1], ln[2])
@@ -585,7 +634,7 @@
 class LayerNormFn(Function):
 
     @staticmethod
-    def forward(ctx, x, x2, gamma, beta, eps, carry=False):
+    def forward(ctx, x, x2, gamma, beta, eps, carry=False, out_row_valid=None):
         C = x.shape[-1]
         xa = x.reshape(-1, C)
         xa = xa if xa.is_contiguous() else xa.contiguous()
@@ -602,6 +651,7 @@
                _code(xa), _stream())
         ctx.save_for_backward(xa, xb, g, mean, rstd)
         ctx.shape = x.shape
+        ctx.out_row_valid = out_row_valid
         if carry:
             return y.view(x.shape), x.view_as(x)
         return y.view(x.shape)
@@ -618,18 +668,23 @@
             extra = extra if extra.is_contiguous() else extra.contiguous()
         dx = torch.empty_like(xa)
         dg, db = _zeros_like_shapes(xa.device, (C,), (C,))
-        A.call("case_layernorm_bwd", _ptr(dy2), _ptr(xa), _ptr(xb), _ptr(g), _ptr(mean), _ptr(rstd), _ptr(dx), _ptr(extra),
-               _ptr(dg), _ptr(db), R, C, _code(xa), _stream())
+        if ctx.out_row_valid is not None:
+            A.call("case_layernorm_bwd_masked", _ptr(dy2), _ptr(xa), _ptr(xb), _ptr(g), _ptr(mean), _ptr(rstd), _ptr(dx), _ptr(extra),
+                   _ptr(ctx.out_row_valid), _ptr(dg), _ptr(db), R, C, _code(xa), _stream())
+        else:
+            A.call("case_layernorm_bwd", _ptr(dy2), _ptr(xa), _ptr(xb), _ptr(g), _ptr(mean), _ptr(rstd), _ptr(dx), _ptr(extra),
+                   _ptr(dg), _ptr(db), R, C, _code(xa), _stream())
         dx = dx.view(ctx.shape)
-        return dx, (dx if xb is not None else None), dg, db, None, None
+        return dx, (dx if xb is not None else None), dg, db, None, None, None
 
 
 def layer_norm(x, gamma, beta, eps=1e-5, add=None):
     return LayerNormFn.apply(x, add, gamma, beta, eps)
 
 
-def layer_norm_carry(x, gamma, beta, eps=1e-5):
-    return LayerNormFn.apply(x, None, gamma, beta, eps, True)
+def layer_norm_carry(x, gamma, beta, eps=1e-5, promise=None):
+    valid = promise.take(x) if promise is not None else None
+    return LayerNormFn.apply(x, None, gamma, beta, eps, True, valid)
 
 
 def _softmax_desc(outer, inner, R, C, causal, in_dt, out_dt, drop):
diff --git a/include/case_hip.h b/include/case_hip.h
--- a/include/case_hip.h
+++ b/include/case_hip.h
@@ -19,7 +19,7 @@
   CASE_E_LAUNCH = -3
 };
 
-#define CASE_ABI_VERSION 600
+#define CASE_ABI_VERSION 610
 int case_version(void);
 enum {
   CASE_FEAT_GEMM_256 = 1u << 0,
@@ -70,7 +70,8 @@
   CASE_EPI_MUL_DGELU = 32,
   CASE_EPI_MUL_DRELU = 64,
   CASE_EPI_ATOMIC = 128,
-  CASE_EPI_DROPOUT = 256
+  CASE_EPI_DROPOUT = 256,
+  CASE_EPI_ROW_MASK = 512
 };
 
 typedef struct {
@@ -88,6 +89,7 @@
   float drop_p;
   uint64_t seed, offset;
   const CaseStepState* state;
+  const uint8_t* row_mask;
 } CaseGemmDesc;
 
 int case_gemm(const CaseGemmDesc* d, const void* A, const void* B, void* C, const float* bias_col,
@@ -118,6 +120,9 @@
 int case_layernorm_bwd(const void* dy, const void* x, const void* x2, const float* gamma, const float* mean,
                        const float* rstd, void* dx, const void* dx_add, float* d_gamma, float* d_beta, int64_t rows,
                        int64_t cols, int32_t dtype, case_stream_t stream);
+int case_layernorm_bwd_masked(const void* dy, const void* x, const void* x2, const float* gamma, const float* mean, const float* rstd,
+                              void* dx, const void* dx_add, const uint8_t* out_row_valid, float* d_gamma, float* d_beta, int64_t rows,
+                              int64_t cols, int32_t dtype, case_stream_t stream);
 int case_layernorm_bwd_dropout(const void* dy, const void* x, const float* gamma, const float* mean, const float* rstd, void* dx,
                                void* dx_dropped, float* d_gamma, float* d_beta, int64_t rows, int64_t cols, float p, uint64_t seed,
                                uint64_t offset, const CaseStepState* state, int32_t dtype, case_stream_t stream);
```

Result: no change. 1.349 million tokens/s, median of 6 (+0.5%).
